# NUSTM/FacialMMT

Measured on AMD Instinct MI355X. Metric: utterances/sec T+A+V forward+bwd, 160-frame face seq, 1/2/4/8 GPU, higher is better.
Workload: dtype bf16; 1 GPU; configs[1]: T+A+V, RoBERTa-large (random init), 160-frame face seq (uint8 112x112 crops, fused pil-bicubic x2 + normalise), batch 4 utterances/GPU, bf16, fwd+bwd+clip+AdamW every step; global_batch=4, parallelism=dp1, hip_graphs=whole step: 2 graphs (fwd+bwd | clip+optimizer), text_encoder_concurrent_with_swin=True, swin_forward_pipelined_across_steps=False, text_encoder_parameters=bf16 with fp32 master weights in the optimizer

## Files before the change

facialmmt_amd/_lib.py:

```python
from __future__ import annotations

import ctypes as C
import os

_HERE = os.path.dirname(os.path.abspath(__file__))
LIB_PATH = os.path.join(_HERE, "libfmmt_hip.so")

F32, BF16 = 0, 1
GENERIC = 0x100
EPI_NONE, EPI_GELU, EPI_GELU_BWD, EPI_GELU_DG, EPI_MUL_AUX = 0, 1, 2, 3, 4
SAVE_DG = 0x200
BATCH_MAJOR = 0x400
RESIZE_PIL, RESIZE_CV2 = 0, 1

_p, _i, _f, _sz, _u64 = C.c_void_p, C.c_int, C.c_float, C.c_size_t, C.c_uint64

SIGNATURES = {
    "fmmt_version": (_i, []),
    "fmmt_linear_fwd": (_i, [_i, _i, _i, _i, _p, _i, _p, _i, _p, _p, _i, _p, _i, _p, _i, _p, _i, _p, _i, _p]),
    "fmmt_linear_splitk_workspace": (_sz, [_i, _i, _i]),
    "fmmt_linear_fwd_splitk": (_i, [_i, _i, _i, _i, _p, _i, _p, _i, _p, _p, _i, _p, _sz, _p]),
    "fmmt_linear_wgrad_workspace": (_sz, [_i, _i, _i, _i]),
    "fmmt_linear_wgrad": (_i, [_i, _i, _i, _i, _p, _i, _p, _i, _p, _p, _p, _i, _i, _p, _sz, _p]),
    "fmmt_linear_wgrad_partials": (_i, [_i, _i, _i, _i, _p, _i, _p, _i, _i, _p, _i, _i, _p, _sz, _p]),
    "fmmt_mlp_fwd": (_i, [_i, _i, _i, _p, _p, _p, _p, _p, _p, _p, _i, _p, _p, _p, _p]),
    "fmmt_mlp_ln_fwd": (_i, [_i, _i, _i, _p, _p, _p, _f, _p, _p, _p, _p, _p, _i, _p, _p, _p, _p, _p, _p, _p]),
    "fmmt_mlp_bwd_input": (_i, [_i, _i, _i, _p, _p, _p, _p, _p, _i, _p, _p, _p]),
    "fmmt_linear_ln_bwd_workspace": (_sz, [_i]),
    "fmmt_linear_ln_bwd": (_i, [_i, _i, _i, _i, _p, _p, _p, _p, _p, _p, _p, _p, _p, _p, _p, _sz, _p]),
    "fmmt_mlp_ln_bwd_input_workspace": (_sz, [_i]),
    "fmmt_mlp_ln_bwd_input": (_i, [_i, _i, _i, _p, _p, _p, _p, _p, _i, _p, _p, _p, _p, _p, _p, _p, _p, _p, _sz, _p]),
    "fmmt_linear_wgrad_finish": (_i, [_i, _i, _i, _i, _p, _p, _p, _sz, _p]),
    "fmmt_layernorm_fwd": (_i, [_i, _i, _i, _p, _p, _p, _f, _p, _p, _p, _i, _p]),
    "fmmt_layernorm_bwd_workspace": (_sz, [_i]),
    "fmmt_layernorm_bwd": (_i, [_i, _i, _i, _p, _p, _p, _p, _p, _p, _p, _p, _p, _i, _p, _sz, _p]),
    "fmmt_window_attn_fwd": (_i, [_i, _i, _i, _i, _i, _i, _i, _p, _p, _p, _p, _i, _i, _f, _p, _p, _p]),
    "fmmt_window_attn_bwd_workspace": (_sz, [_i]),
    "fmmt_window_attn_bwd": (_i, [_i, _i, _i, _i, _i, _i, _i, _p, _p, _p, _p, _p, _p, _p, _i, _i, _f, _p, _p, _p, _sz, _p]),
    "fmmt_window_block_fwd": (_i, [_i, _i, _i, _i, _i, _i, _i, _p, _p, _p, _f, _p, _p, _p, _p, _p, _p, _f, _p, _p, _p, _p, _p, _p, _p, _p]),
    "fmmt_window_block_fwd_ref": (_i, [_i, _i, _i, _i, _i, _i, _i, _p, _p, _p, _f, _p, _p, _p, _p, _p, _p, _f, _p, _p, _p, _p, _p, _p, _p, _p]),
    "fmmt_window_block_attn_bwd": (_i, [_i, _i, _i, _i, _i, _i, _i, _p, _p, _p, _p, _p, _p, _p, _p, _p, _f, _p, _p, _p, _p, _sz, _p]),
    "fmmt_window_block_attn_bwd_ref": (_i, [_i, _i, _i, _i, _i, _i, _i, _p, _p, _p, _p, _p, _p, _p, _p, _p, _f, _p, _p, _p, _p, _sz, _p]),
    "fmmt_linear_fwd_seg3": (_i, [_i, _i, _i, _i, _p, _i, _p, _p, _p, _i, _i, _p, _p, _p, _p, _i, _p]),
    "fmmt_select_frames_fwd": (_i, [_i, _i, _i, _i, _i, _i, _p, _p, _p, _p, _f, _p, _p, _p, _p]),
    "fmmt_select_frames_bwd": (_i, [_i, _i, _i, _i, _i, _i, _p, _p, _p, _p]),
    "fmmt_mha_fwd": (_i, [_i, _i, _i, _i, _i, _i, _p, _i, _p, _p, _i, _f, _p, _f, _u64, _p, _p, _i, _p, _p]),
    "fmmt_mha_bwd": (_i, [_i, _i, _i, _i, _i, _i, _p, _i, _p, _p, _i, _f, _p, _f, _u64, _p, _p, _p, _i, _p, _p, _i, _p, _p, _i, _p]),
    "fmmt_mha_avg_weights": (_i, [_i, _i, _i, _i, _i, _i, _p, _i, _p, _i, _f, _p, _f, _u64, _p, _p, _p, _p]),
    "fmmt_patch_im2col": (_i, [_i, _i, _p, _p, _p]),
    "fmmt_patch_col2im": (_i, [_i, _i, _p, _p, _p]),
    "fmmt_batchnorm1d_fwd": (_i, [_i, _i, _i, _p, _p, _p, _p, _p, _f, _f, _i, _p, _p, _p, _p]),
    "fmmt_batchnorm1d_bwd": (_i, [_i, _i, _i, _p, _p, _p, _p, _p, _i, _p, _p, _p, _p]),
    "fmmt_posemb_scale_fwd": (_i, [_i, _i, _i, _i, _p, _p, _f, _p, _p]),
    "fmmt_scale": (_i, [_i, _sz, _p, _f, _p, _p]),
    "fmmt_colsum": (_i, [_i, _i, _i, _i, _p, _i, _p, _p]),
    "fmmt_cast_batch": (_i, [_i, _i, _p, _p]),
    "fmmt_layernorm_bwd_bf16_workspace": (_sz, [_i, _i]),
    "fmmt_layernorm_bwd_bf16": (_i, [_i, _i, _f, _p, _p, _p, _p, _p, _p, _p, _sz, _p]),
    "fmmt_dropadd_ln_fwd": (_i, [_i, _i, _i, _f, _p, _p, _p, _p, _f, _u64, _p, _u64, _p, _p, _p]),
    "fmmt_dropadd_ln_bwd_workspace": (_sz, [_i, _i]),
    "fmmt_dropadd_ln_bwd": (_i, [_i, _i, _i, _f, _p, _p, _p, _f, _u64, _p, _u64, _p, _p, _p, _p, _p, _p, _sz, _p]),
    "fmmt_plm_dropadd_ln_fwd": (_i, [_i, _i, _f, _p, _p, _p, _p, _f, _u64, _p, _u64, _p, _p, _p]),
    "fmmt_embedding_bwd": (_i, [_i, _i, _i, _p, C.c_int64, _p, _p, _p]),
    "fmmt_plm_gelu_bwd_colsum_workspace": (_sz, [_i, _i]),
    "fmmt_plm_gelu_bwd_colsum": (_i, [_i, _i, _p, _p, _p, _p, _p, _sz, _p]),
    "fmmt_plm_dropadd_ln_bwd_workspace": (_sz, [_i, _i]),
    "fmmt_plm_dropadd_ln_bwd": (_i, [_i, _i, _f, _p, _p, _p, _f, _u64, _p, _u64, _p, _p, _p, _p, _p, _p, _sz, _p]),
    "fmmt_grad_handover": (_i, [_i, _i, _p, _p, _p, _p]),
    "fmmt_adamw_batch": (_i, [_i, _i, _p, _p, _p, _p, _f, _f, _f, _f, _f, _i, _p]),
    "fmmt_resize_table": (_i, [_i, _i, _i, _p, _p]),
    "fmmt_resize_band_rows": (_i, [_p, _i]),
    "fmmt_patch_embed_u8": (_i, [_i, _i, _i, _i, _p, _p, _p, _p, _p]),
    "fmmt_patch_embed_ln_fwd": (_i, [_i, _i, _i, _i, _p, _p, _p, _p, _p, _f, _p, _p, _p, _p, _p]),
    "fmmt_patch_embed_u8_ln_fwd": (_i, [_i, _i, _i, _i, _p, _p, _p, _p, _p, _p, _p, _f, _p, _p, _p, _p, _p, _p]),
    "fmmt_emotion_head_fwd": (_i, [_i, _i, _i, _i, _i, _p, _i, _p, _p, _p, _p, _p, _f, _p, _p, _p]),
    "fmmt_eval_accumulate": (_i, [_i, _i, _i, _p, _i, _p, _p, _p, _p, _p, _p, C.c_int64, C.c_int64, _p]),
}

POOL_HEAD_SIGNATURES = {
    "fmmt_pool_head_bwd_workspace": (_sz, [_i, _i, _i]),
    "fmmt_pool_head_fwd": (_i, [_i, _i, _i, _i, _i, _p, _p, _p, _p, _p, _p, _p, _p, _p, _f, _u64, _p, _p, _p, _p, _p, _p, _p, _sz, _p]),
    "fmmt_pool_head_bwd": (_i, [_i, _i, _i, _i, _i, _p, _p, _p, _p, _p, _p, _p, _p, _p, _p, _p, _p, _p, _p, _p, _p, _p, _p, _p, _sz, _p]),
}

RAGGED_SIGNATURES = {
    "fmmt_pack_frames": (_i, [_i, _i, _i, _sz, _p, _p, _p, _p, _p]),
    "fmmt_batchnorm1d_fwd_n": (_i, [_i, _i, _i, _p, _p, _p, _p, _p, _p, _f, _f, _i, _p, _p, _p, _p]),
    "fmmt_batchnorm1d_bwd_n": (_i, [_i, _i, _i, _p, _p, _p, _p, _p, _p, _i, _p, _p, _p, _p]),
    "fmmt_select_frames_fwd_n": (_i, [_i, _i, _i, _i, _i, _i, _p, _p, _p, _p, _f, _p, _p, _p, _p, _p]),
}

EVAL_COLLECT_SIGNATURES = {
    "fmmt_eval_accumulate_at": (_i, [_i, _i, _i, _p, _i, _p, _p, _p, _p, _p, _p, _p, _p, C.c_int64, _p]),
}

POOL_HEAD_ROWS_SIGNATURES = {
    "fmmt_pool_head_fwd_rows": (_i, [_i, _i, _i, _i, _i, _p, _p, _p, _p, _p, _p, _p, _p, _p, _f, _u64, _p, _p, _p, _p, _p, _p, _p, _p, _sz, _p]),
    "fmmt_pool_head_bwd_rows": (_i, [_i, _i, _i, _i, _i, _p, _p, _p, _p, _p, _p, _p, _p, _p, _p, _p, _p, _p, _p, _p, _p, _p, _p, _p, _p, _sz, _p]),
}

GUARD_SIGNATURES = {
    "fmmt_adamw_batch_guarded": (_i, [_i, _i, _p, _p, _p, _p, _f, _f, _f, _f, _f, _i, _p]),
    "fmmt_guard_commit": (_i, [_p, _p, _p, _p]),
    "fmmt_monitor_loss": (_i, [_p, _f, _p, _p]),
}
GUARD_LOSS_SUM, GUARD_MICRO_STEPS, GUARD_NONFINITE_LOSSES, GUARD_APPLIED, GUARD_SKIPPED, GUARD_LAST_NORM, GUARD_WORDS = 0, 1, 2, 3, 4, 5, 6

FMMT_EINVAL, FMMT_EALIGN, FMMT_EWORKSPACE = -1, -2, -3
_ERR = {-1: "FMMT_EINVAL (bad shape / unsupported size)", -2: "FMMT_EALIGN (pointer or leading dimension not 16-byte aligned)",
        -3: "FMMT_EWORKSPACE (workspace too small)"}

_lib = None


class FmmtError(RuntimeError):
    pass


def load():
    global _lib
    if _lib is not None:
        return _lib
    if not os.path.exists(LIB_PATH):
        raise FmmtError(f"{LIB_PATH} is missing: build it with `python -m facialmmt_amd.build` "
                        f"(or __graft_entry__.build()); there is no CPU / PyTorch fallback for the hot path")
    lib = C.CDLL(LIB_PATH)
    for name, (res, args) in list(SIGNATURES.items()) + list(POOL_HEAD_SIGNATURES.items()) + list(RAGGED_SIGNATURES.items()) + list(EVAL_COLLECT_SIGNATURES.items()) + list(POOL_HEAD_ROWS_SIGNATURES.items()) + list(GUARD_SIGNATURES.items()):
        fn = getattr(lib, name)
        fn.restype = res
        fn.argtypes = args
    _lib = lib
    return lib


def check(rc: int, what: str):
    if rc != 0:
        msg = _ERR.get(rc, f"hipError_t {rc}")
        raise FmmtError(f"{what} failed: {msg}")


def dtype_code(t) -> int:
    import torch
    if t == torch.float32:
        return F32
    if t == torch.bfloat16:
        return BF16
    raise FmmtError(f"unsupported activation dtype {t}: the HIP path computes in float32 (parity) or bfloat16 (throughput)")
```

facialmmt_amd/build.py:

```python
from __future__ import annotations

import glob
import os
import subprocess
import sys
from concurrent.futures import ThreadPoolExecutor

HERE = os.path.dirname(os.path.abspath(__file__))
CSRC = os.path.join(HERE, "csrc")
OUT = os.path.join(HERE, "libfmmt_hip.so")
SOURCES = ["gemm.hip", "layernorm.hip", "attn.hip", "wattn_mfma.hip", "wattn_bwd_ref.hip", "wblock.hip", "wblock_ref.hip", "mha_mfma.hip", "misc.hip", "preproc.hip", "mlp_fused.hip", "mlp_ref.hip", "patch_ln.hip", "lin_lnbwd.hip", "plm_fused.hip", "frame_filter.hip", "eval.hip", "pool_head.hip", "ragged.hip", "guard.hip"]
FLAGS = ["--offload-arch=gfx950", "-O3", "-std=c++17", "-fPIC", "-ffp-contract=fast"]


def _stale(target, deps):
    if not os.path.exists(target):
        return True
    t = os.path.getmtime(target)
    return any(os.path.getmtime(d) > t for d in deps)


def build(force: bool = False, verbose: bool = True, tag: str = "") -> str:
    hipcc = os.environ.get("HIPCC", "/opt/rocm/bin/hipcc")
    tag = tag or os.environ.get("FMMT_BUILD_TAG", "")
    csrc = os.environ.get("FMMT_CSRC_DIR", CSRC) if tag else CSRC
    headers = sorted(glob.glob(os.path.join(csrc, "*.h"))) + [os.path.join(csrc, "..", "..", "include", h) for h in ("fmmt.h", "fmmt_pool_head.h", "fmmt_ragged.h", "fmmt_eval_collect.h", "fmmt_pool_head_rows.h", "fmmt_guard.h")]
    objdir = os.path.join(HERE, "build_" + tag if tag else "build")
    out = os.path.join(HERE, f"libfmmt_hip_{tag}.so") if tag else OUT
    os.makedirs(objdir, exist_ok=True)
    jobs = []
    for s in SOURCES:
        src = os.path.join(csrc, s)
        obj = os.path.join(objdir, s.replace(".hip", ".o"))
        if force or _stale(obj, [src] + headers):
            jobs.append((src, obj))

    def cc(job):
        src, obj = job
        cmd = [hipcc] + FLAGS + os.environ.get("FMMT_CFLAGS", "").split() + ["-c", src, "-o", obj]
        if verbose:
            print(" ".join(cmd), flush=True)
        subprocess.run(cmd, check=True)

    with ThreadPoolExecutor(max_workers=4) as ex:
        list(ex.map(cc, jobs))
    objs = [os.path.join(objdir, s.replace(".hip", ".o")) for s in SOURCES]
    if force or jobs or _stale(out, objs):
        cmd = [hipcc, "--offload-arch=gfx950", "-shared", "-fPIC", "-o", out] + objs
        if verbose:
            print(" ".join(cmd), flush=True)
        subprocess.run(cmd, check=True)
    return out


if __name__ == "__main__":
    print(build(force="--force" in sys.argv))
```

facialmmt_amd/csrc/gemm.hip:

```cpp
#include "gemm_common.h"
#include "gemm_ph.h"
#include "gemm_ph3.h"
#include <stdlib.h>
#include <type_traits>

namespace {

template <typename T> struct Mma;
template <> struct Mma<bf16> {
    static constexpr int KM = 32;
    static constexpr int KP = 8;
    using frag = bf16x8;
    static __device__ __forceinline__ f32x4 mma(frag a, frag b, f32x4 c) {
        return __builtin_amdgcn_mfma_f32_16x16x32_bf16(a, b, c, 0, 0, 0);
    }
    static __device__ __forceinline__ frag load(const bf16* p) { return *reinterpret_cast<const bf16x8*>(p); }
};
template <> struct Mma<float> {
    static constexpr int KM = 4;
    static constexpr int KP = 1;
    using frag = float;
    static __device__ __forceinline__ f32x4 mma(frag a, frag b, f32x4 c) {
        return __builtin_amdgcn_mfma_f32_16x16x4f32(a, b, c, 0, 0, 0);
    }
// ... 362 lines not shown
    }

    auto compute = [&](int buf) {
        const T* sb = S + buf * STAGE;
        bf16x8 wf[NT], xf[MT];
#pragma unroll
        for (int b = 0; b < NT; ++b) wf[b] = *reinterpret_cast<const bf16x8*>(sb + woff[b]);
#pragma unroll
        for (int a = 0; a < MT; ++a) xf[a] = *reinterpret_cast<const bf16x8*>(sb + xoff[a]);
#pragma unroll
        for (int a = 0; a < MT; ++a)
#pragma unroll
            for (int b = 0; b < NT; ++b) acc[a][b] = __builtin_amdgcn_mfma_f32_16x16x32_bf16(wf[b], xf[a], acc[a][b], 0, 0, 0);
    };

    issue(0, 0);
    if (nk > 1) issue(1, BK);
    if constexpr (NK > 0) {
#pragma unroll
        for (int kt = 0; kt < NK; ++kt) {
            wait_stage(kt + 1 < NK);
            __builtin_amdgcn_s_barrier();
            if (kt + 2 < NK) issue((kt + 2) % 3, (kt + 2) * BK);
            compute(kt % 3);
        }
    } else {
        int cur = 0;
        for (int kt = 0; kt < nk; ++kt) {
            wait_stage(kt + 1 < nk);
            __builtin_amdgcn_s_barrier();
            if (kt + 2 < nk) issue(cur == 0 ? 2 : cur - 1, (kt + 2) * BK);
            compute(cur);
            cur = cur == 2 ? 0 : cur + 1;
        }
    }
    const bool plain = p.epi == 0 && !p.y_pre && !p.res && !p.aux && !p.rowscale;
    if (p.part || (!plain && BN != 128)) {
        nt_epilogue<T, MT, NT>(p, acc, m0 + wm * 64, n0 + wn * WN, li, lg);
    } else if (plain) {
        nt_epilogue_slab<T, MT, NT, 2, BN, 512>(p, acc, smem, wm, wn, li, lg, tid, m0, n0);
    } else {
        if constexpr (BN == 128) {
            asm volatile("s_waitcnt lgkmcnt(0)" ::: "memory");
            __builtin_amdgcn_s_barrier();
            nt_epilogue_wslab<T>(p, acc, smem + wave * (16 * 272), lane, li, lg, m0 + wm * 64, n0 + wn * WN);
        }
    }
}


template <int N> __device__ __forceinline__ void wait_vm() { asm volatile("s_waitcnt vmcnt(%0)" ::"n"(N) : "memory"); }

#define FMMT_RD(o, ad) "ds_read_b128 %" #o ", %" #ad "\n\t"
template <int NF>
__device__ __forceinline__ void nt_read_frags(bf16x8 (&o)[NF], const unsigned (&ad)[NF]) {
    static_assert(NF >= 10 && NF <= 12, "fragments per K block");
    if constexpr (NF == 12) {
        asm volatile(FMMT_RD(0, 12) FMMT_RD(1, 13) FMMT_RD(2, 14) FMMT_RD(3, 15) FMMT_RD(4, 16) FMMT_RD(5, 17) FMMT_RD(6, 18) FMMT_RD(7, 19)
                     FMMT_RD(8, 20) FMMT_RD(9, 21) FMMT_RD(10, 22) FMMT_RD(11, 23) "s_waitcnt lgkmcnt(0)"
                     : "=&v"(o[0]), "=&v"(o[1]), "=&v"(o[2]), "=&v"(o[3]), "=&v"(o[4]), "=&v"(o[5]), "=&v"(o[6]), "=&v"(o[7]),
                       "=&v"(o[8]), "=&v"(o[9]), "=&v"(o[10]), "=&v"(o[11])
                     : "v"(ad[0]), "v"(ad[1]), "v"(ad[2]), "v"(ad[3]), "v"(ad[4]), "v"(ad[5]), "v"(ad[6]), "v"(ad[7]),
                       "v"(ad[8]), "v"(ad[9]), "v"(ad[10]), "v"(ad[11])
                     : "memory");
    } else if constexpr (NF == 11) {
        asm volatile(FMMT_RD(0, 11) FMMT_RD(1, 12) FMMT_RD(2, 13) FMMT_RD(3, 14) FMMT_RD(4, 15) FMMT_RD(5, 16) FMMT_RD(6, 17) FMMT_RD(7, 18)
                     FMMT_RD(8, 19) FMMT_RD(9, 20) FMMT_RD(10, 21) "s_waitcnt lgkmcnt(0)"
                     : "=&v"(o[0]), "=&v"(o[1]), "=&v"(o[2]), "=&v"(o[3]), "=&v"(o[4]), "=&v"(o[5]), "=&v"(o[6]), "=&v"(o[7]),
                       "=&v"(o[8]), "=&v"(o[9]), "=&v"(o[10])
                     : "v"(ad[0]), "v"(ad[1]), "v"(ad[2]), "v"(ad[3]), "v"(ad[4]), "v"(ad[5]), "v"(ad[6]), "v"(ad[7]),
                       "v"(ad[8]), "v"(ad[9]), "v"(ad[10])
                     : "memory");
    } else {
        asm volatile(FMMT_RD(0, 10) FMMT_RD(1, 11) FMMT_RD(2, 12) FMMT_RD(3, 13) FMMT_RD(4, 14) FMMT_RD(5, 15) FMMT_RD(6, 16) FMMT_RD(7, 17)
                     FMMT_RD(8, 18) FMMT_RD(9, 19) "s_waitcnt lgkmcnt(0)"
                     : "=&v"(o[0]), "=&v"(o[1]), "=&v"(o[2]), "=&v"(o[3]), "=&v"(o[4]), "=&v"(o[5]), "=&v"(o[6]), "=&v"(o[7]),
                       "=&v"(o[8]), "=&v"(o[9])
                     : "v"(ad[0]), "v"(ad[1]), "v"(ad[2]), "v"(ad[3]), "v"(ad[4]), "v"(ad[5]), "v"(ad[6]), "v"(ad[7]),
                       "v"(ad[8]), "v"(ad[9])
                     : "memory");
    }
}

template <int BN, int BK, int NBUF, bool BATCH = true, bool HASOP = false, bool PIPE = false>
__global__ __launch_bounds__(512) void linear_nt_p256_kernel(LinArgs p) {
    static_assert(BK == 64 && BATCH, "one K step, batched fragment reads");
    using T = bf16;
    constexpr int BM = 256, PITCH = BK, MT = 8, NT = BN / 64, WN = BN / 4, CW = 4 * NT;
    constexpr int RPI = 8;
    constexpr int STAGE = (BN + BM) * PITCH;
    constexpr int NI = (BN + BM) / RPI;
    constexpr int CNT_LO = NI / 8;
    static_assert(BN % 64 == 0 && (NBUF - 2) * (CNT_LO + 2) <= 63, "tile / vmcnt immediate");
    extern __shared__ __attribute__((aligned(16))) char smem[];
    T* S = reinterpret_cast<T*>(smem);
    float* bias_s = reinterpret_cast<float*>(smem + (size_t)NBUF * STAGE * sizeof(T));

    const int tid = threadIdx.x, lane = tid & 63;
    const int wave = __builtin_amdgcn_readfirstlane(tid >> 6);
    const int wm = wave >> 2, wn = wave & 3;
    const int li = lane & 15, lg = lane >> 4;
    const T* __restrict__ xg = reinterpret_cast<const T*>(p.x);
    const T* __restrict__ wg = reinterpret_cast<const T*>(p.w);
    const int nk = p.K / BK;

    typedef __attribute__((address_space(1))) const void gptr_t;
    typedef __attribute__((address_space(3))) void lptr_t;
    auto key = [](int row) { return (row >> 1) & 7; };
    const int rl = lane >> 3, cl = lane & 7;
    const bool wperm = HASOP ? !p.chan_rows : true;
    auto wchan = [&](int r) {
        const int w = r / WN, q = r - w * WN;
        return wperm ? w * WN + chan_of<CW>(q >> 4, (q >> 2) & 3, q & 3) : r;
    };

    const int my_cnt = (NI - wave + 7) / 8 + (wave == 7 ? 1 : 0);
    const bool cnt_hi = my_cnt > CNT_LO;
    constexpr int NP = (NI + 7) / 8;
    unsigned poff[NP], boff = 0;
    auto tile_offsets = [&](int m0, int n0) {
#pragma unroll
        for (int i = 0; i < NP; ++i) {
            const int row0 = (i * 8 + wave) * RPI;
            if (row0 < BN) {
                const int r = row0 + rl;
                poff[i] = ((unsigned)(n0 + wchan(r)) * (unsigned)p.ldw + (unsigned)((cl ^ key(r)) << 3)) * 2u;
            } else {
                const int rx = row0 - BN;
                const int rb = min(m0 + rx, p.M - RPI);
                poff[i] = ((unsigned)(rb + rl) * (unsigned)p.ldx + (unsigned)((cl ^ key(rx + rl)) << 3)) * 2u;
            }
        }
        boff = p.bias ? (unsigned)(n0 + min(lane * 4, BN - 4)) * 4u : (unsigned)lane * 16u;
    };
    auto issue_piece = [&](int i, int slot, unsigned kbyte) {
        const int j = i * 8 + wave;
        if (j < NI) {
            const int row0 = j * RPI;
            const char* b = row0 < BN ? reinterpret_cast<const char*>(wg) : reinterpret_cast<const char*>(xg);
            __builtin_amdgcn_global_load_lds((gptr_t*)(b + (size_t)(poff[i] + kbyte)), (lptr_t*)(S + slot * STAGE + row0 * PITCH), 16, 0, 0);
        }
    };
    auto issue_bias = [&](int par) {
        if (wave == 7) {
            const char* b = p.bias ? reinterpret_cast<const char*>(p.bias) : reinterpret_cast<const char*>(wg);
            __builtin_amdgcn_global_load_lds((gptr_t*)(b + (size_t)boff), (lptr_t*)(bias_s + par * 256), 16, 0, 0);
        }
    };
    auto wait_landed = [&](int ahead, int stores) {
        const int n = (ahead <= 0 ? 0 : (ahead == 1 ? 1 : 2)) * (CNT_LO + (cnt_hi ? 1 : 0)) + stores;
        switch (n) {
#define FMMT_W(N) case N: wait_vm<N>(); break;
            FMMT_W(1) FMMT_W(2) FMMT_W(3) FMMT_W(4) FMMT_W(5) FMMT_W(6) FMMT_W(7) FMMT_W(8) FMMT_W(9) FMMT_W(10) FMMT_W(11) FMMT_W(12)
            FMMT_W(13) FMMT_W(14) FMMT_W(15) FMMT_W(16) FMMT_W(17) FMMT_W(18) FMMT_W(19) FMMT_W(20) FMMT_W(21) FMMT_W(22) FMMT_W(23) FMMT_W(24)
#undef FMMT_W
            default: wait_vm<0>(); break;
        }
    };
    static_assert(NBUF >= 2 && NBUF <= 4, "ring depth");
    static_assert(NI % 8 == 0 || NI % 8 <= 7, "wave 7 never owns a high count plus the bias slab");

    f32x4 acc[MT][NT];
#pragma unroll
    for (int a = 0; a < MT; ++a)
#pragma unroll
        for (int b = 0; b < NT; ++b) acc[a][b] = f32x4{0.f, 0.f, 0.f, 0.f};
    int woff[NT], xoff[MT];
#pragma unroll
    for (int b = 0; b < NT; ++b) {
// ... 13 lines not shown
            unsigned ad[NT + MT];
#pragma unroll
            for (int b = 0; b < NT; ++b) ad[b] = (((unsigned)woff[b] * 2u) ^ (kk ? 64u : 0u)) + sbase;
#pragma unroll
            for (int a = 0; a < MT; ++a) ad[NT + a] = (((unsigned)xoff[a] * 2u) ^ (kk ? 64u : 0u)) + sbase;
            bf16x8 fr[NT + MT];
            nt_read_frags<NT + MT>(fr, ad);
#pragma unroll
            for (int a = 0; a < MT; ++a)
#pragma unroll
                for (int b = 0; b < NT; ++b) acc[a][b] = __builtin_amdgcn_mfma_f32_16x16x32_bf16(fr[b], fr[NT + a], acc[a][b], 0, 0, 0);
        }
    };

    const int G = gridDim.x;
    const int total = p.tiles_m * p.tiles_n;
    const int first = ((int)blockIdx.x & 7) * (G >> 3) + ((int)blockIdx.x >> 3);
    const int tstep = G;
    const int ntile = first < total ? (total - first + G - 1) / G : 0;
    const int nsteps = ntile * nk;
    int it = first, ik = 0, ipar = 0, islot = 0;
    tile_offsets((first / p.tiles_n) * BM, (first % p.tiles_n) * BN);
    auto issue_advance = [&]() {
        islot = islot + 1 == NBUF ? 0 : islot + 1;
        if (++ik == nk) {
            ik = 0;
            it += tstep;
            ipar ^= 1;
            tile_offsets((it / p.tiles_n) * BM, (it % p.tiles_n) * BN);
        }
    };
    auto issue_next = [&]() {
        const unsigned kbyte = (unsigned)ik * (BK * 2);
#pragma unroll
        for (int i = 0; i < NP; ++i) issue_piece(i, islot, kbyte);
        issue_bias(ipar);
        issue_advance();
    };
#pragma unroll
    for (int s = 0; s < NBUF - 1; ++s)
        if (s < nsteps) issue_next();
    int ct = first, ck = 0, cpar = 0, cslot = 0, st_prev = 0;
    EpiPre<MT, NT> pre;
    constexpr int PR = BN == 192 ? 32 : 16;
    constexpr int SP = BN * 2 + 16;
    constexpr int CPR = BN / 8;
    constexpr int NSL = PR * CPR / 256;
    static_assert((PR * CPR) % 256 == 0, "whole store instructions");
    char* scratch = smem + (size_t)NBUF * STAGE * sizeof(T) + 2 * 256 * sizeof(float) + (size_t)wm * PR * SP;
    const bool lds_epi = !HASOP && p.epi == 0 && !p.y_pre && !p.part && p.K <= 1536;
    T* __restrict__ yg = reinterpret_cast<T*>(p.y);
    constexpr int XB = NT >= 4 ? 2 : 4;
    constexpr int UB = MT / XB, U = (BK / 32) * UB;
    bf16x8 pw[2][NT], px[2][XB];
    auto request = [&](int slot, int u) {
        const unsigned sbase = lds0 + (unsigned)slot * (unsigned)(STAGE * 2);
        const int kk = u / UB, h = u % UB;
        const unsigned flip = kk ? 64u : 0u;
        if (h == 0) {
#pragma unroll
            for (int b = 0; b < NT; ++b)
                asm volatile("ds_read_b128 %0, %1" : "=v"(pw[kk & 1][b]) : "v"((((unsigned)woff[b] * 2u) ^ flip) + sbase) : "memory");
        }
#pragma unroll
        for (int a = 0; a < XB; ++a)
            asm volatile("ds_read_b128 %0, %1" : "=v"(px[u & 1][a]) : "v"((((unsigned)xoff[h * XB + a] * 2u) ^ flip) + sbase) : "memory");
    };
    auto landed = [&](int u) {
        const int kk = u / UB, h = u % UB;
        asm volatile("s_waitcnt lgkmcnt(0)" ::: "memory");
#pragma unroll
        for (int a = 0; a < XB; ++a) asm volatile("" : "+v"(px[u & 1][a]));
        if (h == 0) {
#pragma unroll
            for (int b = 0; b < NT; ++b) asm volatile("" : "+v"(pw[kk & 1][b]));
        }
    };
    bool pend = false;
    auto sync_stage = [&](int k, int ck_k, int ct_k) {
        wait_landed(min(nsteps - 1 - k, NBUF - 2), st_prev);
        st_prev = 0;
        __builtin_amdgcn_s_barrier();
        if constexpr (HASOP) {
            if (ck_k == nk - 1) nt_epilogue_prefetch<MT, NT>(p, pre, (ct_k / p.tiles_n) * BM + wm * 128, (ct_k % p.tiles_n) * BN + wn * WN, li, lg);
        }
        if constexpr (PIPE) {
            pend = k + NBUF - 1 < nsteps;
        } else {
            if (k + NBUF - 1 < nsteps) issue_next();
        }
    };
    constexpr int NG = BN == 256 ? 1 : 2;
    auto issue_group = [&](int g) {
        if (!pend) return;
        const unsigned kbyte = (unsigned)ik * (BK * 2);
#pragma unroll
        for (int i = 0; i < NP; ++i)
            if ((i * NG) / NP == g) issue_piece(i, islot, kbyte);
        if (g == NG - 1) {
            issue_bias(ipar);
            issue_advance();
        }
    };
    if constexpr (PIPE) {
        if (nsteps > 0) {
            sync_stage(0, 0, first);
            issue_group(0);
            request(0, 0);
            landed(0);
        }
    }
    for (int s = 0; s < nsteps; ++s) {
        if constexpr (PIPE) {
            const int nslot = cslot + 1 == NBUF ? 0 : cslot + 1;
#pragma unroll
            for (int u = 0; u < U; ++u) {
                int grp_now = -1;
                if (u + 1 < U) {
                    request(cslot, u + 1);
                    if (u + 1 < NG) grp_now = u + 1;
                } else if (s + 1 < nsteps) {
                    const bool wrap = ck + 1 == nk;
                    sync_stage(s + 1, wrap ? 0 : ck + 1, wrap ? ct + tstep : ct);
                    request(nslot, 0);
                    grp_now = 0;
                }
                __builtin_amdgcn_sched_barrier(0);
                if (grp_now >= 0) issue_group(grp_now);
                {
                    const int kk = u / UB, h = u % UB;
#pragma unroll
                    for (int a = 0; a < XB; ++a)
#pragma unroll
                        for (int b = 0; b < NT; ++b)
                            acc[h * XB + a][b] = __builtin_amdgcn_mfma_f32_16x16x32_bf16(pw[kk & 1][b], px[u & 1][a], acc[h * XB + a][b], 0, 0, 0);
                }
                __builtin_amdgcn_sched_barrier(0);
                if (u + 1 < U) landed(u + 1);
                else if (s + 1 < nsteps) landed(0);
            }
        } else {
            sync_stage(s, ck, ct);
            compute(cslot);
        }
        cslot = cslot + 1 == NBUF ? 0 : cslot + 1;
        if (++ck == nk) {
            const int m0 = (ct / p.tiles_n) * BM, n0 = (ct % p.tiles_n) * BN;
            if (p.bias) {
#pragma unroll
                for (int b = 0; b < NT; ++b) {
                    const f32x4 bb = *reinterpret_cast<const f32x4*>(bias_s + cpar * 256 + wn * WN + chan_of<CW>(b, lg, 0));
#pragma unroll
                    for (int a = 0; a < MT; ++a) acc[a][b] += bb;
                }
            }
            const bool gelu_any = p.epi == FMMT_EPI_GELU || p.epi == FMMT_EPI_GELU_DG;
            if (BN == 256 && !HASOP && !p.part && ((p.epi == 0 && !p.y_pre) || gelu_any)) {
                if constexpr (BN == 256) {
                    char* ws = smem + (size_t)NBUF * STAGE * sizeof(T) + 2 * 256 * sizeof(float) + wave * (16 * 144);
                    T* __restrict__ ypre = reinterpret_cast<T*>(p.y_pre);
                    const int mw = m0 + wm * 128, nw = n0 + wn * WN;
                    const int rr = lane >> 3, rc = lane & 7;
                    auto emit = [&](int a, T* dst, bool gelu) {
#pragma unroll
                        for (int c = 0; c < 2; ++c) {
                            float t[8];
#pragma unroll
// ... 10 lines not shown
                            const bf16x8 v = *reinterpret_cast<const bf16x8*>(ws + (h * 8 + rr) * 144 + rc * 16);
                            if (m < p.M) __builtin_nontemporal_store(v, reinterpret_cast<bf16x8*>(dst + (size_t)m * p.ldy + nw + rc * 8));
                        }
                    };
                    auto emit_dg = [&](int a) {
                        bf16x8 dv[2];
#pragma unroll
                        for (int c = 0; c < 2; ++c) {
                            float t[8], d[8];
#pragma unroll
                            for (int e = 0; e < 8; ++e) t[e] = acc[a][2 * c + (e >> 2)][e & 3];
                            gelu_both_inplace<T>(t, d, 8);
                            bf16x8 v;
#pragma unroll
                            for (int e = 0; e < 8; ++e) { v[e] = (bf16)t[e]; dv[c][e] = (bf16)d[e]; }
                            *reinterpret_cast<bf16x8*>(ws + li * 144 + chan_of<CW>(2 * c, lg, 0) * 2) = v;
                        }
#pragma unroll
                        for (int pass = 0; pass < 2; ++pass) {
                            T* dst = pass == 0 ? yg : ypre;
#pragma unroll
                            for (int h = 0; h < 2; ++h) {
                                const int m = mw + a * 16 + h * 8 + rr;
                                const bf16x8 v = *reinterpret_cast<const bf16x8*>(ws + (h * 8 + rr) * 144 + rc * 16);
                                if (m < p.M && dst) __builtin_nontemporal_store(v, reinterpret_cast<bf16x8*>(dst + (size_t)m * p.ldy + nw + rc * 8));
                            }
                            if (pass == 0) {
#pragma unroll
                                for (int c = 0; c < 2; ++c) *reinterpret_cast<bf16x8*>(ws + li * 144 + chan_of<CW>(2 * c, lg, 0) * 2) = dv[c];
                            }
                        }
                    };
                    const bool two = gelu_any && ypre != nullptr;
#pragma unroll
                    for (int a = 0; a < MT; ++a) {
                        if (p.epi == FMMT_EPI_GELU_DG) {
                            emit_dg(a);
                        } else {
                            if (two) emit(a, ypre, false);
                            emit(a, yg, p.epi == FMMT_EPI_GELU);
                        }
                    }
                    if (!PIPE && mw + 128 <= p.M) st_prev = MT * 2 * (two ? 2 : 1);
                }
            } else if (lds_epi) {
                const int rows_left = p.M - (m0 + wm * 128);
                auto round = [&](int pass) {
                    asm volatile("s_waitcnt lgkmcnt(0)" ::: "memory");
                    __builtin_amdgcn_s_barrier();
#pragma unroll
                    for (int f = 0; f < PR / 16; ++f) {
                        const int a = pass * (PR / 16) + f;
                        char* row = scratch + (f * 16 + li) * SP + (wn * WN) * 2;
#pragma unroll
                        for (int c = 0; c < NT / 2; ++c) {
                            bf16x8 v;
#pragma unroll
                            for (int e = 0; e < 8; ++e) v[e] = (bf16)acc[a][2 * c + (e >> 2)][e & 3];
                            *reinterpret_cast<bf16x8*>(row + chan_of<CW>(2 * c, lg, 0) * 2) = v;
                        }
                        if constexpr (NT % 2) {
                            bf16x4 v;
#pragma unroll
                            for (int e = 0; e < 4; ++e) v[e] = (bf16)acc[a][NT - 1][e];
                            *reinterpret_cast<bf16x4*>(row + chan_of<CW>(NT - 1, lg, 0) * 2) = v;
                        }
                    }
                    asm volatile("s_waitcnt lgkmcnt(0)" ::: "memory");
                    __builtin_amdgcn_s_barrier();
#pragma unroll
                    for (int i = 0; i < NSL; ++i) {
                        const int q = i * 256 + wn * 64 + lane, r = q / CPR, cc = q - r * CPR;
                        const int row = pass * PR + r;
                        if (row < rows_left) {
                            const bf16x8 v = *reinterpret_cast<const bf16x8*>(scratch + r * SP + cc * 16);
                            __builtin_nontemporal_store(v, reinterpret_cast<bf16x8*>(yg + (size_t)(m0 + wm * 128 + row) * p.ldy + n0 + cc * 8));
                        }
                    }
                };
#pragma unroll
                for (int pass = 0; pass < 128 / PR; ++pass) round(pass);
                if (!PIPE && rows_left >= 128) st_prev = (128 / PR) * NSL;
            } else if constexpr (HASOP) {
                nt_epilogue<T, MT, NT, true, true>(p, acc, m0 + wm * 128, n0 + wn * WN, li, lg, &pre);
            } else {
                nt_epilogue<T, MT, NT, true, false, true>(p, acc, m0 + wm * 128, n0 + wn * WN, li, lg);
            }
#pragma unroll
            for (int a = 0; a < MT; ++a)
#pragma unroll
                for (int b = 0; b < NT; ++b) acc[a][b] = f32x4{0.f, 0.f, 0.f, 0.f};
            ck = 0;
            ct += tstep;
            cpar ^= 1;
        }
    }
}

template <int BN, int BK, int NBUF, bool BATCH, bool HASOP, bool PIPE = false>
int launch_p256_b(const LinArgs& a, hipStream_t st) {
    constexpr size_t lds = (size_t)NBUF * (BN + 256) * BK * 2 + 2 * 256 * sizeof(float) + (BN == 256 ? 8 * 16 * 144 : 2 * (BN == 192 ? 32 : 16) * (BN * 2 + 16));
    static_assert(lds <= 160 * 1024, "LDS");
    static FmmtLdsOnce lds_once;
    if (int rc_ = lds_once.set(reinterpret_cast<const void*>(&linear_nt_p256_kernel<BN, BK, NBUF, BATCH, HASOP, PIPE>), (int)lds)) return rc_;
    LinArgs p = a;
    p.tiles_m = (a.M + 255) / 256;
    p.tiles_n = a.N / BN;
    hipLaunchKernelGGL((linear_nt_p256_kernel<BN, BK, NBUF, BATCH, HASOP, PIPE>), dim3(256), dim3(512), lds, st, p);
    FMMT_CHECK_LAUNCH();
    return 0;
}
template <int BN, int BK, int NBUF>
int launch_p256(const LinArgs& a, hipStream_t st) {
    if constexpr (BN != 256) {
        if (a.res || a.aux || a.rowscale) return launch_p256_b<BN, BK, NBUF, true, true>(a, st);
    }
    if (a.K >= 384) return launch_p256_b<BN, BK, NBUF, true, false, true>(a, st);
    return launch_p256_b<BN, BK, NBUF, true, false>(a, st);
}

int p256_plan(const LinArgs& a) {
    constexpr int P256_MINM = 16384;
    if (a.ksplit || a.M < P256_MINM || a.M % 16 || a.K % 64 || a.K < 96 || a.ldx % 8 || a.ldw % 8) return 0;
    if ((unsigned long long)a.M * a.ldx >= (1ull << 31) || (unsigned long long)a.N * a.ldw >= (1ull << 31)) return 0;
    const bool has_op = a.res || a.aux || a.rowscale;
    if (has_op && (a.aux || a.ldres % 8 || a.ldaux % 8)) return 0;
    const int tm = (a.M + 255) / 256;
    int best = 0;
    double best_cost = 0;
    const int cand[3] = {256, 192, 128};
    const double pen[3] = {1.0, 1.04, 1.10};
    for (int i = 0; i < 3; ++i) {
        const int bn = cand[i];
        if (a.N % bn) continue;
        if (has_op && bn == 256) continue;
        const int tiles = tm * (a.N / bn);
        if (tiles < 256) continue;
        const double cost = (double)((tiles + 255) / 256) * bn * pen[i];
        if (!best || cost < best_cost) {
            best = bn;
            best_cost = cost;
        }
    }
    return best;
}

template <typename T, int BM, int BN, int BK, int NBUF, bool GLDS = false, bool SEG = false>
int launch_nt(const LinArgs& a, hipStream_t st) {
    constexpr int VEC = Vec<T>::N;
    constexpr size_t lds = (size_t)NBUF * (BM + BN) * (GLDS ? BK : BK + VEC) * sizeof(T);
    static FmmtLdsOnce lds_once;
    if (lds > 65536) {
        if (int rc_ = lds_once.set(reinterpret_cast<const void*>(&linear_nt_kernel<T, BM, BN, BK, NBUF, GLDS, SEG>), (int)lds)) return rc_;
    }
    LinArgs p = a;
    p.tiles_n = (a.N + BN - 1) / BN;
    p.tiles_m = (a.M + BM - 1) / BM;
    const int grid = p.tiles_m * p.tiles_n;
    const int splits = a.ksplit ? (a.K + a.ksplit - 1) / a.ksplit : 1;
    hipLaunchKernelGGL((linear_nt_kernel<T, BM, BN, BK, NBUF, GLDS, SEG>), dim3(grid, splits), dim3(256), lds, st, p);
    FMMT_CHECK_LAUNCH();
    return 0;
}

template <typename T, int BM, int BN>
int dispatch_nt_bk(const LinArgs& a, hipStream_t st) {
    if constexpr (sizeof(T) == 2) {
        if (!a.ksplit && a.K == 96) return launch_nt<T, BM, BN, 96, 1>(a, st);
        if (!a.ksplit && a.K <= 64) return launch_nt<T, BM, BN, 64, 1>(a, st);
        if (a.K % 64 == 0 && !a.ksplit && a.ldx % 8 == 0 && a.ldw % 8 == 0) {
            if constexpr (BM == 64) {
                const int tiles = ((a.M + BM - 1) / BM) * ((a.N + BN - 1) / BN);
                if (a.K >= 2048 && tiles <= 256) return launch_nt<T, BM, BN, 64, 4, true>(a, st);
            }
            return launch_nt<T, BM, BN, 64, 2, true>(a, st);
        }
        if (a.K % 64 == 0 && (!a.ksplit || a.ksplit % 64 == 0)) return launch_nt<T, BM, BN, 64, 2>(a, st);
        return launch_nt<T, BM, BN, 32, 2>(a, st);
    } else {
        return launch_nt<T, BM, BN, 16, 2>(a, st);
    }
}

int ph_plan(const LinArgs& a, int* epi3) {
    const bool mul_aux = a.epi == FMMT_EPI_MUL_AUX && a.aux && !a.res && !a.y_pre && !a.bias;
    if (a.ksplit || a.part || (a.aux && !mul_aux)) return 0;
    const bool gelu_pre = a.epi == FMMT_EPI_GELU && a.y_pre, has_op = a.res || a.rowscale;
    if (!gelu_pre && !mul_aux && (a.epi != 0 || a.y_pre)) return 0;
    if (gelu_pre && (has_op || a.K < 1536)) return 0;
    if (mul_aux && (a.ldaux % 8 || (unsigned long long)a.M * a.ldaux >= (1ull << 31))) return 0;
    if (a.M < 4096 || a.M % 8 || a.N % 128 || a.K % 64 || a.K < 192 || a.ldx % 8 || a.ldw % 8 || a.ldy % 8) return 0;
    if (a.res && a.ldres % 8) return 0;
    if (a.rowscale && a.rows_per_scale <= 0) return 0;
    if ((unsigned long long)a.M * a.ldx >= (1ull << 31) || (unsigned long long)a.N * a.ldw >= (1ull << 31) || (unsigned long long)a.M * a.ldy >= (1ull << 31) ||
        (a.res && (unsigned long long)a.M * a.ldres >= (1ull << 31)))
        return 0;
    if (a.N % 256) {
        if (gelu_pre || a.K > 512) return 0;
        const long long t384 = (long long)((a.M + 383) / 384) * (a.N / 128), r384 = (t384 + 255) / 256;
// ... 38 lines not shown
        if (const int bn = p256_plan(a))
            return bn == 256 ? launch_p256<256, 64, 2>(a, st) : bn == 192 ? launch_p256<192, 64, 2>(a, st) : launch_p256<128, 64, 3>(a, st);
        constexpr int DEEP_MINM = 65536, DEEP_MINK = 96;
        const bool big = a.M >= DEEP_MINM && !a.ksplit && a.K % 32 == 0 && a.K >= DEEP_MINK && a.ldx % 8 == 0 && a.ldw % 8 == 0 &&
                         !(a.K == 96 && a.epi == FMMT_EPI_GELU);
        if (big && (a.N % 128 == 0 || n96)) {
            constexpr size_t lds = (size_t)3 * (256 + 128) * 64 * 2;
            constexpr size_t lds96 = (size_t)3 * (256 + 96) * 32 * 2;
            static FmmtLdsOnce lds_once[7];
            {
                const void* fns[] = {reinterpret_cast<const void*>(&linear_nt_deep_kernel),
                                     reinterpret_cast<const void*>(&linear_nt_deep32_kernel<0, 128>),
                                     reinterpret_cast<const void*>(&linear_nt_deep32_kernel<6, 128>),
                                     reinterpret_cast<const void*>(&linear_nt_deep32_kernel<3, 128>),
                                     reinterpret_cast<const void*>(&linear_nt_deep32_kernel<0, 96>),
                                     reinterpret_cast<const void*>(&linear_nt_deep32_kernel<6, 96>),
                                     reinterpret_cast<const void*>(&linear_nt_deep32_kernel<3, 96>)};
                const int sizes[] = {(int)lds, (int)lds / 2, (int)lds / 2, (int)lds / 2, (int)lds96, (int)lds96, (int)lds96};
                for (int i = 0; i < 7; ++i)
                    if (int rc_ = lds_once[i].set(fns[i], sizes[i])) return rc_;
            }
            LinArgs p = a;
            p.tiles_m = (a.M + 255) / 256;
                    if (n96) {
                p.tiles_n = a.N / 96;
                if (a.K == 192) hipLaunchKernelGGL((linear_nt_deep32_kernel<6, 96>), dim3(p.tiles_m * p.tiles_n), dim3(512), lds96, st, p);
                else if (a.K == 96) hipLaunchKernelGGL((linear_nt_deep32_kernel<3, 96>), dim3(p.tiles_m * p.tiles_n), dim3(512), lds96, st, p);
                else hipLaunchKernelGGL((linear_nt_deep32_kernel<0, 96>), dim3(p.tiles_m * p.tiles_n), dim3(512), lds96, st, p);
                FMMT_CHECK_LAUNCH();
                return 0;
            }
            p.tiles_n = a.N / 128;
            if (a.epi != 0 || a.K <= 512 || a.K % 64 != 0) {
                if (a.K == 192) hipLaunchKernelGGL((linear_nt_deep32_kernel<6, 128>), dim3(p.tiles_m * p.tiles_n), dim3(512), lds / 2, st, p);
                else if (a.K == 96) hipLaunchKernelGGL((linear_nt_deep32_kernel<3, 128>), dim3(p.tiles_m * p.tiles_n), dim3(512), lds / 2, st, p);
                else hipLaunchKernelGGL((linear_nt_deep32_kernel<0, 128>), dim3(p.tiles_m * p.tiles_n), dim3(512), lds / 2, st, p);
            } else {
                hipLaunchKernelGGL(linear_nt_deep_kernel, dim3(p.tiles_m * p.tiles_n), dim3(512), lds, st, p);
            }
            FMMT_CHECK_LAUNCH();
            return 0;
        }
    }
    return n96 ? dispatch_nt_bk<T, 128, 96>(a, st) : dispatch_nt_bk<T, 128, 128>(a, st);
}

template <typename T>
__global__ void splitk_finish_kernel(const float* __restrict__ part, int splits, int M, int N, const float* __restrict__ bias,
                                     T* __restrict__ y, int ldy) {
    const size_t i = (size_t)blockIdx.x * blockDim.x + threadIdx.x;
    if (i >= (size_t)M * N) return;
    const int m = (int)(i / N), n = (int)(i - (size_t)m * N);
    float t = bias ? bias[n] : 0.f;
    for (int s = 0; s < splits; ++s) t += part[(size_t)s * M * N + i];
    y[(size_t)m * ldy + n] = from_f32<T>(t);
}

int splitk_plan(int M, int N, int K, int* ksplit) {
    const int bm = M <= 4096 ? 64 : 128;
    const int tiles = ((M + bm - 1) / bm) * ((N + 127) / 128);
    if (tiles >= 128 || K < 4096) { *ksplit = 0; return 1; }
    int splits = 512 / tiles;
    if (splits > 32) splits = 32;
    int ks = (K + splits - 1) / splits;
    ks = (ks + 63) / 64 * 64;
    *ksplit = ks;
    return (K + ks - 1) / ks;
}

struct TnArgs {
    int M, N, K;
    const void* dy; int lddy;
    const void* x; int ldx;
    float* part_w;
    float* part_b;
    const float* rowscale; int rows_per_scale;
    int tiles_k;
    int chunk;
    int tiles_n;
    int x_gelu;
    int* hdr;
    int splits;
    int npad;
};

__device__ __forceinline__ int tn_swz(int row) { return (row & 3) | (((row >> 3) & 1) << 2); }
__device__ __forceinline__ bf16x8 lds_tr_frag_swz(const bf16* s, int row0, int c0, int li, int lg) {
    const int r = row0 + lg * 8 + (li >> 2);
    const bf16* a0 = s + r * 128 + (((c0 >> 4) ^ tn_swz(r)) << 4) + (li & 3) * 4;
    typedef __attribute__((address_space(3))) s16x4 lds_s16x4;
    s16x4 lo = __builtin_amdgcn_ds_read_tr16_b64_v4i16((lds_s16x4*)(a0));
    s16x4 hi = __builtin_amdgcn_ds_read_tr16_b64_v4i16((lds_s16x4*)(a0 + 4 * 128));
    union { struct { s16x4 lo, hi; } s; bf16x8 v; } u;
    u.s.lo = lo;
    u.s.hi = hi;
    return u.v;
}

template <int BMS> struct TnWaves { static constexpr int value = BMS >= 64 ? 2 : 3; };
template <typename T, int BMS, bool FEW = false, int PF = 1>
__global__ __launch_bounds__(256) __attribute__((amdgpu_waves_per_eu(TnWaves<BMS>::value)))
void linear_tn_kernel(TnArgs p) {
    constexpr int VEC = Vec<T>::N;
    constexpr bool SWZ = sizeof(T) == 2;
    constexpr int PITCH = SWZ ? 128 : 128 + VEC;
    constexpr int CV = 128 / VEC;
    constexpr int NV = BMS * CV / 256;
    constexpr int KM = sizeof(T) == 2 ? 32 : 4;

    extern __shared__ __attribute__((aligned(16))) char smem[];
    T* As = reinterpret_cast<T*>(smem);
    T* Bs = As + 2 * BMS * PITCH;
    float* bsum = reinterpret_cast<float*>(Bs + 2 * BMS * PITCH);

    const int tid = threadIdx.x, lane = tid & 63, wave = tid >> 6;
    const int wn = wave >> 1, wk = wave & 1;
    const int li = lane & 15, lg = lane >> 4;
    const int tiles = p.tiles_n * p.tiles_k;
    const int logical = xcd_remap(blockIdx.x, gridDim.x);
    const int split = logical / tiles, tile = logical - split * tiles;
    const int tile_n = tile / p.tiles_k, tile_k = tile % p.tiles_k;
    const int n0 = tile_n * 128, k0 = tile_k * 128;
    const int mbeg = split * p.chunk, mend = min(p.M, mbeg + p.chunk);
    if (p.hdr && blockIdx.x == 0 && tid == 0) { p.hdr[0] = p.splits; p.hdr[1] = 0; p.hdr[2] = p.N; }

    const T* __restrict__ dyg = reinterpret_cast<const T*>(p.dy);
    const T* __restrict__ xg = reinterpret_cast<const T*>(p.x);
    const bool do_bias = (p.part_b != nullptr) && (tile_k == 0);

    struct Regs { Vec<T> a[NV], b[NV]; float s[NV]; };
    Regs R0, R1;
    float colsum[VEC];
#pragma unroll
    for (int e = 0; e < VEC; ++e) colsum[e] = 0.f;

    int sidx[NV], srem[NV];
#pragma unroll
    for (int i = 0; i < NV; ++i) {
        const int m = mbeg + (tid + i * 256) / CV;
        sidx[i] = p.rowscale ? m / p.rows_per_scale : 0;
        srem[i] = p.rowscale ? m - sidx[i] * p.rows_per_scale : 0;
    }
    auto gload = [&](Regs& R, int mb) {
#pragma unroll
        for (int i = 0; i < NV; ++i) {
            const int v = tid + i * 256;
            const int row = v / CV, c = (v % CV) * VEC;
            const int m = mb + row;
            const bool mv = m < mend;
            R.a[i] = (mv && n0 + c < p.N) ? ldvec<T>(dyg + (size_t)m * p.lddy + n0 + c) : zerovec<T>();
            if (p.rowscale) {
                R.s[i] = mv ? p.rowscale[sidx[i]] : 0.f;
                srem[i] += BMS;
                while (srem[i] >= p.rows_per_scale) {
                    srem[i] -= p.rows_per_scale;
                    ++sidx[i];
                }
            }
            R.b[i] = (mv && k0 + c < p.K) ? ldvec<T>(xg + (size_t)m * p.ldx + k0 + c) : zerovec<T>();
        }
    };
    auto lstore = [&](Regs& R, int buf) {
#pragma unroll
        for (int i = 0; i < NV; ++i) {
            const int v = tid + i * 256;
            const int row = v / CV, c = (v % CV) * VEC;
// ... 241 lines not shown
        }
    if (do_bias && li == 0) {
#pragma unroll
        for (int a = 0; a < 4; ++a)
#pragma unroll
            for (int r = 0; r < 4; ++r) p.part_b[n0 + a * 16 + lg * 4 + r] = accb[a][r];
    }
}

int launch_tn_few(int M, int N, int K, const void* dy, int lddy, const void* x, int ldx, float* dw, float* db, int* hdr, hipStream_t st) {
    constexpr int lds = 80 * 1024;
    static FmmtLdsOnce lds_once;
    if (int rc_ = lds_once.set(reinterpret_cast<const void*>(&linear_tn_few_kernel), lds)) return rc_;
    TnArgs a{M, N, K, dy, lddy, x, ldx, dw, db, nullptr, 1, K / 64, (M + 7) / 8, N / 64, 0, hdr, 1};
    hipLaunchKernelGGL(linear_tn_few_kernel, dim3((N / 64) * (K / 64)), dim3(512), lds, st, a);
    FMMT_CHECK_LAUNCH();
    return 0;
}

bool tn_few_ok(int M, int N, int K, int dtype) {
    return dtype == FMMT_BF16 && M > 128 && M <= 2048 && N % 64 == 0 && K % 64 == 0 && (N / 64) * (K / 64) >= 8 && (N / 64) * (K / 64) <= 1024;
}

__device__ __forceinline__ int tn_swz2(int row) { return ((row >> 1) & 1) | (((row >> 3) & 1) << 1); }
template <int CH>
__device__ __forceinline__ int tn_sigma(int row, int blk) {
    if constexpr (CH == 192) return blk < 8 ? (blk ^ tn_swz(row)) : 8 + ((blk & 3) ^ tn_swz2(row));
    else return blk ^ tn_swz(row);
}


#define FMMT_TR2(o0, o1, ad, im) "ds_read_b64_tr_b16 %" #o0 ", %" #ad "\n\tds_read_b64_tr_b16 %" #o1 ", %" #ad " offset:%" #im "\n\t"
template <int FA, int OFFA, int OFFB>
__device__ __forceinline__ void tn_read12(s16x4 (&o)[24], const unsigned (&ad)[12]) {
    static_assert(FA == 8 || FA == 6, "fragment split");
    if constexpr (FA == 8) {
        asm volatile(FMMT_TR2(0, 1, 24, 36) FMMT_TR2(2, 3, 25, 36) FMMT_TR2(4, 5, 26, 36) FMMT_TR2(6, 7, 27, 36)
                     FMMT_TR2(8, 9, 28, 36) FMMT_TR2(10, 11, 29, 36) FMMT_TR2(12, 13, 30, 36) FMMT_TR2(14, 15, 31, 36)
                     FMMT_TR2(16, 17, 32, 37) FMMT_TR2(18, 19, 33, 37) FMMT_TR2(20, 21, 34, 37) FMMT_TR2(22, 23, 35, 37)
                     "s_waitcnt lgkmcnt(0)"
                     : "=&v"(o[0]), "=&v"(o[1]), "=&v"(o[2]), "=&v"(o[3]), "=&v"(o[4]), "=&v"(o[5]), "=&v"(o[6]), "=&v"(o[7]),
                       "=&v"(o[8]), "=&v"(o[9]), "=&v"(o[10]), "=&v"(o[11]), "=&v"(o[12]), "=&v"(o[13]), "=&v"(o[14]), "=&v"(o[15]),
                       "=&v"(o[16]), "=&v"(o[17]), "=&v"(o[18]), "=&v"(o[19]), "=&v"(o[20]), "=&v"(o[21]), "=&v"(o[22]), "=&v"(o[23])
                     : "v"(ad[0]), "v"(ad[1]), "v"(ad[2]), "v"(ad[3]), "v"(ad[4]), "v"(ad[5]), "v"(ad[6]), "v"(ad[7]),
                       "v"(ad[8]), "v"(ad[9]), "v"(ad[10]), "v"(ad[11]), "n"(OFFA), "n"(OFFB)
                     : "memory");
    } else {
        asm volatile(FMMT_TR2(0, 1, 24, 36) FMMT_TR2(2, 3, 25, 36) FMMT_TR2(4, 5, 26, 36) FMMT_TR2(6, 7, 27, 36)
                     FMMT_TR2(8, 9, 28, 36) FMMT_TR2(10, 11, 29, 36) FMMT_TR2(12, 13, 30, 37) FMMT_TR2(14, 15, 31, 37)
                     FMMT_TR2(16, 17, 32, 37) FMMT_TR2(18, 19, 33, 37) FMMT_TR2(20, 21, 34, 37) FMMT_TR2(22, 23, 35, 37)
                     "s_waitcnt lgkmcnt(0)"
                     : "=&v"(o[0]), "=&v"(o[1]), "=&v"(o[2]), "=&v"(o[3]), "=&v"(o[4]), "=&v"(o[5]), "=&v"(o[6]), "=&v"(o[7]),
                       "=&v"(o[8]), "=&v"(o[9]), "=&v"(o[10]), "=&v"(o[11]), "=&v"(o[12]), "=&v"(o[13]), "=&v"(o[14]), "=&v"(o[15]),
                       "=&v"(o[16]), "=&v"(o[17]), "=&v"(o[18]), "=&v"(o[19]), "=&v"(o[20]), "=&v"(o[21]), "=&v"(o[22]), "=&v"(o[23])
                     : "v"(ad[0]), "v"(ad[1]), "v"(ad[2]), "v"(ad[3]), "v"(ad[4]), "v"(ad[5]), "v"(ad[6]), "v"(ad[7]),
                       "v"(ad[8]), "v"(ad[9]), "v"(ad[10]), "v"(ad[11]), "n"(OFFA), "n"(OFFB)
                     : "memory");
    }
}

template <int TNn, int TKk, int NBUF, int WN, bool SCALED = false>
__global__ __launch_bounds__(512) void linear_tn_dma_kernel(TnArgs p) {
    using T = bf16;
    constexpr int BT = 32, WK = 8 / WN;
    constexpr int CPRA = TNn / 8, CPRB = TKk / 8;
    constexpr int A_EL = BT * TNn, B_EL = BT * TKk, STAGE = A_EL + B_EL;
    constexpr int NIA = BT * CPRA / 64, NIB = BT * CPRB / 64, NI = NIA + NIB;
    static_assert((BT * CPRA) % 64 == 0 && (BT * CPRB) % 64 == 0, "whole DMA instructions per operand");
    constexpr int CNT = NI / 8, REM = NI % 8;
    constexpr int FA = TNn / (16 * WN), FB = TKk / (16 * WK);
    static_assert(TNn % (16 * WN) == 0 && TKk % (16 * WK) == 0 && FA + FB == 12 && NBUF >= 2 && NBUF <= 5, "tile");
    extern __shared__ __attribute__((aligned(16))) char smem[];
    T* S = reinterpret_cast<T*>(smem);

    const int tid = threadIdx.x, lane = tid & 63;
    const int wave = __builtin_amdgcn_readfirstlane(tid >> 6);
    const int wn = wave / WK, wk = wave % WK;
    const int li = lane & 15, lg = lane >> 4;
    const int tiles = p.tiles_n * p.tiles_k;
    const int logical = xcd_remap(blockIdx.x, gridDim.x);
    const int split = logical / tiles, tile = logical - split * tiles;
    const int tile_n = tile / p.tiles_k, tile_k = tile % p.tiles_k;
    const int n0 = tile_n * TNn, k0 = tile_k * TKk;
    const int mbeg = split * p.chunk, mend = min(p.M, mbeg + p.chunk);
    const int NP = p.npad ? p.npad : p.N;
    if (p.hdr && blockIdx.x == 0 && tid == 0) { p.hdr[0] = p.splits; p.hdr[1] = TNn; p.hdr[2] = NP; }
    const T* __restrict__ dyg = reinterpret_cast<const T*>(p.dy);
    const T* __restrict__ xg = reinterpret_cast<const T*>(p.x);
    const bool extra = wave < REM;

    typedef __attribute__((address_space(1))) const void gptr_t;
    typedef __attribute__((address_space(3))) void lptr_t;
    constexpr int NISS = CNT + (REM != 0 ? 1 : 0);
    unsigned goff[NISS];
#pragma unroll
    for (int i = 0; i < NISS; ++i) {
        const int j = i * 8 + wave;
        if (j < NIA) {
            const int q = j * 64 + lane, row = q / CPRA, pos = q - row * CPRA;
            const int gpos = (tn_sigma<TNn>(row, pos >> 1) << 1) | (pos & 1);
            int col = n0 + gpos * 8;
            if (col >= p.N) col -= NP - p.N;
            goff[i] = (unsigned)(row * p.lddy + col) * 2u;
        } else {
            const int q = (j - NIA) * 64 + lane, row = q / CPRB, pos = q - row * CPRB;
            const int gpos = (tn_sigma<TKk>(row, pos >> 1) << 1) | (pos & 1);
            goff[i] = (unsigned)(row * p.ldx + k0 + gpos * 8) * 2u;
        }
    }
    auto issue_one = [&](T* base, int i, int mb) {
        const int j = i * 8 + wave;
        const char* sb = j < NIA ? reinterpret_cast<const char*>(dyg) + (size_t)mb * p.lddy * 2 : reinterpret_cast<const char*>(xg) + (size_t)mb * p.ldx * 2;
        T* dst = j < NIA ? base + j * 512 : base + A_EL + (j - NIA) * 512;
        __builtin_amdgcn_global_load_lds((gptr_t*)(sb + goff[i]), (lptr_t*)dst, 16, 0, 0);
    };
    auto issue = [&](int slot, int mb) {
        T* base = S + slot * STAGE;
#pragma unroll
        for (int i = 0; i < CNT; ++i) issue_one(base, i, mb);
        if constexpr (REM != 0)
            if (extra) issue_one(base, CNT, mb);
    };
    auto wait_landed = [&](bool steady) {
        if (!steady) { wait_vm<0>(); return; }
        if constexpr (REM != 0) {
            if (extra) wait_vm<(NBUF - 2) * (CNT + 1)>();
            else wait_vm<(NBUF - 2) * CNT>();
        } else {
            wait_vm<(NBUF - 2) * CNT>();
        }
    };

    static_assert(FA > WK && FA <= 3 * WK, "positions 0, WK and 2 WK");
    const int o0 = wk * p.tiles_k + tile_k;
    const bool has0 = p.part_b != nullptr && o0 < FA;
    const bool has1 = has0 && p.tiles_k == 1 && o0 + WK < FA;
    const bool has2 = has1 && FA > 2 * WK && o0 + 2 * WK < FA;
    const int rot = has0 ? o0 : 0;
    auto block_of = [&](int j) { const int a = j + rot; return a >= FA ? a - FA : a; };
    unsigned foff[12];
    {
        const int r0 = lg * 8 + (li >> 2);
#pragma unroll
        for (int a = 0; a < FA; ++a) {
            const int c0 = wn * (TNn / WN) + block_of(a) * 16;
            foff[a] = (unsigned)(r0 * TNn + (tn_sigma<TNn>(r0, c0 >> 4) << 4) + (li & 3) * 4) * 2u;
        }
#pragma unroll
        for (int b = 0; b < FB; ++b) {
            const int c0 = wk * (TKk / WK) + b * 16;
            foff[FA + b] = (unsigned)(A_EL + r0 * TKk + (tn_sigma<TKk>(r0, c0 >> 4) << 4) + (li & 3) * 4) * 2u;
        }
    }
    const unsigned lds0 = (unsigned)(uintptr_t)(lptr_t*)S;

    f32x4 acc[FA][FB];
#pragma unroll
    for (int a = 0; a < FA; ++a)
#pragma unroll
        for (int b = 0; b < FB; ++b) acc[a][b] = f32x4{0.f, 0.f, 0.f, 0.f};
    f32x4 accb0 = f32x4{0.f, 0.f, 0.f, 0.f}, accb1 = f32x4{0.f, 0.f, 0.f, 0.f}, accb2 = f32x4{0.f, 0.f, 0.f, 0.f};
    bf16x8 ones;
#pragma unroll
    for (int e = 0; e < 8; ++e) ones[e] = (bf16)1.0f;

    auto compute = [&](int slot) {
        const unsigned sbase = lds0 + (unsigned)slot * (unsigned)(STAGE * 2);
// ... 426 lines not shown
                   const float* rowscale, int rows_per_scale, int x_epi, int* hdr, hipStream_t st) {
    if (x_epi != 0 && x_epi != FMMT_EPI_GELU) return FMMT_EINVAL;
    if (tn_few_ok(M, N, K, dtype) && !rowscale && !x_epi && lddy % 8 == 0 && ldx % 8 == 0)
        return launch_tn_few(M, N, K, dy, lddy, x, ldx, part_w, part_b, hdr, st);
    if (dtype == FMMT_BF16 && hdr && !x_epi && lddy % 8 == 0 && ldx % 8 == 0) {
        const TnPlan pd = tn_plan_dma(M, N, K);
        const bool scaled_ok = !rowscale || (rows_per_scale >= 32 && pd.tn && pd.tk != 192 && pd.chunk / rows_per_scale + 2 <= 1024);
        if (pd.tn && scaled_ok) {
            TnArgs a{M, N, K, dy, lddy, x, ldx, part_w, part_b, rowscale, rows_per_scale, pd.tiles_k, pd.chunk, pd.tiles_n, 0, hdr, pd.splits, pd.npad};
            const int grid = pd.tiles_n * pd.tiles_k * pd.splits;
            if (rowscale) return pd.tk == 256 ? launch_tn_dma<256, 256, 4, 2, true>(a, grid, st) : launch_tn_dma<192, 384, 4, 2, true>(a, grid, st);
            if (pd.tk == 192) return launch_tn_dma<384, 192, 4, 4>(a, grid, st);
            return pd.tk == 256 ? launch_tn_dma<256, 256, 4, 2>(a, grid, st) : launch_tn_dma<192, 384, 4, 2>(a, grid, st);
        }
    }
    const TnPlan pl = tn_plan(M, N, K, dtype);
    TnArgs a{M, N, K, dy, lddy, x, ldx, part_w, part_b, rowscale, rows_per_scale, pl.tiles_k, pl.chunk, pl.tiles_n, x_epi == FMMT_EPI_GELU, hdr, pl.splits};
    dim3 grid(pl.tiles_n * pl.tiles_k * pl.splits);
    if (dtype == FMMT_BF16) {
        if (M <= 4096) return launch_tn<bf16, 32, true>(a, grid, st);
        if (M <= 262144) return launch_tn<bf16, 64, false, 2>(a, grid, st);
        return launch_tn<bf16, 32, false, 2>(a, grid, st);
    }
    return launch_tn<float, 16>(a, grid, st);
}
}

extern "C" int fmmt_linear_wgrad_partials(int dtype, int M, int N, int K,
                                          const void* dy, int lddy, const void* x, int ldx, int want_bias,
                                          const float* rowscale, int rows_per_scale, int x_epi,
                                          void* workspace, size_t workspace_bytes, void* stream) {
    if (M <= 0 || N <= 0 || K <= 0) return FMMT_EINVAL;
    if (dtype != FMMT_BF16 && dtype != FMMT_F32) return FMMT_EINVAL;
    const int vec = dtype == FMMT_BF16 ? 8 : 4;
    if (N % vec || K % vec || lddy % vec || ldx % vec) return FMMT_EINVAL;
    if (rowscale && rows_per_scale <= 0) return FMMT_EINVAL;
    if (!aligned16(dy) || !aligned16(x) || !aligned16(workspace)) return FMMT_EALIGN;
    if (workspace_bytes < tn_ws_bytes(M, N, K, dtype)) return FMMT_EWORKSPACE;
    const int smax = tn_smax(M, N, K, dtype);
    int* hdr = reinterpret_cast<int*>(workspace);
    float* part_b = reinterpret_cast<float*>(reinterpret_cast<char*>(workspace) + TN_HDR);
    float* part_w = part_b + (size_t)smax * tn_rows(M, N, K, dtype);
    return launch_tn_plan(dtype, M, N, K, dy, lddy, x, ldx, part_w, want_bias ? part_b : nullptr, rowscale, rows_per_scale, x_epi, hdr,
                          reinterpret_cast<hipStream_t>(stream));
}

extern "C" int fmmt_linear_wgrad_finish(int dtype, int M, int N, int K, float* dw, float* db,
                                        const void* workspace, size_t workspace_bytes, void* stream) {
    if (M <= 0 || N <= 0 || K <= 0 || !dw) return FMMT_EINVAL;
    if (dtype != FMMT_BF16 && dtype != FMMT_F32) return FMMT_EINVAL;
    if (!aligned16(dw) || !aligned16(workspace)) return FMMT_EALIGN;
    if (workspace_bytes < tn_ws_bytes(M, N, K, dtype)) return FMMT_EWORKSPACE;
    hipStream_t st = reinterpret_cast<hipStream_t>(stream);
    const int smax = tn_smax(M, N, K, dtype);
    const int* hdr = reinterpret_cast<const int*>(workspace);
    const float* part_b = reinterpret_cast<const float*>(reinterpret_cast<const char*>(workspace) + TN_HDR);
    const int rows = tn_rows(M, N, K, dtype);
    const float* part_w = part_b + (size_t)smax * rows;
    const size_t nw = (size_t)N * K;
    if (nw % 4 || N % 4) return FMMT_EINVAL;
    const int wblocks = (int)(((size_t)rows * K / 4 + 63) / 64), bblocks = db ? (rows / 4 + 63) / 64 : 0;
    hipLaunchKernelGGL(reduce_partials_kernel, dim3(wblocks + bblocks), dim3(64 * RP_GROUPS), 0, st, part_w, dw, nw, hdr, wblocks, part_b, db, (size_t)N, K);
    FMMT_CHECK_LAUNCH();
    return 0;
}

extern "C" int fmmt_linear_wgrad(int dtype, int M, int N, int K,
                                 const void* dy, int lddy, const void* x, int ldx,
                                 float* dw, float* db, const float* rowscale, int rows_per_scale, int x_epi,
                                 void* workspace, size_t workspace_bytes, void* stream) {
    if (!aligned16(dw)) return FMMT_EALIGN;
    const bool few = M > 0 && N > 0 && K > 0 && tn_few_ok(M, N, K, dtype) && !rowscale && !x_epi && lddy % 8 == 0 && ldx % 8 == 0;
    if (M > 0 && N > 0 && K > 0 && (dtype == FMMT_BF16 || dtype == FMMT_F32) && (few || tn_smax(M, N, K, dtype) == 1)) {
        const int vec = dtype == FMMT_BF16 ? 8 : 4;
        if (N % vec || K % vec || lddy % vec || ldx % vec) return FMMT_EINVAL;
        if (rowscale && rows_per_scale <= 0) return FMMT_EINVAL;
        if (!aligned16(dy) || !aligned16(x)) return FMMT_EALIGN;
        return launch_tn_plan(dtype, M, N, K, dy, lddy, x, ldx, dw, db, rowscale, rows_per_scale, x_epi, nullptr, reinterpret_cast<hipStream_t>(stream));
    }
    if (int rc = fmmt_linear_wgrad_partials(dtype, M, N, K, dy, lddy, x, ldx, db != nullptr, rowscale, rows_per_scale, x_epi,
                                            workspace, workspace_bytes, stream)) return rc;
    return fmmt_linear_wgrad_finish(dtype, M, N, K, dw, db, workspace, workspace_bytes, stream);
}
```

facialmmt_amd/csrc/gemm_common.h:

```cpp
#pragma once
#include "fmmt_common.h"
#include "../../include/fmmt.h"

namespace {

struct LinArgs {
    int M, N, K;
    const void* x; int ldx;
    const void* w; int ldw;
    const float* bias;
    void* y; int ldy;
    void* y_pre;
    int epi;
    const void* aux; int ldaux;
    const void* res; int ldres;
    const float* rowscale; int rows_per_scale;
    int tiles_n, tiles_m;
    int chan_rows;
    int ksplit;
    float* part;
    const void* w1; const void* w2;
    const float* bias1; const float* bias2;
    int wseg, wseg_mode;
};

template <int CW>
__device__ __forceinline__ int chan_of(int nt, int g, int r) {
    const int t0 = nt * 4;
    return (t0 < (CW / 8) * 8) ? (t0 / 8) * 32 + g * 8 + (t0 % 8) + r : (CW / 8) * 32 + g * 4 + r;
}

template <int MT, int NT>
struct EpiPre {
    bf16x8 full[MT][NT / 2 > 0 ? NT / 2 : 1];
    bf16x4 tail[MT];
    float rs[MT];
};
template <int MT, int NT>
__device__ __forceinline__ void nt_epilogue_prefetch(const LinArgs& p, EpiPre<MT, NT>& pre, int mbase, int nbase, int li, int lg) {
    const bool use_aux = p.epi == FMMT_EPI_GELU_BWD || p.epi == FMMT_EPI_MUL_AUX;
    const bf16* __restrict__ src = reinterpret_cast<const bf16*>(use_aux ? p.aux : p.res);
    const int ld = use_aux ? p.ldaux : p.ldres;
#pragma unroll
    for (int a = 0; a < MT; ++a) {
        const int m = min(mbase + a * 16 + li, p.M - 1);
        pre.rs[a] = row_scale(p.rowscale, m, p.rows_per_scale);
        if (src) {
#pragma unroll
            for (int c = 0; c < NT / 2; ++c)
                pre.full[a][c] = *reinterpret_cast<const bf16x8*>(src + (size_t)m * ld + nbase + chan_of<4 * NT>(2 * c, lg, 0));
            if constexpr (NT % 2) pre.tail[a] = *reinterpret_cast<const bf16x4*>(src + (size_t)m * ld + nbase + chan_of<4 * NT>(NT - 1, lg, 0));
        }
    }
}

template <typename T, int MT, int NT, bool BIAS_DONE = false, bool PRE = false, bool NOOPS = false>
__device__ __forceinline__ void nt_epilogue(const LinArgs& p, f32x4 (&acc)[MT][NT], int mbase, int nbase, int li, int lg,
                                            const EpiPre<MT, NT>* pre = nullptr) {
    constexpr int VEC = Vec<T>::N;
    T* __restrict__ yg = reinterpret_cast<T*>(p.y);
    T* __restrict__ ypre = reinterpret_cast<T*>(p.y_pre);
    const T* __restrict__ auxg = reinterpret_cast<const T*>(p.aux);
    const T* __restrict__ resg = reinterpret_cast<const T*>(p.res);
        if (p.part) {
            float* pp = p.part + (size_t)blockIdx.y * p.M * p.N;
#pragma unroll
            for (int a = 0; a < MT; ++a) {
                const int m = mbase + a * 16 + li;
                if (m >= p.M) continue;
#pragma unroll
                for (int b = 0; b < NT; ++b) {
                    const int n = nbase + chan_of<4 * NT>(b, lg, 0);
                    if (n + 4 <= p.N) *reinterpret_cast<f32x4*>(pp + (size_t)m * p.N + n) = acc[a][b];
                }
            }
            return;
        }
        constexpr int TPC = VEC / 4;
#pragma unroll
        for (int a = 0; a < MT; ++a) {
            const int m = mbase + a * 16 + li;
            if (m >= p.M) continue;
            float rs;
            if constexpr (NOOPS) rs = 1.0f;
            else if constexpr (PRE) rs = pre->rs[a];
            else rs = row_scale(p.rowscale, m, p.rows_per_scale);
#pragma unroll
            for (int b0 = 0; b0 < NT; b0 += TPC) {
                const int w = (NT - b0 >= TPC) ? VEC : 4;
                const int n = nbase + chan_of<4 * NT>(b0, lg, 0);
                if (n + w > p.N) continue;
                float v[VEC];
#pragma unroll
                for (int e = 0; e < VEC; ++e) v[e] = (e < w) ? acc[a][b0 + (e >> 2)][e & 3] : 0.f;
                if (!BIAS_DONE && p.bias) {
#pragma unroll
                    for (int e4 = 0; e4 < VEC; e4 += 4)
                        if (e4 < w) {
                            const f32x4 bb = *reinterpret_cast<const f32x4*>(p.bias + n + e4);
#pragma unroll
                            for (int r = 0; r < 4; ++r) v[e4 + r] += bb[r];
                        }
                }
                auto load_chunk = [&](const T* base, int ld, float* out) {
                    if constexpr (PRE) {
                        if (w == VEC) {
#pragma unroll
                            for (int e = 0; e < 8; ++e) out[e] = (float)pre->full[a][b0 / 2][e];
                        } else {
#pragma unroll
                            for (int e = 0; e < 4; ++e) out[e] = (float)pre->tail[a][e];
                        }
                        return;
                    }
                    if (w == VEC) {
                        const Vec<T> t = ldvec<T>(base + (size_t)m * ld + n);
#pragma unroll
                        for (int e = 0; e < VEC; ++e) out[e] = t.get(e);
                    } else {
#pragma unroll
                        for (int e = 0; e < 4; ++e) out[e] = to_f32(base[(size_t)m * ld + n + e]);
                    }
                };
                auto store_chunk = [&](T* base, int ld, const float* in) {
                    if (w == VEC) {
                        Vec<T> t;
#pragma unroll
                        for (int e = 0; e < VEC; ++e) t.set(e, in[e]);
                        stvec<T>(base + (size_t)m * ld + n, t);
                    } else {
                        T o[4];
#pragma unroll
                        for (int e = 0; e < 4; ++e) o[e] = from_f32<T>(in[e]);
                        *reinterpret_cast<uint2*>(base + (size_t)m * ld + n) = *reinterpret_cast<const uint2*>(o);
                    }
                };
                if (p.epi == FMMT_EPI_GELU) {
                    if (ypre) store_chunk(ypre, p.ldy, v);
                    gelu_inplace<T>(v, VEC);
                } else if (p.epi == FMMT_EPI_GELU_DG) {
                    float d[VEC];
                    gelu_both_inplace<T>(v, d, VEC);
                    if (ypre) store_chunk(ypre, p.ldy, d);
                } else if (!NOOPS && p.epi == FMMT_EPI_GELU_BWD) {
                    float ax[VEC];
                    load_chunk(auxg, p.ldaux, ax);
#pragma unroll
                    for (int e = 0; e < VEC; ++e) ax[e] = (e < w) ? ax[e] : 0.f;
                    gelu_grad_mul_inplace<T>(v, ax, VEC);
                } else if (!NOOPS && p.epi == FMMT_EPI_MUL_AUX) {
                    float ax[VEC];
                    load_chunk(auxg, p.ldaux, ax);
#pragma unroll
                    for (int e = 0; e < VEC; ++e) v[e] *= (e < w) ? ax[e] : 0.f;
                }
#pragma unroll
                for (int e = 0; e < VEC; ++e) v[e] *= rs;
                if (!NOOPS && resg) {
                    float rx[VEC];
                    load_chunk(resg, p.ldres, rx);
#pragma unroll
                    for (int e = 0; e < VEC; ++e) v[e] += (e < w) ? rx[e] : 0.f;
                }
                store_chunk(yg, p.ldy, v);
            }
        }
}

template <typename T, int MT, int NT, int NWN, int BN, int NTHREADS>
__device__ __forceinline__ void nt_epilogue_slab(const LinArgs& p, f32x4 (&acc)[MT][NT], char* lds, int wm, int wn, int li, int lg, int tid,
                                                 int m0, int n0) {
    static_assert(sizeof(T) == 2, "bf16 path");
    constexpr int CW = 4 * NT, WN = BN / NWN, RPW = MT * 16, GPP = 128 / RPW, PITCH = BN * 4 + 16, CPR = BN / 8;
    constexpr int PER = 128 * CPR / NTHREADS;
    static_assert(128 % RPW == 0 && (128 * CPR) % NTHREADS == 0, "slab geometry");
    T* __restrict__ yg = reinterpret_cast<T*>(p.y);
#pragma unroll
    for (int pass = 0; pass < 2; ++pass) {
        asm volatile("s_waitcnt lgkmcnt(0)" ::: "memory");
        __builtin_amdgcn_s_barrier();
        if (wm / GPP == pass) {
#pragma unroll
            for (int a = 0; a < MT; ++a)
#pragma unroll
                for (int b = 0; b < NT; ++b)
                    *reinterpret_cast<f32x4*>(lds + ((wm % GPP) * RPW + a * 16 + li) * PITCH + (wn * WN + chan_of<CW>(b, lg, 0)) * 4) = acc[a][b];
        }
        asm volatile("s_waitcnt lgkmcnt(0)" ::: "memory");
        __builtin_amdgcn_s_barrier();
#pragma unroll
        for (int i = 0; i < PER; ++i) {
            const int q = i * NTHREADS + tid, r = q / CPR, cc = q - r * CPR;
            const int m = m0 + pass * 128 + r, n = n0 + cc * 8;
            if (m < p.M) {
                const f32x4 lo = *reinterpret_cast<const f32x4*>(lds + r * PITCH + cc * 32);
                const f32x4 hi = *reinterpret_cast<const f32x4*>(lds + r * PITCH + cc * 32 + 16);
                float v[8];
#pragma unroll
                for (int e = 0; e < 4; ++e) { v[e] = lo[e]; v[4 + e] = hi[e]; }
                if (p.bias) {
                    const f32x4 b0 = *reinterpret_cast<const f32x4*>(p.bias + n), b1 = *reinterpret_cast<const f32x4*>(p.bias + n + 4);
#pragma unroll
                    for (int e = 0; e < 4; ++e) { v[e] += b0[e]; v[4 + e] += b1[e]; }
                }
                Vec<T> t;
#pragma unroll
                for (int e = 0; e < 8; ++e) t.set(e, v[e]);
                stvec<T>(yg + (size_t)m * p.ldy + n, t);
            }
        }
    }
}

template <typename T>
__device__ __forceinline__ void nt_epilogue_wslab(const LinArgs& p, f32x4 (&acc)[4][4], char* wslab, int lane, int li, int lg, int mbase, int nbase) {
    static_assert(sizeof(T) == 2, "bf16 path");
    constexpr int PITCH = 64 * 4 + 16;
    T* __restrict__ yg = reinterpret_cast<T*>(p.y);
    T* __restrict__ ypre = reinterpret_cast<T*>(p.y_pre);
    const T* __restrict__ auxg = reinterpret_cast<const T*>(p.aux);
    const T* __restrict__ resg = reinterpret_cast<const T*>(p.res);
#pragma unroll
    for (int a = 0; a < 4; ++a) {
#pragma unroll
        for (int b = 0; b < 4; ++b) *reinterpret_cast<f32x4*>(wslab + li * PITCH + chan_of<16>(b, lg, 0) * 4) = acc[a][b];
#pragma unroll
        for (int i = 0; i < 2; ++i) {
            const int q = i * 64 + lane, r = q >> 3, cc = q & 7;
            const int m = mbase + a * 16 + r, n = nbase + cc * 8;
            const f32x4 lo = *reinterpret_cast<const f32x4*>(wslab + r * PITCH + cc * 32);
            const f32x4 hi = *reinterpret_cast<const f32x4*>(wslab + r * PITCH + cc * 32 + 16);
            if (m < p.M) {
                float v[8];
#pragma unroll
                for (int e = 0; e < 4; ++e) { v[e] = lo[e]; v[4 + e] = hi[e]; }
                if (p.bias) {
                    const f32x4 b0 = *reinterpret_cast<const f32x4*>(p.bias + n), b1 = *reinterpret_cast<const f32x4*>(p.bias + n + 4);
#pragma unroll
                    for (int e = 0; e < 4; ++e) { v[e] += b0[e]; v[4 + e] += b1[e]; }
                }
                const float rs = row_scale(p.rowscale, m, p.rows_per_scale);
                auto put = [&](T* base, int ld) {
                    Vec<T> t;
#pragma unroll
                    for (int e = 0; e < 8; ++e) t.set(e, v[e]);
                    stvec<T>(base + (size_t)m * ld + n, t);
                };
// ... 38 lines not shown
```

facialmmt_amd/csrc/gemm_ph3.h:

```cpp
#pragma once
#include <type_traits>
#include "gemm_common.h"

namespace {

template <int OFF> __device__ __forceinline__ void q3_rd(bf16x8& dst, unsigned addr) {
    asm volatile("ds_read_b128 %0, %1 offset:%2" : "=v"(dst) : "v"(addr), "n"(OFF) : "memory");
}

template <int NE> __device__ __forceinline__ void q3_gelu(float (&v)[NE]) {
#pragma unroll
    for (int j = 0; j < NE; ++j) v[j] = gelu_exp_f(v[j]);
}
template <int NE> __device__ __forceinline__ void q3_gelu_grad_mul(float (&v)[NE], const float (&pre)[NE]) {
#pragma unroll
    for (int j = 0; j < NE; ++j) v[j] *= gelu_grad_exp_f(pre[j]);
}

template <int EPI = 2, bool STAGGER = true, int WT = 2>
__global__ __launch_bounds__(512) void linear_nt_ph3_kernel(LinArgs p) {
    const int p_M = p.M, p_K = p.K, p_ldx = p.ldx, p_ldw = p.ldw, p_ldy = p.ldy, p_ldaux = p.ldaux, p_ldres = p.ldres, p_tiles_m = p.tiles_m, p_tiles_n = p.tiles_n,
              p_rows_per_scale = p.rows_per_scale;
    const void* const p_x = p.x; const void* const p_w = p.w; const void* const p_aux = p.aux; const void* const p_res = p.res;
    void* const p_y = p.y; void* const p_y_pre = p.y_pre;
    const float* const p_bias = p.bias; const float* const p_rowscale = p.rowscale;
    static_assert(WT == 2 || WT == 4, "wave layout");
    constexpr int BM = WT * 96, BN = (8 / WT) * 64;
    constexpr int WP = BN / 64, XP = BM / 64;
    constexpr int XOFF = BN * 128, XB = BM * 128;
    constexpr int BUF = XOFF + XB;
    extern __shared__ __attribute__((aligned(16))) char smem[];
    typedef __attribute__((address_space(1))) const void gptr_t;
    typedef __attribute__((address_space(3))) void lptr_t;

    const int tid = threadIdx.x, lane = tid & 63;
    const int wave = __builtin_amdgcn_readfirstlane(tid >> 6);
    const int wm = WT == 2 ? wave >> 2 : wave >> 1, wn = WT == 2 ? wave & 3 : wave & 1;
    const int grp = wave >> 2;
    const int li = lane & 15, lg = lane >> 4;
    const char* __restrict__ xg = reinterpret_cast<const char*>(p_x);
    const char* __restrict__ wg = reinterpret_cast<const char*>(p_w);
    const int nk = p_K >> 6;
    const unsigned lds0 = (unsigned)(uintptr_t)(lptr_t*)smem;

    const int G = gridDim.x;
    const int total = p_tiles_m * p_tiles_n;
    const int first = ((int)blockIdx.x & 7) * (G >> 3) + ((int)blockIdx.x >> 3);
    const int ntile = first < total ? (total - first + G - 1) / G : 0;
    const int nsteps = ntile * nk;
    if (nsteps == 0) return;

    const int r8 = lane >> 3, cp = lane & 7;
    unsigned xo[XP], wo[WP];
    int st_tile = first, st_k = 0, st_step = 0;
    auto tile_offsets = [&](int t) __attribute__((always_inline)) {
        const int m0 = (t / p_tiles_n) * BM, n0 = (t % p_tiles_n) * BN;
#pragma unroll
        for (int i = 0; i < XP; ++i) {
            const int r = (XP * wave + i) * 8 + r8;
            xo[i] = (unsigned)min(m0 + r, p_M - 1) * (unsigned)p_ldx * 2u + (unsigned)((cp ^ ((r >> 1) & 7)) << 4);
        }
#pragma unroll
        for (int i = 0; i < WP; ++i) {
            const int r = (WP * wave + i) * 8 + r8;
            const int q = r & 63;
            const int ch = (r & ~63) + chan_of<16>(q >> 4, (q >> 2) & 3, q & 3);
            wo[i] = (unsigned)(n0 + ch) * (unsigned)p_ldw * 2u + (unsigned)((cp ^ ((r >> 1) & 7)) << 4);
        }
    };
    auto stage_x = [&](int buf) __attribute__((always_inline)) {
        const unsigned kb = (unsigned)st_k * 128u;
        char* dst = smem + buf * BUF + XOFF + (XP * wave) * 1024;
#pragma unroll
        for (int i = 0; i < XP; ++i) __builtin_amdgcn_global_load_lds((gptr_t*)(xg + (size_t)(xo[i] + kb)), (lptr_t*)(dst + i * 1024), 16, 0, 0);
    };
    auto stage_w = [&](int buf) __attribute__((always_inline)) {
        const unsigned kb = (unsigned)st_k * 128u;
        char* dst = smem + buf * BUF + (WP * wave) * 1024;
#pragma unroll
        for (int i = 0; i < WP; ++i) __builtin_amdgcn_global_load_lds((gptr_t*)(wg + (size_t)(wo[i] + kb)), (lptr_t*)(dst + i * 1024), 16, 0, 0);
    };
    auto advance = [&]() __attribute__((always_inline)) {
        if (st_step + 1 >= nsteps) return;
        ++st_step;
        if (++st_k == nk) {
            st_k = 0;
            st_tile += G;
            tile_offsets(st_tile);
        }
    };

    const unsigned sw0 = (unsigned)(((0 + lg) ^ ((li >> 1) & 7)) << 4), sw1 = (unsigned)(((4 + lg) ^ ((li >> 1) & 7)) << 4);
    const unsigned xrow = (unsigned)(wm * 96 + li) * 128u, wrow = (unsigned)(wn * 64 + li) * 128u;
    const unsigned xa0 = lds0 + XOFF + xrow + sw0, xa1 = lds0 + XOFF + xrow + sw1;
    const unsigned wa0 = lds0 + wrow + sw0, wa1 = lds0 + wrow + sw1;

    f32x4 acc[6][4];
    bf16x8 cf[4][2], tfa[2][2], tfb[4][2];

    auto landed = [&]() __attribute__((always_inline)) { asm volatile("s_waitcnt lgkmcnt(0)" ::: "memory"); };
    auto bar = [&]() __attribute__((always_inline)) {
        __builtin_amdgcn_sched_barrier(0);
        __builtin_amdgcn_s_barrier();
        __builtin_amdgcn_sched_barrier(0);
    };
// ... 297 lines not shown
```

facialmmt_amd/csrc/layernorm.hip:

```cpp
#include "fmmt_common.h"
#include "../../include/fmmt.h"

namespace {

constexpr int LN_BWD_MAX_BLOCKS = 1024;

struct LnArgs {
    int M, C;
    const void* x;
    const float* gamma;
    const float* beta;
    float eps;
    void* y;
    float* mean;
    float* rstd;
    int merge_hw;
    const void* dy;
    const void* add;
    void* dx;
    float* part;
};

template <bool MERGE>
__device__ __forceinline__ size_t src_offset(int row, int ch, int C, int hw) {
    if constexpr (!MERGE) {
        return (size_t)row * C + ch;
    } else {
        const int Cq = C >> 2, hh = hw >> 1;
        const int q = ch / Cq, cc = ch - q * Cq;
        const int n = row / (hh * hh), rem = row - n * hh * hh;
        const int h2 = rem / hh, w2 = rem - h2 * hh;
        const size_t tok = (size_t)n * hw * hw + (size_t)(2 * h2 + (q & 1)) * hw + 2 * w2 + (q >> 1);
        return tok * Cq + cc;
    }
}

template <int G> __device__ __forceinline__ float group_sum(float v) {
    if constexpr (G == 16) return group16_sum(v);
    else return wave_sum(v);
}

template <typename T, int G, int NCH, bool MERGE>
__global__ __launch_bounds__(256) void ln_fwd_kernel(LnArgs p) {
    constexpr int VEC = Vec<T>::N;
    constexpr int ROWS = 256 / G;
    const int sub = threadIdx.x % G, rib = threadIdx.x / G;
    const int chunks = p.C / VEC;
    const T* __restrict__ xg = reinterpret_cast<const T*>(p.x);
    T* __restrict__ yg = reinterpret_cast<T*>(p.y);
    const float invC = 1.0f / (float)p.C;
    for (int row = blockIdx.x * ROWS + rib; row < p.M; row += gridDim.x * ROWS) {
        Vec<T> v[NCH];
        float s = 0.f;
#pragma unroll
        for (int i = 0; i < NCH; ++i) {
            const int c = sub + i * G;
            if (c < chunks) {
                v[i] = ldvec<T>(xg + src_offset<MERGE>(row, c * VEC, p.C, p.merge_hw));
#pragma unroll
                for (int e = 0; e < VEC; ++e) s += v[i].get(e);
            }
        }
        const float mean = group_sum<G>(s) * invC;
        float q = 0.f;
#pragma unroll
        for (int i = 0; i < NCH; ++i) {
            const int c = sub + i * G;
            if (c < chunks) {
#pragma unroll
                for (int e = 0; e < VEC; ++e) {
                    const float d = v[i].get(e) - mean;
                    q += d * d;
                }
            }
        }
        const float rstd = rsqrtf(group_sum<G>(q) * invC + p.eps);
#pragma unroll
        for (int i = 0; i < NCH; ++i) {
            const int c = sub + i * G;
            if (c < chunks) {
                Vec<T> o;
#pragma unroll
                for (int e = 0; e < VEC; ++e) {
                    const int ch = c * VEC + e;
                    o.set(e, (v[i].get(e) - mean) * rstd * p.gamma[ch] + p.beta[ch]);
                }
                stvec<T>(yg + (size_t)row * p.C + c * VEC, o);
            }
        }
        if (sub == 0) {
            if (p.mean) p.mean[row] = mean;
            if (p.rstd) p.rstd[row] = rstd;
        }
    }
}

template <typename T, int G, int NCH, bool MERGE>
__global__ __launch_bounds__(256) void ln_bwd_kernel(LnArgs p) {
    constexpr int VEC = Vec<T>::N;
    constexpr int ROWS = 256 / G;
    __shared__ float red[2][ROWS][G * VEC];
    const int sub = threadIdx.x % G, rib = threadIdx.x / G;
    const int chunks = p.C / VEC;
    const T* __restrict__ xg = reinterpret_cast<const T*>(p.x);
    const T* __restrict__ dyg = reinterpret_cast<const T*>(p.dy);
    const T* __restrict__ addg = reinterpret_cast<const T*>(p.add);
    T* __restrict__ dxg = reinterpret_cast<T*>(p.dx);
    const float invC = 1.0f / (float)p.C;

    float dg[NCH][VEC], db[NCH][VEC];
#pragma unroll
    for (int i = 0; i < NCH; ++i)
#pragma unroll
        for (int e = 0; e < VEC; ++e) dg[i][e] = db[i][e] = 0.f;

    for (int row = blockIdx.x * ROWS + rib; row < p.M; row += gridDim.x * ROWS) {
        const float mean = p.mean[row], rstd = p.rstd[row];
        constexpr bool EARLY_ADD = MERGE || NCH >= 3;
        Vec<T> xv[NCH], gv[NCH], avp[EARLY_ADD ? NCH : 1];
        float s1 = 0.f, s2 = 0.f;
        if constexpr (EARLY_ADD) {
#pragma unroll
            for (int i = 0; i < NCH; ++i) {
                const int c = sub + i * G;
                if (c < chunks) {
                    const size_t off = src_offset<MERGE>(row, c * VEC, p.C, p.merge_hw);
                    xv[i] = ldvec<T>(xg + off);
                    gv[i] = ldvec<T>(dyg + (size_t)row * p.C + c * VEC);
                    if (addg) avp[i] = ldvec<T>(addg + off);
                }
            }
        }
#pragma unroll
        for (int i = 0; i < NCH; ++i) {
            const int c = sub + i * G;
            if (c < chunks) {
                if constexpr (!EARLY_ADD) {
                    xv[i] = ldvec<T>(xg + src_offset<MERGE>(row, c * VEC, p.C, p.merge_hw));
                    gv[i] = ldvec<T>(dyg + (size_t)row * p.C + c * VEC);
                }
#pragma unroll
                for (int e = 0; e < VEC; ++e) {
                    const float xh = (xv[i].get(e) - mean) * rstd;
                    const float dyv = gv[i].get(e);
                    const float g = dyv * p.gamma[c * VEC + e];
                    s1 += g;
                    s2 += g * xh;
                    dg[i][e] += dyv * xh;
                    db[i][e] += dyv;
                }
            }
        }
        s1 = group_sum<G>(s1) * invC;
        s2 = group_sum<G>(s2) * invC;
#pragma unroll
        for (int i = 0; i < NCH; ++i) {
            const int c = sub + i * G;
            if (c < chunks) {
                const size_t off = src_offset<MERGE>(row, c * VEC, p.C, p.merge_hw);
                Vec<T> o, av;
                if constexpr (EARLY_ADD) {
                    if (addg) av = avp[i];
                } else {
                    if (addg) av = ldvec<T>(addg + off);
                }
#pragma unroll
                for (int e = 0; e < VEC; ++e) {
                    const float xh = (xv[i].get(e) - mean) * rstd;
                    const float g = gv[i].get(e) * p.gamma[c * VEC + e];
                    float d = rstd * (g - s1 - xh * s2);
                    if (addg) d += av.get(e);
                    o.set(e, d);
                }
                stvec<T>(dxg + off, o);
            }
        }
    }

    float* part = p.part + (size_t)blockIdx.x * 2 * p.C;
#pragma unroll
    for (int i = 0; i < NCH; ++i) {
        __syncthreads();
#pragma unroll
        for (int e = 0; e < VEC; ++e) {
            red[0][rib][sub * VEC + e] = dg[i][e];
            red[1][rib][sub * VEC + e] = db[i][e];
        }
        __syncthreads();
        for (int t = threadIdx.x; t < 2 * G * VEC; t += 256) {
            const int which = t / (G * VEC), col = t % (G * VEC);
            const int ch = i * G * VEC + col;
            if (ch < p.C) {
                float a = 0.f;
#pragma unroll
                for (int r = 0; r < ROWS; ++r) a += red[which][r][col];
                part[which * p.C + ch] = a;
            }
        }
    }
}

__global__ __launch_bounds__(1024) void ln_reduce_kernel(const float* __restrict__ part, int nblocks, int C, float* dgamma, float* dbeta) {
    __shared__ float red[64][17];
    const int tx = threadIdx.x & 15, ty = threadIdx.x >> 4;
    const int i = blockIdx.x * 16 + tx;
    float a = 0.f;
    if (i < 2 * C)
        for (int b = ty; b < nblocks; b += 64) a += part[(size_t)b * 2 * C + i];
    red[ty][tx] = a;
    __syncthreads();
    if (ty < 16) {
        float t = (red[ty][tx] + red[ty + 16][tx]) + (red[ty + 32][tx] + red[ty + 48][tx]);
        red[ty][tx] = t;
    }
    __syncthreads();
    if (ty == 0 && i < 2 * C) {
        a = 0.f;
#pragma unroll
        for (int g = 0; g < 16; ++g) a += red[g][tx];
        if (i < C) { if (dgamma) dgamma[i] = a; }
        else { if (dbeta) dbeta[i - C] = a; }
    }
}

template <typename T, bool MERGE, bool BWD>
int launch_ln(const LnArgs& a, int g, int nch, int grid, hipStream_t st) {
#define FMMT_LN_CASE(GG, N)                                                                                  \
    if (g == GG && nch == N) {                                                                               \
        if constexpr (BWD) hipLaunchKernelGGL((ln_bwd_kernel<T, GG, N, MERGE>), dim3(grid), dim3(256), 0, st, a); \
        else hipLaunchKernelGGL((ln_fwd_kernel<T, GG, N, MERGE>), dim3(grid), dim3(256), 0, st, a);          \
        FMMT_CHECK_LAUNCH();                                                                                 \
        return 0;                                                                                            \
    }
    FMMT_LN_CASE(16, 1)
    FMMT_LN_CASE(16, 2)
    FMMT_LN_CASE(16, 3)
    FMMT_LN_CASE(64, 2)
    FMMT_LN_CASE(64, 3)
    FMMT_LN_CASE(64, 6)
#undef FMMT_LN_CASE
    return FMMT_EINVAL;
}

bool pick_shape(int C, int vec, int* g, int* nch) {
    const int chunks = C / vec;
    if (chunks <= 48) {
        *g = 16;
        *nch = (chunks + 15) / 16;
        return true;
    }
    *g = 64;
    const int need = (chunks + 63) / 64;
    *nch = need <= 2 ? 2 : need <= 3 ? 3 : need <= 6 ? 6 : -1;
    return *nch > 0;
}

int check_ln(int dtype, int M, int C, int merge_hw) {
    if (dtype != FMMT_BF16 && dtype != FMMT_F32) return FMMT_EINVAL;
    const int vec = dtype == FMMT_BF16 ? 8 : 4;
    if (M <= 0 || C <= 0 || C % vec) return FMMT_EINVAL;
    if (merge_hw) {
        if (merge_hw % 2 || C % 4 || (C / 4) % vec) return FMMT_EINVAL;
        if (M % ((merge_hw / 2) * (merge_hw / 2))) return FMMT_EINVAL;
    }
    int g, nch;
    return pick_shape(C, vec, &g, &nch) ? 0 : FMMT_EINVAL;
}

}

extern "C" int fmmt_layernorm_fwd(int dtype, int M, int C, const void* x, const float* gamma, const float* beta,
                                  float eps, void* y, float* mean, float* rstd, int merge_hw, void* stream) {
    if (int e = check_ln(dtype, M, C, merge_hw)) return e;
    LnArgs a{};
    a.M = M; a.C = C; a.x = x; a.gamma = gamma; a.beta = beta; a.eps = eps; a.y = y; a.mean = mean; a.rstd = rstd;
    a.merge_hw = merge_hw;
    hipStream_t st = reinterpret_cast<hipStream_t>(stream);
    const int vec = dtype == FMMT_BF16 ? 8 : 4;
    int g, nch;
    pick_shape(C, vec, &g, &nch);
    const int rows = 256 / g;
    int grid = (M + rows - 1) / rows;
    if (grid > 8192) grid = 8192;
    if (dtype == FMMT_BF16) return merge_hw ? launch_ln<bf16, true, false>(a, g, nch, grid, st) : launch_ln<bf16, false, false>(a, g, nch, grid, st);
    return merge_hw ? launch_ln<float, true, false>(a, g, nch, grid, st) : launch_ln<float, false, false>(a, g, nch, grid, st);
}

extern "C" size_t fmmt_layernorm_bwd_workspace(int C) { return (size_t)LN_BWD_MAX_BLOCKS * 2 * (size_t)C * sizeof(float); }

extern "C" int fmmt_layernorm_bwd(int dtype, int M, int C, const void* dy, const void* x, const float* mean,
                                  const float* rstd, const float* gamma, const void* add, void* dx,
                                  float* dgamma, float* dbeta, int merge_hw,
                                  void* workspace, size_t workspace_bytes, void* stream) {
    if (int e = check_ln(dtype, M, C, merge_hw)) return e;
    if (workspace_bytes < fmmt_layernorm_bwd_workspace(C)) return FMMT_EWORKSPACE;
    LnArgs a{};
    a.M = M; a.C = C; a.x = x; a.gamma = gamma; a.mean = const_cast<float*>(mean); a.rstd = const_cast<float*>(rstd);
    a.merge_hw = merge_hw; a.dy = dy; a.add = add; a.dx = dx; a.part = reinterpret_cast<float*>(workspace);
    hipStream_t st = reinterpret_cast<hipStream_t>(stream);
    const int vec = dtype == FMMT_BF16 ? 8 : 4;
    int g, nch;
    pick_shape(C, vec, &g, &nch);
    const int rows = 256 / g;
    int grid = (M + rows - 1) / rows;
    if (grid > LN_BWD_MAX_BLOCKS) grid = LN_BWD_MAX_BLOCKS;
    int rc;
    if (dtype == FMMT_BF16) rc = merge_hw ? launch_ln<bf16, true, true>(a, g, nch, grid, st) : launch_ln<bf16, false, true>(a, g, nch, grid, st);
    else rc = merge_hw ? launch_ln<float, true, true>(a, g, nch, grid, st) : launch_ln<float, false, true>(a, g, nch, grid, st);
    if (rc) return rc;
    hipLaunchKernelGGL(ln_reduce_kernel, dim3((2 * C + 15) / 16), dim3(1024), 0, st, a.part, grid, C, dgamma, dbeta);
    FMMT_CHECK_LAUNCH();
    return 0;
}
```

facialmmt_amd/modules/SwinTransformer/Swin_Transformer.py:

```python
from __future__ import annotations

import torch
import torch.nn as nn

from ... import ops


def to_2tuple(v):
    return tuple(v) if isinstance(v, (tuple, list)) else (v, v)


def _require(cond: bool, msg: str):
    if not cond:
        raise NotImplementedError("facialmmt_amd HIP path: " + msg)


DROP_PATH_ONE_DRAW = True


class DropPath(nn.Module):

    def __init__(self, drop_prob: float = 0.0):
        super().__init__()
        self.drop_prob = float(drop_prob)
        self._rows = None

    def sample_scale(self, n: int, device):
        if self.drop_prob == 0.0 or not self.training:
            return None
        if self._rows:
            row = self._rows.pop(0)
            if row.shape[0] == n and row.device == torch.device(device):
                return row
        keep = 1.0 - self.drop_prob
        return torch.empty(n, dtype=torch.float32, device=device).bernoulli_(keep).div_(keep)

    def forward(self, x):
        s = self.sample_scale(x.shape[0], x.device)
        return x if s is None else x * s.to(x.dtype).view(-1, *([1] * (x.dim() - 1)))

    def extra_repr(self):
        return f"drop_prob={self.drop_prob}"


class Flatten(nn.Module):
    def forward(self, input):
        return input.view(input.size(0), -1)


class Mlp(nn.Module):

    def __init__(self, in_features, hidden_features=None, out_features=None, act_layer=nn.GELU, drop=0.):
        super().__init__()
        out_features = out_features or in_features
        hidden_features = hidden_features or in_features
        _require(act_layer is nn.GELU, "Mlp activation must be nn.GELU (erf form)")
        self.fc1 = nn.Linear(in_features, hidden_features)
        self.act = act_layer()
        self.fc2 = nn.Linear(hidden_features, out_features)
        self.drop = nn.Dropout(drop)

    def forward(self, x, res=None, rowscale=None, rows_per_scale=1):
        _require(self.drop.p == 0.0 or not self.training, "Mlp dropout p > 0 in training")
        return ops.mlp(x, self.fc1.weight, self.fc1.bias, self.fc2.weight, self.fc2.bias, res, rowscale, rows_per_scale)


class WindowAttention(nn.Module):

    def __init__(self, dim, window_size, num_heads, qkv_bias=True, qk_scale=None, attn_drop=0., proj_drop=0.):
        super().__init__()
        self.dim = dim
        self.window_size = window_size
        self.num_heads = num_heads
        head_dim = dim // num_heads
        self.scale = qk_scale or head_dim ** -0.5
        ws_h, ws_w = window_size
        self.relative_position_bias_table = nn.Parameter(torch.zeros((2 * ws_h - 1) * (2 * ws_w - 1), num_heads))
        t = torch.arange(ws_h * ws_w)
        ti, tj = t // ws_w, t % ws_w
        rel = (ti[:, None] - ti[None, :] + ws_h - 1) * (2 * ws_w - 1) + (tj[:, None] - tj[None, :] + ws_w - 1)
        self.register_buffer("relative_position_index", rel)
        self.qkv = nn.Linear(dim, dim * 3, bias=qkv_bias)
        self.attn_drop = nn.Dropout(attn_drop)
        self.proj = nn.Linear(dim, dim)
        self.proj_drop = nn.Dropout(proj_drop)
        nn.init.trunc_normal_(self.relative_position_bias_table, std=.02)
        self.softmax = nn.Softmax(dim=-1)
        self._index_i32 = None

    def _index(self, device):
        if self._index_i32 is None or self._index_i32.device != device:
            self._index_i32 = self.relative_position_index.to(device=device, dtype=torch.int32).contiguous()
        return self._index_i32

    def _check(self):
        _require(tuple(self.window_size) == (7, 7), "window_size must be 7 (kernel constant)")
        _require(self.dim // self.num_heads == 32, "head_dim must be 32")
        _require(not self.training or (self.attn_drop.p == 0.0 and self.proj_drop.p == 0.0),
                 "attention / projection dropout p > 0 in training")

    def forward_tokens(self, x, n_img, H, W, shift, mask, res=None, rowscale=None, mask_is_shift=False):
        self._check()
        qkv = ops.linear(x, self.qkv.weight, self.qkv.bias)
        o = ops.window_attn_core(qkv.view(-1, 3 * self.dim), self.relative_position_bias_table, self._index(x.device),
                                 mask, n_img, H, W, self.num_heads, shift, float(self.scale), mask_is_shift)
        return ops.linear(o.view(n_img, H * W, self.dim), self.proj.weight, self.proj.bias, res, rowscale, H * W)

    def forward(self, x, mask=None):
        B_, N, C = x.shape
        assert N == self.window_size[0] * self.window_size[1] and C == self.dim, "input feature has wrong size"
        return self.forward_tokens(x, B_, self.window_size[0], self.window_size[1], 0, mask)

    def extra_repr(self) -> str:
        return f'dim={self.dim}, window_size={self.window_size}, num_heads={self.num_heads}'

    def flops(self, N):
        return N * self.dim * 3 * self.dim + 2 * self.num_heads * N * (self.dim // self.num_heads) * N + N * self.dim * self.dim


def build_shift_mask(H, W, window_size, shift_size):
    def region(n):
        r = torch.zeros(n, dtype=torch.long)
        r[n - window_size:n - shift_size] = 1
        r[n - shift_size:] = 2
        return r
    rid = region(H)[:, None] * 3 + region(W)[None, :]
    ids = rid.view(H // window_size, window_size, W // window_size, window_size).permute(0, 2, 1, 3).reshape(-1, window_size * window_size)
    same = ids[:, None, :] == ids[:, :, None]
    return torch.where(same, torch.tensor(0.0), torch.tensor(-100.0))


class SwinTransformerBlock(nn.Module):

    def __init__(self, dim, input_resolution, num_heads, window_size=7, shift_size=0,
                 mlp_ratio=4., qkv_bias=True, qk_scale=None, drop=0., attn_drop=0., drop_path=0.,
                 act_layer=nn.GELU, norm_layer=nn.LayerNorm):
        super().__init__()
        self.dim = dim
        self.input_resolution = input_resolution
        self.num_heads = num_heads
        self.window_size = window_size
        self.shift_size = shift_size
        self.mlp_ratio = mlp_ratio
        if min(self.input_resolution) <= self.window_size:
            self.shift_size = 0
            self.window_size = min(self.input_resolution)
        assert 0 <= self.shift_size < self.window_size, "shift_size must in 0-window_size"
        _require(norm_layer is nn.LayerNorm, "norm_layer must be nn.LayerNorm")
        self.norm1 = norm_layer(dim)
        self.attn = WindowAttention(dim, window_size=to_2tuple(self.window_size), num_heads=num_heads,
                                    qkv_bias=qkv_bias, qk_scale=qk_scale, attn_drop=attn_drop, proj_drop=drop)
        self.drop_path = DropPath(drop_path) if drop_path > 0. else nn.Identity()
        self.norm2 = norm_layer(dim)
        self.mlp = Mlp(in_features=dim, hidden_features=int(dim * mlp_ratio), act_layer=act_layer, drop=drop)
        attn_mask = None
        if self.shift_size > 0:
            H, W = self.input_resolution
            attn_mask = build_shift_mask(H, W, self.window_size, self.shift_size)
        self.register_buffer("attn_mask", attn_mask)
        self._mask_checked = None

    def _mask_is_standard(self) -> bool:
        m = self.attn_mask
        if m is None:
            return False
        key = (m.data_ptr(), m._version)
        if self._mask_checked is None or self._mask_checked[0] != key:
            H, W = self.input_resolution
            ok = bool(torch.equal(m.detach().float().cpu(), build_shift_mask(H, W, self.window_size, self.shift_size)))
            self._mask_checked = (key, ok)
        return self._mask_checked[1]

    def _scale(self, n, device):
        return self.drop_path.sample_scale(n, device) if isinstance(self.drop_path, DropPath) else None

    def forward(self, x):
        H, W = self.input_resolution
        B, L, C = x.shape
        assert L == H * W, "input feature has wrong size"
        a = self.attn
        std = self._mask_is_standard()
        if ops.window_block_fusable(x, C, a.num_heads, a.window_size, self.shift_size, self.attn_mask, std):
            a._check()
            x = ops.window_block(x, self.norm1.weight, self.norm1.bias, self.norm1.eps, a.qkv.weight, a.qkv.bias, a.proj.weight, a.proj.bias,
                                 a.relative_position_bias_table, a._index(x.device), self.attn_mask, B, H, W, a.num_heads, self.shift_size,
                                 float(a.scale), self._scale(B, x.device))
        else:
            x, xn = ops.residual_layer_norm(x, self.norm1.weight, self.norm1.bias, self.norm1.eps)
            x = a.forward_tokens(xn, B, H, W, self.shift_size, self.attn_mask, res=x, rowscale=self._scale(B, x.device), mask_is_shift=std)
        mlp = self.mlp
        if ops.mlp_ln_fusable(x, mlp.fc1.weight, mlp.fc2.weight, mlp.fc1.bias, mlp.fc2.bias) and (mlp.drop.p == 0.0 or not self.training):
            return ops.mlp_ln(x, self.norm2.weight, self.norm2.bias, self.norm2.eps, mlp.fc1.weight, mlp.fc1.bias, mlp.fc2.weight, mlp.fc2.bias,
                              self._scale(B, x.device), L)
        x, xn = ops.residual_layer_norm(x, self.norm2.weight, self.norm2.bias, self.norm2.eps)
        return mlp(xn, res=x, rowscale=self._scale(B, x.device), rows_per_scale=L)

    def extra_repr(self) -> str:
        return (f"dim={self.dim}, input_resolution={self.input_resolution}, num_heads={self.num_heads}, "
                f"window_size={self.window_size}, shift_size={self.shift_size}, mlp_ratio={self.mlp_ratio}")

    def flops(self):
        H, W = self.input_resolution
        nW = H * W / self.window_size / self.window_size
        return 2 * self.dim * H * W + nW * self.attn.flops(self.window_size * self.window_size) + 2 * H * W * self.dim * self.dim * self.mlp_ratio


class PatchMerging(nn.Module):

    def __init__(self, input_resolution, dim, norm_layer=nn.LayerNorm):
        super().__init__()
        self.input_resolution = input_resolution
        self.dim = dim
        self.reduction = nn.Linear(4 * dim, 2 * dim, bias=False)
        self.norm = norm_layer(4 * dim)

    def forward(self, x):
        H, W = self.input_resolution
        B, L, C = x.shape
        assert L == H * W, "input feature has wrong size"
        assert H % 2 == 0 and W % 2 == 0, f"x size ({H}*{W}) are not even."
        _require(H == W, "square token grid")
        xn = ops.layer_norm(x, self.norm.weight, self.norm.bias, self.norm.eps, merge_hw=H)
        return ops.linear(xn, self.reduction.weight)

    def extra_repr(self) -> str:
        return f"input_resolution={self.input_resolution}, dim={self.dim}"

    def flops(self):
        H, W = self.input_resolution
        return H * W * self.dim + (H // 2) * (W // 2) * 4 * self.dim * 2 * self.dim


class BasicLayer(nn.Module):

    def __init__(self, dim, input_resolution, depth, num_heads, window_size, mlp_ratio=4., qkv_bias=True,
                 qk_scale=None, drop=0., attn_drop=0., drop_path=0., norm_layer=nn.LayerNorm, downsample=None,
                 use_checkpoint=False):
        super().__init__()
        self.dim = dim
        self.input_resolution = input_resolution
        self.depth = depth
        self.use_checkpoint = use_checkpoint
        _require(not use_checkpoint, "activation checkpointing (288 GB of HBM: activations are kept)")
        self.blocks = nn.ModuleList([
            SwinTransformerBlock(dim=dim, input_resolution=input_resolution, num_heads=num_heads,
                                 window_size=window_size, shift_size=0 if (i % 2 == 0) else window_size // 2,
                                 mlp_ratio=mlp_ratio, qkv_bias=qkv_bias, qk_scale=qk_scale, drop=drop,
                                 attn_drop=attn_drop,
                                 drop_path=drop_path[i] if isinstance(drop_path, list) else drop_path,
                                 norm_layer=norm_layer)
            for i in range(depth)])
        self.downsample = downsample(input_resolution, dim=dim, norm_layer=norm_layer) if downsample is not None else None

    def forward(self, x):
        for blk in self.blocks:
            x = blk(x)
        if self.downsample is not None:
            x = self.downsample(x)
        return x

    def extra_repr(self) -> str:
        return f"dim={self.dim}, input_resolution={self.input_resolution}, depth={self.depth}"

    def flops(self):
        return sum(b.flops() for b in self.blocks) + (self.downsample.flops() if self.downsample is not None else 0)


class PatchEmbed(nn.Module):

    def __init__(self, img_size=224, patch_size=4, in_chans=3, embed_dim=96, norm_layer=None):
        super().__init__()
        img_size = to_2tuple(img_size)
        patch_size = to_2tuple(patch_size)
        self.img_size = img_size
        self.patch_size = patch_size
        self.patches_resolution = [img_size[0] // patch_size[0], img_size[1] // patch_size[1]]
        self.num_patches = self.patches_resolution[0] * self.patches_resolution[1]
        self.in_chans = in_chans
        self.embed_dim = embed_dim
        self.proj = nn.Conv2d(in_chans, embed_dim, kernel_size=patch_size, stride=patch_size)
        self.norm = norm_layer(embed_dim) if norm_layer is not None else None

    def forward_u8(self, x, resize="pil", dtype=None):
        _require(tuple(self.img_size) == (224, 224) and tuple(self.patch_size) == (4, 4) and self.in_chans == 3,
                 "PatchEmbed kernel is built for 3x224x224 images and 4x4 patches")
        B = x.shape[0]
        w2d = self.proj.weight.view(self.embed_dim, -1)
        dt = dtype or self.proj.weight.dtype
        if ops.patch_embed_u8_ln_fusable(x, w2d, self.norm, dt):
            return ops.patch_embed_u8_ln(x, resize, w2d, self.proj.bias, self.norm.weight, self.norm.bias, self.norm.eps, dt).view(B, self.num_patches, self.embed_dim)
        cols = ops.patch_embed_u8(x, resize, dt)
        if ops.patch_proj_ln_fusable(cols, w2d, self.norm):
            return ops.patch_proj_ln(cols, w2d, self.proj.bias, self.norm.weight, self.norm.bias, self.norm.eps).view(B, self.num_patches, self.embed_dim)
        y = ops.linear(cols, w2d, self.proj.bias).view(B, self.num_patches, self.embed_dim)
        if self.norm is not None:
            y = ops.layer_norm(y, self.norm.weight, self.norm.bias, self.norm.eps)
        return y

    def forward(self, x):
        B, C, H, W = x.shape
        assert H == self.img_size[0] and W == self.img_size[1], \
            f"Input image size ({H}*{W}) doesn't match model ({self.img_size[0]}*{self.img_size[1]})."
        _require(tuple(self.img_size) == (224, 224) and tuple(self.patch_size) == (4, 4) and C == 3,
                 "PatchEmbed kernel is built for 3x224x224 images and 4x4 patches")
        cols = ops.patch_im2col(x)
        w2d = self.proj.weight.view(self.embed_dim, -1)
        if ops.patch_proj_ln_fusable(cols, w2d, self.norm):
            return ops.patch_proj_ln(cols, w2d, self.proj.bias, self.norm.weight, self.norm.bias, self.norm.eps).view(B, self.num_patches, self.embed_dim)
        y = ops.linear(cols, w2d, self.proj.bias).view(B, self.num_patches, self.embed_dim)
        if self.norm is not None:
            y = ops.layer_norm(y, self.norm.weight, self.norm.bias, self.norm.eps)
        return y

    def flops(self):
        Ho, Wo = self.patches_resolution
        f = Ho * Wo * self.embed_dim * self.in_chans * (self.patch_size[0] * self.patch_size[1])
        return f + (Ho * Wo * self.embed_dim if self.norm is not None else 0)


class SwinTransformer(nn.Module):

    def __init__(self, img_size=224, patch_size=4, in_chans=3, embed_dim=96, depths=[2, 2, 6, 2],
                 num_heads=[3, 6, 12, 24], window_size=7, mlp_ratio=4., qkv_bias=True, qk_scale=None,
                 drop_rate=0., attn_drop_rate=0., drop_path_rate=0.1, norm_layer=nn.LayerNorm, ape=False,
                 patch_norm=True, use_checkpoint=False, **kwargs):
        super().__init__()
        self.num_layers = len(depths)
        self.embed_dim = embed_dim
        self.ape = ape
        self.patch_norm = patch_norm
        self.num_features = int(embed_dim * 2 ** (self.num_layers - 1))
        self.mlp_ratio = mlp_ratio
        _require(not ape, "absolute position embedding (ape=True)")
        self.patch_embed = PatchEmbed(img_size=img_size, patch_size=patch_size, in_chans=in_chans, embed_dim=embed_dim,
                                      norm_layer=norm_layer if self.patch_norm else None)
        self.patches_resolution = self.patch_embed.patches_resolution
        self.pos_drop = nn.Dropout(p=drop_rate)
        dpr = [v.item() for v in torch.linspace(0, drop_path_rate, sum(depths))]
        self.layers = nn.ModuleList()
        for i in range(self.num_layers):
            self.layers.append(BasicLayer(
                dim=int(embed_dim * 2 ** i),
                input_resolution=(self.patches_resolution[0] // (2 ** i), self.patches_resolution[1] // (2 ** i)),
                depth=depths[i], num_heads=num_heads[i], window_size=window_size, mlp_ratio=self.mlp_ratio,
                qkv_bias=qkv_bias, qk_scale=qk_scale, drop=drop_rate, attn_drop=attn_drop_rate,
                drop_path=dpr[sum(depths[:i]):sum(depths[:i + 1])], norm_layer=norm_layer,
                downsample=PatchMerging if (i < self.num_layers - 1) else None, use_checkpoint=use_checkpoint))
        self.output_layer = nn.Sequential(norm_layer(self.num_features), Flatten(), nn.Linear(49 * 768, 512), nn.BatchNorm1d(512))
        self.apply(self._init_weights)
        keep = [1.0 - blk.drop_path.drop_prob for layer in self.layers for blk in layer.blocks
                if isinstance(blk.drop_path, DropPath) and blk.drop_path.drop_prob > 0.0 for _ in range(2)]
        self.register_buffer("_dp_keep", torch.tensor(keep, dtype=torch.float32).view(-1, 1), persistent=False)
        self.register_buffer("_dp_inv", (1.0 / torch.tensor(keep, dtype=torch.float64)).float().view(-1, 1), persistent=False)

    def _draw_drop_paths(self, n, device):
        dps = [blk.drop_path for layer in self.layers for blk in layer.blocks if isinstance(blk.drop_path, DropPath) and blk.drop_path.drop_prob > 0.0]
        for dp in dps:
            dp._rows = None
        if not DROP_PATH_ONE_DRAW or not self.training or not dps or self._dp_keep.numel() != 2 * len(dps) or self._dp_keep.device != torch.device(device):
            return
        keep = self._dp_keep
        pool = torch.where(torch.rand(keep.shape[0], n, dtype=torch.float32, device=device) < keep, self._dp_inv, 0.0)
        for i, dp in enumerate(dps):
            dp._rows = [pool[2 * i], pool[2 * i + 1]]

    def _init_weights(self, m):
        if isinstance(m, nn.Linear):
            nn.init.trunc_normal_(m.weight, std=.02)
            if m.bias is not None:
                nn.init.constant_(m.bias, 0)
        elif isinstance(m, nn.LayerNorm):
            nn.init.constant_(m.bias, 0)
            nn.init.constant_(m.weight, 1.0)

    @torch.jit.ignore
    def no_weight_decay(self):
        return {'absolute_pos_embed'}

    @torch.jit.ignore
    def no_weight_decay_keywords(self):
        return {'relative_position_bias_table'}

    def _head(self, x, n_valid=None):
        ln, _, fc, bn = self.output_layer
        x = ops.layer_norm(x, ln.weight, ln.bias, ln.eps)
        x = ops.linear(x.reshape(x.shape[0], -1), fc.weight, fc.bias)
        use_batch = self.training or not bn.track_running_stats
        if self.training and bn.track_running_stats:
            bn.num_batches_tracked += 1
        return ops.batch_norm_1d(x, bn.weight, bn.bias, bn.running_mean, bn.running_var, bn.momentum, bn.eps, use_batch, n_valid=n_valid)

    input_resize = "pil"
    input_dtype = None

    def forward_features(self, x, n_valid=None):
        _require(self.pos_drop.p == 0.0 or not self.training, "pos_drop p > 0 in training")
        if x.dtype == torch.uint8:
            x = self.patch_embed.forward_u8(x, self.input_resize, self.input_dtype)
        else:
            x = self.patch_embed(x)
        self._draw_drop_paths(x.shape[0], x.device)
        for layer in self.layers:
            x = layer(x)
        return self._head(x, n_valid)

    def forward(self, x, n_valid=None):
        if n_valid is not None:
            return self.forward_features(x, n_valid)
        if len(x) == 1:
            return self.forward_features(torch.cat((x, x), dim=0))[:1]
        return self.forward_features(x)
```

facialmmt_amd/ops.py:

```python
from __future__ import annotations

import math
import weakref

import torch
from torch.autograd import Function

from . import _lib
from ._lib import EPI_GELU, EPI_GELU_BWD, EPI_GELU_DG, EPI_MUL_AUX, EPI_NONE, SAVE_DG, check, dtype_code


def _st():
    return torch.cuda.current_stream().cuda_stream


def _p(t):
    return None if t is None else t.data_ptr()


def _c16(t: torch.Tensor) -> torch.Tensor:
    t = t.contiguous()
    return t.clone() if t.data_ptr() % 16 else t


def _need_cuda(t: torch.Tensor, what: str):
    if not t.is_cuda:
        raise _lib.FmmtError(f"{what}: the hot path runs on the GPU only (got a {t.device} tensor); "
                             f"the CPU restatement lives in oracle/ and is test infrastructure")


def _ws(nbytes: int, device) -> torch.Tensor:
    return torch.empty(max(int(nbytes), 16), dtype=torch.uint8, device=device)


def linear_raw(x2, w, bias, *, epi=EPI_NONE, y_pre=None, aux=None, res=None, rowscale=None, rows_per_scale=1):
    M, K = x2.shape
    N = w.shape[0]
    y = torch.empty((M, N), dtype=x2.dtype, device=x2.device)
    lib = _lib.load()
    if epi == EPI_NONE and res is None and rowscale is None and K >= 4096:
        nbytes = lib.fmmt_linear_splitk_workspace(M, N, K)
        if nbytes:
            ws = _ws(nbytes, x2.device)
            rc = lib.fmmt_linear_fwd_splitk(dtype_code(x2.dtype), M, N, K, _p(x2), K, _p(w), K, _p(bias), _p(y), N,
                                            _p(ws), nbytes, _st())
            check(rc, f"fmmt_linear_fwd_splitk(M={M},N={N},K={K})")
            return y
    rc = lib.fmmt_linear_fwd(dtype_code(x2.dtype), M, N, K, _p(x2), K, _p(w), K, _p(bias), _p(y), N, _p(y_pre),
                             epi, _p(aux), N, _p(res), N, _p(rowscale), rows_per_scale, _st())
    check(rc, f"fmmt_linear_fwd(M={M},N={N},K={K})")
    return y


def wgrad_partials_raw(dy2, x2, want_bias, ws, nbytes, rowscale=None, rows_per_scale=1, x_gelu=False):
    M, N = dy2.shape
    K = x2.shape[1]
    rc = _lib.load().fmmt_linear_wgrad_partials(dtype_code(dy2.dtype), M, N, K, _p(dy2), N, _p(x2), K, 1 if want_bias else 0,
                                                _p(rowscale), rows_per_scale, EPI_GELU if x_gelu else EPI_NONE, _p(ws), nbytes, _st())
    check(rc, f"fmmt_linear_wgrad_partials(M={M},N={N},K={K})")


def wgrad_raw(dy2, x2, want_bias, rowscale=None, rows_per_scale=1, x_gelu=False, out=None):
    M, N = dy2.shape
    K = x2.shape[1]
    lib = _lib.load()
    if out is not None:
        dw, db = out
        assert dw.shape == (N, K) and dw.dtype == torch.float32 and dw.is_contiguous() and (not want_bias or (db.shape == (N,) and db.is_contiguous()))
    else:
        dw = torch.empty((N, K), dtype=torch.float32, device=dy2.device)
        db = torch.empty((N,), dtype=torch.float32, device=dy2.device) if want_bias else None
    nbytes = lib.fmmt_linear_wgrad_workspace(dtype_code(dy2.dtype), M, N, K)
    ws = _ws(nbytes, dy2.device)
    if M <= 2048:
        rc = lib.fmmt_linear_wgrad(dtype_code(dy2.dtype), M, N, K, _p(dy2), N, _p(x2), K, _p(dw), _p(db), _p(rowscale), rows_per_scale,
                                   EPI_GELU if x_gelu else EPI_NONE, _p(ws), nbytes, _st())
        check(rc, f"fmmt_linear_wgrad(M={M},N={N},K={K})")
        return dw, db
    wgrad_partials_raw(dy2, x2, want_bias, ws, nbytes, rowscale, rows_per_scale, x_gelu)
    rc = lib.fmmt_linear_wgrad_finish(dtype_code(dy2.dtype), M, N, K, _p(dw), _p(db), _p(ws), nbytes, _st())
    check(rc, f"fmmt_linear_wgrad_finish(M={M},N={N},K={K})")
    return dw, db


_CAST_CACHE: dict = {}


def _lp(w: torch.Tensor, dtype, transpose: bool = False) -> torch.Tensor:
    base = w._base if w._base is not None else w
    wd = w.detach()
    if wd.dtype == dtype and not transpose:
        return wd.contiguous()
    capturing = wd.is_cuda and torch.cuda.is_current_stream_capturing()
    key = (w.storage_offset(), tuple(w.shape), tuple(w.stride()), dtype, transpose)
    if capturing and _PIN_SCOPE:
        pin = _PINNED.get(id(base))
        if pin is not None and key in pin:
            return pin[key]
    sub = None if capturing else _CAST_CACHE.get(id(base))
    if sub is not None:
        hit = sub.get(key)
        if hit is not None and hit[0] == w._version:
            return hit[1]
    out = wd.to(dtype)
    out = out.t().contiguous() if transpose else out.contiguous()
    if capturing:
        return out
    if sub is None:
        sub = _CAST_CACHE[id(base)] = {}
        weakref.finalize(base, _CAST_CACHE.pop, id(base), None)
    sub[key] = (w._version, out)
    return out


_PINNED: dict = {}
_PIN_SCOPE: list = []


class pinned_scope:

    def __init__(self, shadows):
        self.shadows = shadows

    def __enter__(self):
        if self.shadows is not None:
            _PIN_SCOPE.append(self.shadows)
        return self

    def __exit__(self, *exc):
        if self.shadows is not None:
            _PIN_SCOPE.remove(self.shadows)
        return False


class PinnedShadows:

    def __init__(self, params):
        import numpy as np
        recs, self.keep = [], []
        tiles = 0
        for p in params:
            sub = _CAST_CACHE.get(id(p))
            if not sub or not p.is_cuda or p.dtype not in (torch.float32, torch.bfloat16):
                continue
            pins = _PINNED.setdefault(id(p), {})
            if not pins:
                weakref.finalize(p, _PINNED.pop, id(p), None)
            for key, (_, shadow) in sub.items():
                off, shape, stride, dtype, transpose = key
                if dtype != torch.bfloat16 or len(shape) != 2 or stride[1] != 1:
                    continue
                rows, cols = shape
                dst = pins.get(key)
                if dst is None:
                    dst = pins[key] = torch.empty_like(shadow)
                self.keep.append((p, dst))
                tr, tc = (rows + 63) // 64, (cols + 63) // 64
                recs.append((p.untyped_storage().data_ptr() + off * p.element_size(), dst.data_ptr(), rows, cols, stride[0],
                             (1 if transpose else 0) | (2 if p.dtype == torch.float32 else 0), tiles, tc))
                tiles += tr * tc
        self.n, self.tiles = len(recs), tiles
        self.desc = None
# ... 465 lines not shown
                                            _p(rowscale), rows_per_scale, _p(dh), _p(dx), _st())
        check(rc, f"fmmt_mlp_bwd_input(M={M},C={C})")
        return dh, dx
    dh = linear_raw(dy2, _lp(w2, dt, transpose=True), None, epi=EPI_MUL_AUX if dg else EPI_GELU_BWD, aux=h_pre, rowscale=rowscale, rows_per_scale=rows_per_scale)
    return dh, linear_raw(dh, _lp(w1, dt, transpose=True), None)


class MlpLnFn(Function):

    @staticmethod
    def forward(ctx, x, ln_w, ln_b, eps, w1, b1, w2, b2, rowscale, rows_per_scale, grad_on=True):
        _need_cuda(x, "mlp_ln")
        C = x.shape[-1]
        x2 = x.reshape(-1, C).contiguous()
        M = x2.shape[0]
        train = grad_on and any(ctx.needs_input_grad)
        dev = x.device
        g, b = ln_w.detach().float().contiguous(), ln_b.detach().float().contiguous()
        y = torch.empty_like(x2)
        xn = torch.empty_like(x2) if train else None
        mean = torch.empty(M, dtype=torch.float32, device=dev) if train else None
        rstd = torch.empty(M, dtype=torch.float32, device=dev) if train else None
        h_pre = torch.empty((M, 4 * C), dtype=x.dtype, device=dev) if train else None
        h = torch.empty_like(h_pre) if train else None
        ctx.dg = bool(train and _MLP_SAVE_DG and C in _MLP_FUSED_DG_WIDTHS)
        w1l, w2l, b1f, b2f = _lp(w1, x.dtype), _lp(w2, x.dtype), b1.detach().float().contiguous(), b2.detach().float().contiguous()
        rc = _lib.load().fmmt_mlp_ln_fwd(dtype_code(x.dtype) | (SAVE_DG if ctx.dg else 0), M, C, _p(x2), _p(g), _p(b), float(eps), _p(w1l), _p(b1f),
                                         _p(w2l), _p(b2f), _p(rowscale), rows_per_scale, _p(y), _p(xn), _p(mean), _p(rstd),
                                         _p(h_pre), _p(h), _st())
        check(rc, f"fmmt_mlp_ln_fwd(M={M},C={C})")
        ctx.save_for_backward(x2, xn, mean, rstd, g, w1, w2, h_pre, h, rowscale)
        ctx.rps = rows_per_scale
        ctx.xshape = x.shape
        return y.reshape(x.shape)

    @staticmethod
    def backward(ctx, dy):
        x2, xn, mean, rstd, g, w1, w2, h_pre, h, rowscale = ctx.saved_tensors
        C = x2.shape[1]
        lib = _lib.load()
        dy2 = dy.reshape(-1, C).contiguous()
        M, dt = x2.shape[0], x2.dtype
        if _MLP_BWD_FUSED and _MLP_BWD_LN and _mlp_dtype_ok(dt) and C in _MLP_BWD_WIDTHS and M >= 4096:
            dh = torch.empty((M, 4 * C), dtype=dt, device=x2.device)
            dx = torch.empty_like(x2)
            dg = torch.empty(C, dtype=torch.float32, device=x2.device)
            db = torch.empty(C, dtype=torch.float32, device=x2.device)
            nbytes = lib.fmmt_mlp_ln_bwd_input_workspace(C)
            ws = _ws(nbytes, x2.device)
            w2t, w1t = _lp(w2, dt, transpose=True), _lp(w1, dt, transpose=True)
            rc = lib.fmmt_mlp_ln_bwd_input(dtype_code(dt) | (SAVE_DG if ctx.dg else 0), M, C, _p(dy2), _p(h_pre), _p(w2t), _p(w1t),
                                           _p(rowscale), ctx.rps, _p(x2), _p(mean), _p(rstd), _p(g), _p(dh), _p(dx), _p(dg), _p(db), _p(ws), nbytes, _st())
            check(rc, f"fmmt_mlp_ln_bwd_input(M={M},C={C})")
            dw2, db2 = wgrad_raw(dy2, h, True, rowscale, ctx.rps)
            dw1, db1 = wgrad_raw(dh, xn, True)
            return dx.reshape(ctx.xshape), dg, db, None, dw1, db1, dw2, db2, None, None, None
        dh, dxn = mlp_bwd_input_raw(dy2, h_pre, w1, w2, rowscale, ctx.rps, ctx.dg)
        dw2, db2 = wgrad_raw(dy2, h, True, rowscale, ctx.rps)
        dw1, db1 = wgrad_raw(dh, xn, True)
        del dh
        dx = torch.empty_like(x2)
        dg = torch.empty(C, dtype=torch.float32, device=x2.device)
        db = torch.empty(C, dtype=torch.float32, device=x2.device)
        nbytes = lib.fmmt_layernorm_bwd_workspace(C)
        ws = _ws(nbytes, x2.device)
        rc = lib.fmmt_layernorm_bwd(dtype_code(x2.dtype), x2.shape[0], C, _p(dxn), _p(x2), _p(mean), _p(rstd), _p(g), _p(dy2), _p(dx), _p(dg), _p(db), 0,
                                    _p(ws), nbytes, _st())
        check(rc, "fmmt_layernorm_bwd(mlp_ln)")
        return dx.reshape(ctx.xshape), dg, db, None, dw1, db1, dw2, db2, None, None, None


def mlp_ln_fusable(x, w1, w2, b1, b2):
    C = x.shape[-1]
    return (_MLP_FUSED and x.is_cuda and _mlp_dtype_ok(x.dtype) and C in _MLP_FUSED_WIDTHS and w1.shape == (4 * C, C) and w2.shape == (C, 4 * C)
            and b1 is not None and b2 is not None and x.numel() // C >= 4096)


def mlp_ln(x, ln_w, ln_b, eps, w1, b1, w2, b2, rowscale=None, rows_per_scale=1):
    return MlpLnFn.apply(x, ln_w, ln_b, eps, w1, b1, w2, b2, rowscale, rows_per_scale, torch.is_grad_enabled())


def mlp(x, w1, b1, w2, b2, res=None, rowscale=None, rows_per_scale=1):
    return MlpFn.apply(x, w1, b1, w2, b2, res, rowscale, rows_per_scale, torch.is_grad_enabled())


class LayerNormFn(Function):
    @staticmethod
    def forward(ctx, x, gamma, beta, eps, merge_hw):
        _need_cuda(x, "layer_norm")
        lib = _lib.load()
        x = x.contiguous()
        if merge_hw:
            n, L, Cq = x.shape
            assert L == merge_hw * merge_hw
            M, C = n * (merge_hw // 2) ** 2, 4 * Cq
            out_shape = (n, (merge_hw // 2) ** 2, C)
        else:
            C = x.shape[-1]
            M = x.numel() // C
            out_shape = x.shape
        y = torch.empty(out_shape, dtype=x.dtype, device=x.device)
        mean = torch.empty(M, dtype=torch.float32, device=x.device)
        rstd = torch.empty(M, dtype=torch.float32, device=x.device)
        g, b = gamma.detach().float().contiguous(), beta.detach().float().contiguous()
        rc = lib.fmmt_layernorm_fwd(dtype_code(x.dtype), M, C, _p(x), _p(g), _p(b), eps, _p(y), _p(mean), _p(rstd),
                                    merge_hw, _st())
        check(rc, f"fmmt_layernorm_fwd(M={M},C={C},merge={merge_hw})")
        ctx.save_for_backward(x, mean, rstd, g)
        ctx.dims = (M, C, merge_hw)
        return y

    @staticmethod
    def backward(ctx, dy):
        x, mean, rstd, g = ctx.saved_tensors
        M, C, merge_hw = ctx.dims
        lib = _lib.load()
        dy = dy.contiguous()
        dx = torch.empty_like(x)
        dg = torch.empty(C, dtype=torch.float32, device=x.device)
        db = torch.empty(C, dtype=torch.float32, device=x.device)
        nbytes = lib.fmmt_layernorm_bwd_workspace(C)
        ws = _ws(nbytes, x.device)
        rc = lib.fmmt_layernorm_bwd(dtype_code(x.dtype), M, C, _p(dy), _p(x), _p(mean), _p(rstd), _p(g), None, _p(dx),
                                    _p(dg), _p(db), merge_hw, _p(ws), nbytes, _st())
        check(rc, f"fmmt_layernorm_bwd(M={M},C={C},merge={merge_hw})")
        return dx, dg, db, None, None


def layer_norm(x, gamma, beta, eps=1e-5, merge_hw=0):
    return LayerNormFn.apply(x, gamma, beta, eps, merge_hw)


_PATCH_LN = True


class PatchProjLnFn(Function):

    @staticmethod
    def forward(ctx, cols, weight, bias, gamma, beta, eps, grad_on=True):
        _need_cuda(cols, "patch_proj_ln")
        M, K = cols.shape
        C = weight.shape[0]
        train = grad_on and any(ctx.needs_input_grad)
        dev, dt = cols.device, cols.dtype
        g, b = gamma.detach().float().contiguous(), beta.detach().float().contiguous()
        y = torch.empty((M, C), dtype=dt, device=dev)
        x_pre = torch.empty_like(y) if train else None
        mean = torch.empty(M, dtype=torch.float32, device=dev) if train else None
        rstd = torch.empty(M, dtype=torch.float32, device=dev) if train else None
        rc = _lib.load().fmmt_patch_embed_ln_fwd(dtype_code(dt), M, C, K, _p(cols), _p(_lp(weight, dt)), _p(bias.detach().float().contiguous() if bias is not None else None),
                                                 _p(g), _p(b), float(eps), _p(x_pre), _p(y), _p(mean), _p(rstd), _st())
        check(rc, f"fmmt_patch_embed_ln_fwd(M={M})")
        ctx.save_for_backward(cols, weight, x_pre, mean, rstd, g)
        ctx.has_bias = bias is not None
        return y

    @staticmethod
    def backward(ctx, dy):
        cols, weight, x_pre, mean, rstd, g = ctx.saved_tensors
        M, C = x_pre.shape
        lib = _lib.load()
        dy = dy.contiguous()
        dxp = torch.empty_like(x_pre)
        dg = torch.empty(C, dtype=torch.float32, device=dy.device)
        db = torch.empty(C, dtype=torch.float32, device=dy.device)
        nbytes = lib.fmmt_layernorm_bwd_workspace(C)
# ... 988 lines not shown
```

include/fmmt.h:

```cpp
#ifndef FMMT_H
#define FMMT_H
#include <stddef.h>
#include <stdint.h>

#ifdef __cplusplus
extern "C" {
#endif

#define FMMT_F32 0
#define FMMT_BF16 1
#define FMMT_GENERIC 0x100
#define FMMT_SAVE_DG 0x200
#define FMMT_BATCH_MAJOR 0x400

#define FMMT_EINVAL (-1)
#define FMMT_EALIGN (-2)
#define FMMT_EWORKSPACE (-3)

#define FMMT_EPI_GELU 1
#define FMMT_EPI_GELU_BWD 2
#define FMMT_EPI_GELU_DG 3
#define FMMT_EPI_MUL_AUX 4

int fmmt_version(void);
// ... 98 lines not shown
                 const float* lse, void* dq, int lddq, void* dk, void* dv, int lddkv, void* stream);

int fmmt_mha_avg_weights(int dtype, int Lq, int Lk, int B, int E, int num_heads, const void* q, int ldq, const void* k, int ldkv,
                         float scale, const float* key_bias, float dropout_p, uint64_t seed, const uint64_t* seed_dev,
                         const float* lse, float* weights, void* stream);

int fmmt_patch_im2col(int dtype, int n_img, const void* img, void* cols, void* stream);
int fmmt_patch_col2im(int dtype, int n_img, const void* cols, void* dimg, void* stream);

int fmmt_batchnorm1d_fwd(int dtype, int n, int C, const void* x, const float* gamma, const float* beta,
                         float* running_mean, float* running_var, float momentum, float eps,
                         int training, void* y, float* save_mean, float* save_invstd, void* stream);
int fmmt_batchnorm1d_bwd(int dtype, int n, int C, const void* dy, const void* x, const float* gamma,
                         const float* save_mean, const float* save_invstd, int training,
                         void* dx, float* dgamma, float* dbeta, void* stream);

int fmmt_posemb_scale_fwd(int dtype, int L, int B, int E, const void* x, const float* table,
                          float scale, void* y, void* stream);

int fmmt_scale(int dtype, size_t n, const void* x, float alpha, void* y, void* stream);

int fmmt_colsum(int dtype, int out_dtype, int M, int N, const void* x, int ldx, void* out, void* stream);

size_t fmmt_layernorm_bwd_bf16_workspace(int M, int C);
int fmmt_layernorm_bwd_bf16(int M, int C, float eps, const void* dy, const void* x, const void* gamma, void* dx,
                            void* dgamma, void* dbeta, void* workspace, size_t workspace_bytes, void* stream);

int fmmt_plm_dropadd_ln_fwd(int M, int C, float eps, const void* h, const void* res, const void* gamma, const void* beta, float p,
                            uint64_t seed, const uint64_t* seed_dev, uint64_t salt, void* xsum, void* y, void* stream);
size_t fmmt_plm_dropadd_ln_bwd_workspace(int M, int C);
int fmmt_plm_dropadd_ln_bwd(int M, int C, float eps, const void* dy, const void* xsum, const void* gamma, float p, uint64_t seed,
                            const uint64_t* seed_dev, uint64_t salt, void* dx, void* dh, void* dgamma, void* dbeta, void* dbias, void* workspace,
                            size_t workspace_bytes, void* stream);

size_t fmmt_plm_gelu_bwd_colsum_workspace(int M, int H);
int fmmt_plm_gelu_bwd_colsum(int M, int H, const void* dact, const void* pre, void* dpre, void* dbias, void* workspace, size_t workspace_bytes, void* stream);

int fmmt_embedding_bwd(int T, int C, int V, const int64_t* ids, int64_t padding_idx, const void* dy, void* dweight, void* stream);

int fmmt_dropadd_ln_fwd(int param_dtype, int M, int C, float eps, const void* h, const void* res, const void* gamma, const void* beta, float p,
                        uint64_t seed, const uint64_t* seed_dev, uint64_t salt, void* xsum, void* y, void* stream);
size_t fmmt_dropadd_ln_bwd_workspace(int M, int C);
int fmmt_dropadd_ln_bwd(int param_dtype, int M, int C, float eps, const void* dy, const void* xsum, const void* gamma, float p, uint64_t seed,
                        const uint64_t* seed_dev, uint64_t salt, void* dx, void* dh, void* dgamma, void* dbeta, void* dbias, void* workspace,
                        size_t workspace_bytes, void* stream);

int fmmt_select_frames_fwd(int dtype, int nF, int NL, int B, int Lv, int D, const float* preds, const void* vision_inputs,
                           const float* vision_mask, const int64_t* num_imgs, float threshold, void* out, float* new_mask,
                           int32_t* src_face, void* stream);
int fmmt_select_frames_bwd(int dtype, int nF, int NL, int B, int Lv, int D, const void* dout, const int32_t* src_face, float* dpreds,
                           void* stream);

int fmmt_cast_batch(int n_desc, int n_tiles, const void* desc, void* stream);

int fmmt_grad_handover(int n_desc, int n_blocks, const void* desc, float* partial, float* norm_out, void* stream);

int fmmt_adamw_batch(int n_desc, int n_blocks, const void* desc, const float* lr, const float* step, const float* total_norm,
                     float beta1, float beta2, float eps, float weight_decay, float max_norm, int hf_semantics, void* stream);

#define FMMT_RESIZE_PIL 0
#define FMMT_RESIZE_CV2 1
int fmmt_resize_table(int mode, int in_size, int out_size, int32_t* table, float* lut);
int fmmt_resize_band_rows(const int32_t* table, int out_size);
int fmmt_patch_embed_u8(int dtype, int mode, int n_img, int in_size, const void* img_u8, const int32_t* table_dev,
                        const float* lut_dev, void* cols, void* stream);

int fmmt_patch_embed_ln_fwd(int dtype, int M, int C, int K, const void* cols, const void* w, const float* bias, const float* ln_gamma,
                            const float* ln_beta, float eps, void* x_pre, void* y, float* mean, float* rstd, void* stream);

int fmmt_patch_embed_u8_ln_fwd(int dtype, int mode, int n_img, int in_size, const void* img_u8, const int32_t* table_dev, const float* lut_dev,
                               const void* w, const float* bias, const float* ln_gamma, const float* ln_beta, float eps,
                               void* cols, void* x_pre, void* y, float* mean, float* rstd, void* stream);

int fmmt_emotion_head_fwd(int dtype, int N, int K, int H, int NL, const void* feats, int ld, const float* w1, const float* b1, const float* w2,
                          const float* b2, const float* gumbel, float tau, float* preds, float* importance, void* stream);
int fmmt_eval_accumulate(int dtype, int B, int NL, const void* logits, int ld, const int64_t* labels, double* loss_sum, int64_t* count,
                         int64_t* confusion, int32_t* pred, float* logits_out, int64_t out_offset, int64_t out_capacity, void* stream);

#include "fmmt_pool_head.h"
#include "fmmt_ragged.h"
#include "fmmt_eval_collect.h"
#include "fmmt_pool_head_rows.h"
#include "fmmt_guard.h"

#ifdef __cplusplus
}
#endif
#endif
```

Measured before the change: 74.02 utterances/s.

## Skip MLP compute for drop-path-dropped images via compacted row plans

Adds a device-side drop-path plan that reorders images so kept ones come first, records how many rows to process and a per-row offset back to the original rows. Row-limited variants of the linear forward, weight-gradient partials and layernorm forward/backward kernels read that count on device, so Swin MLP blocks only run GEMMs on rows whose residual branch survives. The residual add scatters through the row offsets and the backward gathers the incoming gradient accordingly. This cuts GEMM work in proportion to the drop-path rate, at the cost of extra plan and gather kernels and new templated kernel variants; it is limited to bf16 shapes that match the expected kernel families.

```diff
diff --git a/facialmmt_amd/_lib.py b/facialmmt_amd/_lib.py
--- a/facialmmt_amd/_lib.py
+++ b/facialmmt_amd/_lib.py
@@ -104,6 +104,17 @@
     "fmmt_guard_commit": (_i, [_p, _p, _p, _p]),
     "fmmt_monitor_loss": (_i, [_p, _f, _p, _p]),
 }
+
+ROWS_SIGNATURES = {
+    "fmmt_droppath_plan": (_i, [_i, _i, _i, _i, _p, _p, _p, _p, _p, _p]),
+    "fmmt_gather_rows": (_i, [_i, _sz, _i, _p, _p, _p, _p, _p]),
+    "fmmt_linear_fwd_rows": (_i, [_i, _i, _i, _i, _p, _i, _p, _i, _p, _p, _i, _p, _i, _p, _i, _p, _i, _p, _i, _p, _p, _p]),
+    "fmmt_linear_fwd_rows_kernel": (_i, [_i, _i, _i, _i, _i, _i, _i, _i, _i, _i, _i]),
+    "fmmt_linear_wgrad_rows_kernel": (_i, [_i, _i, _i, _i, _i]),
+    "fmmt_linear_wgrad_partials_rows": (_i, [_i, _i, _i, _i, _p, _i, _p, _i, _i, _p, _i, _i, _p, _sz, _p, _p]),
+    "fmmt_layernorm_fwd_rows": (_i, [_i, _i, _i, _p, _p, _p, _f, _p, _p, _p, _p, _p, _i, _p, _p]),
+    "fmmt_layernorm_bwd_rows": (_i, [_i, _i, _i, _p, _p, _p, _p, _p, _p, _p, _p, _p, _p, _sz, _p, _p, _i, _p]),
+}
 GUARD_LOSS_SUM, GUARD_MICRO_STEPS, GUARD_NONFINITE_LOSSES, GUARD_APPLIED, GUARD_SKIPPED, GUARD_LAST_NORM, GUARD_WORDS = 0, 1, 2, 3, 4, 5, 6
 
 FMMT_EINVAL, FMMT_EALIGN, FMMT_EWORKSPACE = -1, -2, -3
@@ -125,7 +136,7 @@
         raise FmmtError(f"{LIB_PATH} is missing: build it with `python -m facialmmt_amd.build` "
                         f"(or __graft_entry__.build()); there is no CPU / PyTorch fallback for the hot path")
     lib = C.CDLL(LIB_PATH)
-    for name, (res, args) in list(SIGNATURES.items()) + list(POOL_HEAD_SIGNATURES.items()) + list(RAGGED_SIGNATURES.items()) + list(EVAL_COLLECT_SIGNATURES.items()) + list(POOL_HEAD_ROWS_SIGNATURES.items()) + list(GUARD_SIGNATURES.items()):
+    for name, (res, args) in list(SIGNATURES.items()) + list(POOL_HEAD_SIGNATURES.items()) + list(RAGGED_SIGNATURES.items()) + list(EVAL_COLLECT_SIGNATURES.items()) + list(POOL_HEAD_ROWS_SIGNATURES.items()) + list(GUARD_SIGNATURES.items()) + list(ROWS_SIGNATURES.items()):
         fn = getattr(lib, name)
         fn.restype = res
         fn.argtypes = args
diff --git a/facialmmt_amd/build.py b/facialmmt_amd/build.py
--- a/facialmmt_amd/build.py
+++ b/facialmmt_amd/build.py
@@ -9,7 +9,7 @@
 HERE = os.path.dirname(os.path.abspath(__file__))
 CSRC = os.path.join(HERE, "csrc")
 OUT = os.path.join(HERE, "libfmmt_hip.so")
-SOURCES = ["gemm.hip", "layernorm.hip", "attn.hip", "wattn_mfma.hip", "wattn_bwd_ref.hip", "wblock.hip", "wblock_ref.hip", "mha_mfma.hip", "misc.hip", "preproc.hip", "mlp_fused.hip", "mlp_ref.hip", "patch_ln.hip", "lin_lnbwd.hip", "plm_fused.hip", "frame_filter.hip", "eval.hip", "pool_head.hip", "ragged.hip", "guard.hip"]
+SOURCES = ["gemm.hip", "layernorm.hip", "attn.hip", "wattn_mfma.hip", "wattn_bwd_ref.hip", "wblock.hip", "wblock_ref.hip", "mha_mfma.hip", "misc.hip", "preproc.hip", "mlp_fused.hip", "mlp_ref.hip", "patch_ln.hip", "lin_lnbwd.hip", "plm_fused.hip", "frame_filter.hip", "eval.hip", "pool_head.hip", "ragged.hip", "guard.hip", "rows.hip"]
 FLAGS = ["--offload-arch=gfx950", "-O3", "-std=c++17", "-fPIC", "-ffp-contract=fast"]
 
 
@@ -24,7 +24,7 @@
     hipcc = os.environ.get("HIPCC", "/opt/rocm/bin/hipcc")
     tag = tag or os.environ.get("FMMT_BUILD_TAG", "")
     csrc = os.environ.get("FMMT_CSRC_DIR", CSRC) if tag else CSRC
-    headers = sorted(glob.glob(os.path.join(csrc, "*.h"))) + [os.path.join(csrc, "..", "..", "include", h) for h in ("fmmt.h", "fmmt_pool_head.h", "fmmt_ragged.h", "fmmt_eval_collect.h", "fmmt_pool_head_rows.h", "fmmt_guard.h")]
+    headers = sorted(glob.glob(os.path.join(csrc, "*.h"))) + [os.path.join(csrc, "..", "..", "include", h) for h in ("fmmt.h", "fmmt_pool_head.h", "fmmt_ragged.h", "fmmt_eval_collect.h", "fmmt_pool_head_rows.h", "fmmt_guard.h", "fmmt_rows.h")]
     objdir = os.path.join(HERE, "build_" + tag if tag else "build")
     out = os.path.join(HERE, f"libfmmt_hip_{tag}.so") if tag else OUT
     os.makedirs(objdir, exist_ok=True)
diff --git a/facialmmt_amd/csrc/gemm.hip b/facialmmt_amd/csrc/gemm.hip
--- a/facialmmt_amd/csrc/gemm.hip
+++ b/facialmmt_amd/csrc/gemm.hip
@@ -468,9 +468,13 @@
     }
 }
 
-template <int BN, int BK, int NBUF, bool BATCH = true, bool HASOP = false, bool PIPE = false>
+template <int BN, int BK, int NBUF, bool BATCH = true, bool HASOP = false, bool PIPE = false, bool ROWMAP = false>
 __global__ __launch_bounds__(512) void linear_nt_p256_kernel(LinArgs p) {
     static_assert(BK == 64 && BATCH, "one K step, batched fragment reads");
+    if (p.m_rows) {
+        p.M = min(max(*p.m_rows, 0), p.M);
+        p.tiles_m = (p.M + 255) / 256;
+    }
     using T = bf16;
     constexpr int BM = 256, PITCH = BK, MT = 8, NT = BN / 64, WN = BN / 4, CW = 4 * NT;
     constexpr int RPI = 8;
@@ -650,7 +654,7 @@
         st_prev = 0;
         __builtin_amdgcn_s_barrier();
         if constexpr (HASOP) {
-            if (ck_k == nk - 1) nt_epilogue_prefetch<MT, NT>(p, pre, (ct_k / p.tiles_n) * BM + wm * 128, (ct_k % p.tiles_n) * BN + wn * WN, li, lg);
+            if (ck_k == nk - 1) nt_epilogue_prefetch<MT, NT, ROWMAP>(p, pre, (ct_k / p.tiles_n) * BM + wm * 128, (ct_k % p.tiles_n) * BN + wn * WN, li, lg);
         }
         if constexpr (PIPE) {
             pend = k + NBUF - 1 < nsteps;
@@ -827,7 +831,7 @@
                 for (int pass = 0; pass < 128 / PR; ++pass) round(pass);
                 if (!PIPE && rows_left >= 128) st_prev = (128 / PR) * NSL;
             } else if constexpr (HASOP) {
-                nt_epilogue<T, MT, NT, true, true>(p, acc, m0 + wm * 128, n0 + wn * WN, li, lg, &pre);
+                nt_epilogue<T, MT, NT, true, true, false, ROWMAP>(p, acc, m0 + wm * 128, n0 + wn * WN, li, lg, &pre);
             } else {
                 nt_epilogue<T, MT, NT, true, false, true>(p, acc, m0 + wm * 128, n0 + wn * WN, li, lg);
             }
@@ -842,24 +846,29 @@
     }
 }
 
-template <int BN, int BK, int NBUF, bool BATCH, bool HASOP, bool PIPE = false>
+template <int BN, int BK, int NBUF, bool BATCH, bool HASOP, bool PIPE = false, bool ROWMAP = false>
 int launch_p256_b(const LinArgs& a, hipStream_t st) {
     constexpr size_t lds = (size_t)NBUF * (BN + 256) * BK * 2 + 2 * 256 * sizeof(float) + (BN == 256 ? 8 * 16 * 144 : 2 * (BN == 192 ? 32 : 16) * (BN * 2 + 16));
     static_assert(lds <= 160 * 1024, "LDS");
     static FmmtLdsOnce lds_once;
-    if (int rc_ = lds_once.set(reinterpret_cast<const void*>(&linear_nt_p256_kernel<BN, BK, NBUF, BATCH, HASOP, PIPE>), (int)lds)) return rc_;
+    if (int rc_ = lds_once.set(reinterpret_cast<const void*>(&linear_nt_p256_kernel<BN, BK, NBUF, BATCH, HASOP, PIPE, ROWMAP>), (int)lds)) return rc_;
     LinArgs p = a;
     p.tiles_m = (a.M + 255) / 256;
     p.tiles_n = a.N / BN;
-    hipLaunchKernelGGL((linear_nt_p256_kernel<BN, BK, NBUF, BATCH, HASOP, PIPE>), dim3(256), dim3(512), lds, st, p);
+    hipLaunchKernelGGL((linear_nt_p256_kernel<BN, BK, NBUF, BATCH, HASOP, PIPE, ROWMAP>), dim3(256), dim3(512), lds, st, p);
     FMMT_CHECK_LAUNCH();
     return 0;
 }
 template <int BN, int BK, int NBUF>
 int launch_p256(const LinArgs& a, hipStream_t st) {
     if constexpr (BN != 256) {
+        if (a.row_delta) {
+            if constexpr (BN == 192) return (a.res || a.rowscale) && !a.aux ? launch_p256_b<BN, BK, NBUF, true, true, false, true>(a, st) : FMMT_EINVAL;
+            else return FMMT_EINVAL;
+        }
         if (a.res || a.aux || a.rowscale) return launch_p256_b<BN, BK, NBUF, true, true>(a, st);
     }
+    if (a.row_delta) return FMMT_EINVAL;
     if (a.K >= 384) return launch_p256_b<BN, BK, NBUF, true, false, true>(a, st);
     return launch_p256_b<BN, BK, NBUF, true, false>(a, st);
 }
@@ -1064,6 +1073,7 @@
     int* hdr;
     int splits;
     int npad;
+    const int* m_rows;
 };
 
 __device__ __forceinline__ int tn_swz(int row) { return (row & 3) | (((row >> 3) & 1) << 2); }
@@ -1471,7 +1481,14 @@
     const int split = logical / tiles, tile = logical - split * tiles;
     const int tile_n = tile / p.tiles_k, tile_k = tile % p.tiles_k;
     const int n0 = tile_n * TNn, k0 = tile_k * TKk;
-    const int mbeg = split * p.chunk, mend = min(p.M, mbeg + p.chunk);
+    int rows_m = p.M, chunk = p.chunk;
+    if (p.m_rows) {
+        rows_m = min(max(*p.m_rows, 0), p.M);
+        const int c = ((rows_m + p.splits - 1) / p.splits + 63) / 64 * 64;
+        if (c >= 512 && rows_m < p.M) chunk = c;
+    }
+    int mbeg = split * chunk, mend = min(rows_m, mbeg + chunk);
+    if (mbeg >= mend) mbeg = mend = 0;
     const int NP = p.npad ? p.npad : p.N;
     if (p.hdr && blockIdx.x == 0 && tid == 0) { p.hdr[0] = p.splits; p.hdr[1] = TNn; p.hdr[2] = NP; }
     const T* __restrict__ dyg = reinterpret_cast<const T*>(p.dy);
@@ -2064,3 +2081,89 @@
                                             workspace, workspace_bytes, stream)) return rc;
     return fmmt_linear_wgrad_finish(dtype, M, N, K, dw, db, workspace, workspace_bytes, stream);
 }
+
+namespace {
+int rows_kernel(const LinArgs& a) {
+    if (a.M <= 4096) return 0;
+    int epi3 = 2;
+    if (const int ph = ph_plan(a, &epi3)) return (ph == 3 && epi3 == 6 && !a.row_delta) ? 36 : 0;
+    if (const int bn = p256_plan(a)) {
+        if (bn == 128) return 0;
+        if (a.row_delta && (!(a.res || a.rowscale) || a.aux || bn == 256)) return 0;
+        return bn;
+    }
+    return 0;
+}
+}
+
+extern "C" int fmmt_linear_fwd_rows(int dtype, int M, int N, int K,
+                                    const void* x, int ldx, const void* w, int ldw, const float* bias,
+                                    void* y, int ldy, void* y_pre,
+                                    int epi, const void* aux, int ldaux,
+                                    const void* res, int ldres, const float* rowscale, int rows_per_scale,
+                                    const int* m_rows, const int* row_delta, void* stream) {
+    if (!m_rows) return row_delta ? FMMT_EINVAL : fmmt_linear_fwd(dtype, M, N, K, x, ldx, w, ldw, bias, y, ldy, y_pre, epi, aux, ldaux, res, ldres, rowscale, rows_per_scale, stream);
+    if (dtype != FMMT_BF16 || M <= 0 || N <= 0 || K <= 0) return FMMT_EINVAL;
+    if (K % 8 || N % 4 || ldx % 8 || ldw % 8 || ldy % 4) return FMMT_EINVAL;
+    if (epi < 0 || epi > FMMT_EPI_MUL_AUX) return FMMT_EINVAL;
+    if ((epi == FMMT_EPI_GELU_BWD || epi == FMMT_EPI_MUL_AUX) && (!aux || ldaux % 4)) return FMMT_EINVAL;
+    if (res && ldres % 4) return FMMT_EINVAL;
+    if ((rowscale || row_delta) && rows_per_scale <= 0) return FMMT_EINVAL;
+    if (!aligned16(x) || !aligned16(w) || !aligned16(y) || (bias && !aligned16(bias)) ||
+        (res && !aligned16(res)) || (aux && !aligned16(aux)) || (y_pre && !aligned16(y_pre)))
+        return FMMT_EALIGN;
+    LinArgs a{M, N, K, x, ldx, w, ldw, bias, y, ldy, y_pre, epi, aux, ldaux, res, ldres, rowscale, rows_per_scale, 0, 0, 0, 0, nullptr};
+    a.m_rows = m_rows;
+    a.row_delta = row_delta;
+    hipStream_t st = reinterpret_cast<hipStream_t>(stream);
+    const int kind = rows_kernel(a);
+    if (!kind) return FMMT_EINVAL;
+    if (kind == 36) return launch_ph3<6>(a, st);
+    return kind == 256 ? launch_p256<256, 64, 2>(a, st) : launch_p256<192, 64, 2>(a, st);
+}
+
+extern "C" int fmmt_linear_fwd_rows_kernel(int M, int N, int K, int has_bias, int has_y_pre, int epi, int has_aux, int has_res, int has_rowscale,
+                                           int rows_per_scale, int has_row_delta) {
+    if (M <= 0 || N <= 0 || K <= 0 || K % 8 || N % 8) return 0;
+    static const int one = 0;
+    const void* some = &one;
+    LinArgs a{M, N, K, some, K, some, K, has_bias ? reinterpret_cast<const float*>(some) : nullptr, const_cast<void*>(some), N, has_y_pre ? const_cast<void*>(some) : nullptr,
+              epi, has_aux ? some : nullptr, N, has_res ? some : nullptr, N, has_rowscale ? reinterpret_cast<const float*>(some) : nullptr, rows_per_scale, 0, 0, 0, 0, nullptr};
+    a.m_rows = &one;
+    a.row_delta = has_row_delta ? &one : nullptr;
+    return rows_kernel(a);
+}
+
+extern "C" int fmmt_linear_wgrad_rows_kernel(int M, int N, int K, int has_rowscale, int rows_per_scale) {
+    if (M <= 0 || N <= 0 || K <= 0 || N % 8 || K % 8) return 0;
+    if (tn_few_ok(M, N, K, FMMT_BF16) && !has_rowscale) return 0;
+    const TnPlan pd = tn_plan_dma(M, N, K);
+    if (!pd.tn || pd.tk == 192) return 0;
+    if (has_rowscale && !(rows_per_scale >= 32 && pd.chunk / rows_per_scale + 2 <= 1024)) return 0;
+    return pd.tn;
+}
+
+extern "C" int fmmt_linear_wgrad_rows_kernel(int M, int N, int K, int has_rowscale, int rows_per_scale);
+extern "C" int fmmt_linear_wgrad_partials_rows(int dtype, int M, int N, int K,
+                                               const void* dy, int lddy, const void* x, int ldx, int want_bias,
+                                               const float* rowscale, int rows_per_scale, int x_epi,
+                                               void* workspace, size_t workspace_bytes, const int* m_rows, void* stream) {
+    if (!m_rows) return fmmt_linear_wgrad_partials(dtype, M, N, K, dy, lddy, x, ldx, want_bias, rowscale, rows_per_scale, x_epi, workspace, workspace_bytes, stream);
+    if (dtype != FMMT_BF16 || M <= 0 || N <= 0 || K <= 0 || x_epi) return FMMT_EINVAL;
+    if (N % 8 || K % 8 || lddy % 8 || ldx % 8) return FMMT_EINVAL;
+    if (rowscale && rows_per_scale <= 0) return FMMT_EINVAL;
+    if (!aligned16(dy) || !aligned16(x) || !aligned16(workspace)) return FMMT_EALIGN;
+    if (workspace_bytes < tn_ws_bytes(M, N, K, dtype)) return FMMT_EWORKSPACE;
+    if (!fmmt_linear_wgrad_rows_kernel(M, N, K, rowscale != nullptr, rows_per_scale)) return FMMT_EINVAL;
+    const TnPlan pd = tn_plan_dma(M, N, K);
+    const int smax = tn_smax(M, N, K, dtype);
+    int* hdr = reinterpret_cast<int*>(workspace);
+    float* part_b = reinterpret_cast<float*>(reinterpret_cast<char*>(workspace) + TN_HDR);
+    float* part_w = part_b + (size_t)smax * tn_rows(M, N, K, dtype);
+    TnArgs a{M, N, K, dy, lddy, x, ldx, part_w, want_bias ? part_b : nullptr, rowscale, rows_per_scale, pd.tiles_k, pd.chunk, pd.tiles_n, 0, hdr, pd.splits, pd.npad};
+    a.m_rows = m_rows;
+    const int grid = pd.tiles_n * pd.tiles_k * pd.splits;
+    hipStream_t st = reinterpret_cast<hipStream_t>(stream);
+    if (rowscale) return pd.tk == 256 ? launch_tn_dma<256, 256, 4, 2, true>(a, grid, st) : launch_tn_dma<192, 384, 4, 2, true>(a, grid, st);
+    return pd.tk == 256 ? launch_tn_dma<256, 256, 4, 2>(a, grid, st) : launch_tn_dma<192, 384, 4, 2>(a, grid, st);
+}
diff --git a/facialmmt_amd/csrc/gemm_common.h b/facialmmt_amd/csrc/gemm_common.h
--- a/facialmmt_amd/csrc/gemm_common.h
+++ b/facialmmt_amd/csrc/gemm_common.h
@@ -22,6 +22,8 @@
     const void* w1; const void* w2;
     const float* bias1; const float* bias2;
     int wseg, wseg_mode;
+    const int* m_rows;
+    const int* row_delta;
 };
 
 template <int CW>
@@ -35,8 +37,9 @@
     bf16x8 full[MT][NT / 2 > 0 ? NT / 2 : 1];
     bf16x4 tail[MT];
     float rs[MT];
+    int mrow[MT];
 };
-template <int MT, int NT>
+template <int MT, int NT, bool ROWMAP = false>
 __device__ __forceinline__ void nt_epilogue_prefetch(const LinArgs& p, EpiPre<MT, NT>& pre, int mbase, int nbase, int li, int lg) {
     const bool use_aux = p.epi == FMMT_EPI_GELU_BWD || p.epi == FMMT_EPI_MUL_AUX;
     const bf16* __restrict__ src = reinterpret_cast<const bf16*>(use_aux ? p.aux : p.res);
@@ -45,16 +48,21 @@
     for (int a = 0; a < MT; ++a) {
         const int m = min(mbase + a * 16 + li, p.M - 1);
         pre.rs[a] = row_scale(p.rowscale, m, p.rows_per_scale);
+        int mo = m;
+        if constexpr (ROWMAP) {
+            mo = m + p.row_delta[m / p.rows_per_scale];
+            pre.mrow[a] = mo;
+        }
         if (src) {
 #pragma unroll
             for (int c = 0; c < NT / 2; ++c)
-                pre.full[a][c] = *reinterpret_cast<const bf16x8*>(src + (size_t)m * ld + nbase + chan_of<4 * NT>(2 * c, lg, 0));
-            if constexpr (NT % 2) pre.tail[a] = *reinterpret_cast<const bf16x4*>(src + (size_t)m * ld + nbase + chan_of<4 * NT>(NT - 1, lg, 0));
+                pre.full[a][c] = *reinterpret_cast<const bf16x8*>(src + (size_t)mo * ld + nbase + chan_of<4 * NT>(2 * c, lg, 0));
+            if constexpr (NT % 2) pre.tail[a] = *reinterpret_cast<const bf16x4*>(src + (size_t)mo * ld + nbase + chan_of<4 * NT>(NT - 1, lg, 0));
         }
     }
 }
 
-template <typename T, int MT, int NT, bool BIAS_DONE = false, bool PRE = false, bool NOOPS = false>
+template <typename T, int MT, int NT, bool BIAS_DONE = false, bool PRE = false, bool NOOPS = false, bool ROWMAP = false>
 __device__ __forceinline__ void nt_epilogue(const LinArgs& p, f32x4 (&acc)[MT][NT], int mbase, int nbase, int li, int lg,
                                             const EpiPre<MT, NT>* pre = nullptr) {
     constexpr int VEC = Vec<T>::N;
@@ -85,6 +93,8 @@
             if constexpr (NOOPS) rs = 1.0f;
             else if constexpr (PRE) rs = pre->rs[a];
             else rs = row_scale(p.rowscale, m, p.rows_per_scale);
+            int my = m;
+            if constexpr (PRE && ROWMAP) my = pre->mrow[a];
 #pragma unroll
             for (int b0 = 0; b0 < NT; b0 += TPC) {
                 const int w = (NT - b0 >= TPC) ? VEC : 4;
@@ -122,26 +132,26 @@
                         for (int e = 0; e < 4; ++e) out[e] = to_f32(base[(size_t)m * ld + n + e]);
                     }
                 };
-                auto store_chunk = [&](T* base, int ld, const float* in) {
+                auto store_chunk = [&](T* base, int ld, const float* in, int mr) {
                     if (w == VEC) {
                         Vec<T> t;
 #pragma unroll
                         for (int e = 0; e < VEC; ++e) t.set(e, in[e]);
-                        stvec<T>(base + (size_t)m * ld + n, t);
+                        stvec<T>(base + (size_t)mr * ld + n, t);
                     } else {
                         T o[4];
 #pragma unroll
                         for (int e = 0; e < 4; ++e) o[e] = from_f32<T>(in[e]);
-                        *reinterpret_cast<uint2*>(base + (size_t)m * ld + n) = *reinterpret_cast<const uint2*>(o);
+                        *reinterpret_cast<uint2*>(base + (size_t)mr * ld + n) = *reinterpret_cast<const uint2*>(o);
                     }
                 };
                 if (p.epi == FMMT_EPI_GELU) {
-                    if (ypre) store_chunk(ypre, p.ldy, v);
+                    if (ypre) store_chunk(ypre, p.ldy, v, m);
                     gelu_inplace<T>(v, VEC);
                 } else if (p.epi == FMMT_EPI_GELU_DG) {
                     float d[VEC];
                     gelu_both_inplace<T>(v, d, VEC);
-                    if (ypre) store_chunk(ypre, p.ldy, d);
+                    if (ypre) store_chunk(ypre, p.ldy, d, m);
                 } else if (!NOOPS && p.epi == FMMT_EPI_GELU_BWD) {
                     float ax[VEC];
                     load_chunk(auxg, p.ldaux, ax);
@@ -162,7 +172,7 @@
 #pragma unroll
                     for (int e = 0; e < VEC; ++e) v[e] += (e < w) ? rx[e] : 0.f;
                 }
-                store_chunk(yg, p.ldy, v);
+                store_chunk(yg, p.ldy, v, my);
             }
         }
 }
diff --git a/facialmmt_amd/csrc/gemm_ph3.h b/facialmmt_amd/csrc/gemm_ph3.h
--- a/facialmmt_amd/csrc/gemm_ph3.h
+++ b/facialmmt_amd/csrc/gemm_ph3.h
@@ -19,8 +19,9 @@
 
 template <int EPI = 2, bool STAGGER = true, int WT = 2>
 __global__ __launch_bounds__(512) void linear_nt_ph3_kernel(LinArgs p) {
-    const int p_M = p.M, p_K = p.K, p_ldx = p.ldx, p_ldw = p.ldw, p_ldy = p.ldy, p_ldaux = p.ldaux, p_ldres = p.ldres, p_tiles_m = p.tiles_m, p_tiles_n = p.tiles_n,
-              p_rows_per_scale = p.rows_per_scale;
+    const int p_M = p.m_rows ? min(max(*p.m_rows, 0), p.M) : p.M;
+    const int p_K = p.K, p_ldx = p.ldx, p_ldw = p.ldw, p_ldy = p.ldy, p_ldaux = p.ldaux, p_ldres = p.ldres, p_tiles_n = p.tiles_n, p_rows_per_scale = p.rows_per_scale;
+    const int p_tiles_m = p.m_rows ? (p_M + (WT * 96) - 1) / (WT * 96) : p.tiles_m;
     const void* const p_x = p.x; const void* const p_w = p.w; const void* const p_aux = p.aux; const void* const p_res = p.res;
     void* const p_y = p.y; void* const p_y_pre = p.y_pre;
     const float* const p_bias = p.bias; const float* const p_rowscale = p.rowscale;
diff --git a/facialmmt_amd/csrc/layernorm.hip b/facialmmt_amd/csrc/layernorm.hip
--- a/facialmmt_amd/csrc/layernorm.hip
+++ b/facialmmt_amd/csrc/layernorm.hip
@@ -19,6 +19,10 @@
     const void* add;
     void* dx;
     float* part;
+    const int* m_rows;
+    const int* row_delta;
+    int rows_per_img;
+    void* copy_dst;
 };
 
 template <bool MERGE>
@@ -49,14 +53,23 @@
     const T* __restrict__ xg = reinterpret_cast<const T*>(p.x);
     T* __restrict__ yg = reinterpret_cast<T*>(p.y);
     const float invC = 1.0f / (float)p.C;
+    const int m_rows = p.m_rows ? min(max(*p.m_rows, 0), p.M) : p.M;
     for (int row = blockIdx.x * ROWS + rib; row < p.M; row += gridDim.x * ROWS) {
+        const int xrow = p.row_delta ? row + p.row_delta[row / p.rows_per_img] : row;
+        if (row >= m_rows) {
+            if (p.copy_dst) {
+                T* __restrict__ cg = reinterpret_cast<T*>(p.copy_dst);
+                for (int c = sub; c < chunks; c += G) stvec<T>(cg + (size_t)xrow * p.C + c * VEC, ldvec<T>(xg + (size_t)xrow * p.C + c * VEC));
+            }
+            continue;
+        }
         Vec<T> v[NCH];
         float s = 0.f;
 #pragma unroll
         for (int i = 0; i < NCH; ++i) {
             const int c = sub + i * G;
             if (c < chunks) {
-                v[i] = ldvec<T>(xg + src_offset<MERGE>(row, c * VEC, p.C, p.merge_hw));
+                v[i] = ldvec<T>(xg + src_offset<MERGE>(xrow, c * VEC, p.C, p.merge_hw));
 #pragma unroll
                 for (int e = 0; e < VEC; ++e) s += v[i].get(e);
             }
@@ -114,7 +127,21 @@
 #pragma unroll
         for (int e = 0; e < VEC; ++e) dg[i][e] = db[i][e] = 0.f;
 
+    const int m_rows = p.m_rows ? min(max(*p.m_rows, 0), p.M) : p.M;
     for (int row = blockIdx.x * ROWS + rib; row < p.M; row += gridDim.x * ROWS) {
+        const int xrow = p.row_delta ? row + p.row_delta[row / p.rows_per_img] : row;
+        if (row >= m_rows) {
+            for (int c = sub; c < chunks; c += G) {
+                Vec<T> o;
+                if (addg) o = ldvec<T>(addg + (size_t)xrow * p.C + c * VEC);
+                else {
+#pragma unroll
+                    for (int e = 0; e < VEC; ++e) o.set(e, 0.f);
+                }
+                stvec<T>(dxg + (size_t)xrow * p.C + c * VEC, o);
+            }
+            continue;
+        }
         const float mean = p.mean[row], rstd = p.rstd[row];
         constexpr bool EARLY_ADD = MERGE || NCH >= 3;
         Vec<T> xv[NCH], gv[NCH], avp[EARLY_ADD ? NCH : 1];
@@ -124,7 +151,7 @@
             for (int i = 0; i < NCH; ++i) {
                 const int c = sub + i * G;
                 if (c < chunks) {
-                    const size_t off = src_offset<MERGE>(row, c * VEC, p.C, p.merge_hw);
+                    const size_t off = src_offset<MERGE>(xrow, c * VEC, p.C, p.merge_hw);
                     xv[i] = ldvec<T>(xg + off);
                     gv[i] = ldvec<T>(dyg + (size_t)row * p.C + c * VEC);
                     if (addg) avp[i] = ldvec<T>(addg + off);
@@ -136,7 +163,7 @@
             const int c = sub + i * G;
             if (c < chunks) {
                 if constexpr (!EARLY_ADD) {
-                    xv[i] = ldvec<T>(xg + src_offset<MERGE>(row, c * VEC, p.C, p.merge_hw));
+                    xv[i] = ldvec<T>(xg + src_offset<MERGE>(xrow, c * VEC, p.C, p.merge_hw));
                     gv[i] = ldvec<T>(dyg + (size_t)row * p.C + c * VEC);
                 }
 #pragma unroll
@@ -157,7 +184,7 @@
         for (int i = 0; i < NCH; ++i) {
             const int c = sub + i * G;
             if (c < chunks) {
-                const size_t off = src_offset<MERGE>(row, c * VEC, p.C, p.merge_hw);
+                const size_t off = src_offset<MERGE>(xrow, c * VEC, p.C, p.merge_hw);
                 Vec<T> o, av;
                 if constexpr (EARLY_ADD) {
                     if (addg) av = avp[i];
@@ -269,12 +296,14 @@
 
 }
 
-extern "C" int fmmt_layernorm_fwd(int dtype, int M, int C, const void* x, const float* gamma, const float* beta,
-                                  float eps, void* y, float* mean, float* rstd, int merge_hw, void* stream) {
+namespace {
+int ln_fwd_launch(int dtype, int M, int C, const void* x, const float* gamma, const float* beta, float eps, void* y, float* mean, float* rstd, int merge_hw,
+                  const int* m_rows, const int* row_delta, int rows_per_img, void* copy_dst, void* stream) {
     if (int e = check_ln(dtype, M, C, merge_hw)) return e;
     LnArgs a{};
     a.M = M; a.C = C; a.x = x; a.gamma = gamma; a.beta = beta; a.eps = eps; a.y = y; a.mean = mean; a.rstd = rstd;
     a.merge_hw = merge_hw;
+    a.m_rows = m_rows; a.row_delta = row_delta; a.rows_per_img = rows_per_img; a.copy_dst = copy_dst;
     hipStream_t st = reinterpret_cast<hipStream_t>(stream);
     const int vec = dtype == FMMT_BF16 ? 8 : 4;
     int g, nch;
@@ -285,18 +314,31 @@
     if (dtype == FMMT_BF16) return merge_hw ? launch_ln<bf16, true, false>(a, g, nch, grid, st) : launch_ln<bf16, false, false>(a, g, nch, grid, st);
     return merge_hw ? launch_ln<float, true, false>(a, g, nch, grid, st) : launch_ln<float, false, false>(a, g, nch, grid, st);
 }
+}
+
+extern "C" int fmmt_layernorm_fwd(int dtype, int M, int C, const void* x, const float* gamma, const float* beta,
+                                  float eps, void* y, float* mean, float* rstd, int merge_hw, void* stream) {
+    return ln_fwd_launch(dtype, M, C, x, gamma, beta, eps, y, mean, rstd, merge_hw, nullptr, nullptr, 1, nullptr, stream);
+}
+
+extern "C" int fmmt_layernorm_fwd_rows(int dtype, int M, int C, const void* x, const float* gamma, const float* beta, float eps, void* y, float* mean,
+                                       float* rstd, const int* m_rows, const int* row_delta, int rows_per_img, void* copy_dst, void* stream) {
+    if (!m_rows || (row_delta && (rows_per_img <= 0 || M % rows_per_img))) return FMMT_EINVAL;
+    return ln_fwd_launch(dtype, M, C, x, gamma, beta, eps, y, mean, rstd, 0, m_rows, row_delta, rows_per_img, copy_dst, stream);
+}
 
 extern "C" size_t fmmt_layernorm_bwd_workspace(int C) { return (size_t)LN_BWD_MAX_BLOCKS * 2 * (size_t)C * sizeof(float); }
 
-extern "C" int fmmt_layernorm_bwd(int dtype, int M, int C, const void* dy, const void* x, const float* mean,
-                                  const float* rstd, const float* gamma, const void* add, void* dx,
-                                  float* dgamma, float* dbeta, int merge_hw,
-                                  void* workspace, size_t workspace_bytes, void* stream) {
+namespace {
+int ln_bwd_launch(int dtype, int M, int C, const void* dy, const void* x, const float* mean, const float* rstd, const float* gamma, const void* add, void* dx,
+                  float* dgamma, float* dbeta, int merge_hw, void* workspace, size_t workspace_bytes,
+                  const int* m_rows, const int* row_delta, int rows_per_img, void* stream) {
     if (int e = check_ln(dtype, M, C, merge_hw)) return e;
     if (workspace_bytes < fmmt_layernorm_bwd_workspace(C)) return FMMT_EWORKSPACE;
     LnArgs a{};
     a.M = M; a.C = C; a.x = x; a.gamma = gamma; a.mean = const_cast<float*>(mean); a.rstd = const_cast<float*>(rstd);
     a.merge_hw = merge_hw; a.dy = dy; a.add = add; a.dx = dx; a.part = reinterpret_cast<float*>(workspace);
+    a.m_rows = m_rows; a.row_delta = row_delta; a.rows_per_img = rows_per_img;
     hipStream_t st = reinterpret_cast<hipStream_t>(stream);
     const int vec = dtype == FMMT_BF16 ? 8 : 4;
     int g, nch;
@@ -312,3 +354,18 @@
     FMMT_CHECK_LAUNCH();
     return 0;
 }
+}
+
+extern "C" int fmmt_layernorm_bwd(int dtype, int M, int C, const void* dy, const void* x, const float* mean,
+                                  const float* rstd, const float* gamma, const void* add, void* dx,
+                                  float* dgamma, float* dbeta, int merge_hw,
+                                  void* workspace, size_t workspace_bytes, void* stream) {
+    return ln_bwd_launch(dtype, M, C, dy, x, mean, rstd, gamma, add, dx, dgamma, dbeta, merge_hw, workspace, workspace_bytes, nullptr, nullptr, 1, stream);
+}
+
+extern "C" int fmmt_layernorm_bwd_rows(int dtype, int M, int C, const void* dy, const void* x, const float* mean, const float* rstd, const float* gamma,
+                                       const void* add, void* dx, float* dgamma, float* dbeta, void* workspace, size_t workspace_bytes,
+                                       const int* m_rows, const int* row_delta, int rows_per_img, void* stream) {
+    if (!m_rows || (row_delta && (rows_per_img <= 0 || M % rows_per_img))) return FMMT_EINVAL;
+    return ln_bwd_launch(dtype, M, C, dy, x, mean, rstd, gamma, add, dx, dgamma, dbeta, 0, workspace, workspace_bytes, m_rows, row_delta, rows_per_img, stream);
+}
diff --git a/facialmmt_amd/csrc/rows.hip b/facialmmt_amd/csrc/rows.hip
--- /dev/null
+++ b/facialmmt_amd/csrc/rows.hip
@@ -0,0 +1,78 @@
+#include "fmmt_common.h"
+#include "../../include/fmmt.h"
+
+namespace {
+
+constexpr int PLAN_THREADS = 256;
+
+__global__ __launch_bounds__(PLAN_THREADS) void droppath_plan_kernel(const float* __restrict__ scale, int n_img, int granule, int tokens,
+                                                                     int* __restrict__ perm, float* __restrict__ scale_c, int* __restrict__ delta,
+                                                                     int* __restrict__ words) {
+    __shared__ int cnt[PLAN_THREADS + 1];
+    const int d = blockIdx.x, t = threadIdx.x;
+    const float* s = scale + (size_t)d * n_img;
+    const int per = (n_img + PLAN_THREADS - 1) / PLAN_THREADS;
+    const int i0 = min(t * per, n_img), i1 = min(i0 + per, n_img);
+    int k = 0;
+    for (int i = i0; i < i1; ++i) k += s[i] != 0.f ? 1 : 0;
+    cnt[t + 1] = k;
+    if (t == 0) cnt[0] = 0;
+    __syncthreads();
+    if (t == 0)
+        for (int i = 1; i <= PLAN_THREADS; ++i) cnt[i] += cnt[i - 1];
+    __syncthreads();
+    const int n_keep = cnt[PLAN_THREADS];
+    int kept_before = cnt[t];
+    for (int i = i0; i < i1; ++i) {
+        const bool kept = s[i] != 0.f;
+        const int c = kept ? kept_before : n_keep + (i - kept_before);
+        perm[(size_t)d * n_img + c] = i;
+        scale_c[(size_t)d * n_img + c] = s[i];
+        delta[(size_t)d * n_img + c] = (i - c) * tokens;
+        kept_before += kept ? 1 : 0;
+    }
+    if (t == 0) {
+        const int up = (n_keep + granule - 1) / granule * granule;
+        const int n_proc = min(n_img, max(granule, up));
+        words[2 * d] = n_proc;
+        words[2 * d + 1] = n_proc * tokens;
+    }
+}
+
+__global__ __launch_bounds__(256) void gather_rows_kernel(const uint4* __restrict__ src, uint4* __restrict__ dst, int M, int chunks, int tokens,
+                                                          const int* __restrict__ m_rows, const int* __restrict__ delta) {
+    const int rows = min(max(*m_rows, 0), M);
+    const long long total = (long long)rows * chunks;
+    for (long long q = (long long)blockIdx.x * 256 + threadIdx.x; q < total; q += (long long)gridDim.x * 256) {
+        const int r = (int)(q / chunks), c = (int)(q - (long long)r * chunks);
+        const int sr = r + delta[r / tokens];
+        dst[(size_t)r * chunks + c] = src[(size_t)sr * chunks + c];
+    }
+}
+
+bool aligned16r(const void* p) { return (reinterpret_cast<uintptr_t>(p) & 15) == 0; }
+
+}
+
+extern "C" int fmmt_droppath_plan(int n_draws, int n_img, int granule, int tokens, const float* scale, int* perm, float* scale_c, int* row_delta,
+                                  int* words, void* stream) {
+    if (n_draws <= 0 || n_img <= 0 || granule <= 0 || tokens <= 0 || n_img % granule || n_img > 65536) return FMMT_EINVAL;
+    if ((long long)n_img * tokens >= (1ll << 31)) return FMMT_EINVAL;
+    if (!scale || !perm || !scale_c || !row_delta || !words) return FMMT_EINVAL;
+    hipLaunchKernelGGL(droppath_plan_kernel, dim3(n_draws), dim3(PLAN_THREADS), 0, reinterpret_cast<hipStream_t>(stream), scale, n_img, granule, tokens,
+                       perm, scale_c, row_delta, words);
+    FMMT_CHECK_LAUNCH();
+    return 0;
+}
+
+extern "C" int fmmt_gather_rows(int M, size_t row_bytes, int tokens, const void* src, void* dst, const int* m_rows, const int* row_delta, void* stream) {
+    if (M <= 0 || row_bytes == 0 || tokens <= 0 || M % tokens || !src || !dst || !m_rows || !row_delta) return FMMT_EINVAL;
+    if (row_bytes % 16 || !aligned16r(src) || !aligned16r(dst)) return FMMT_EALIGN;
+    const int chunks = (int)(row_bytes / 16);
+    long long blocks = ((long long)M * chunks + 255) / 256;
+    if (blocks > 4096) blocks = 4096;
+    hipLaunchKernelGGL(gather_rows_kernel, dim3((unsigned)blocks), dim3(256), 0, reinterpret_cast<hipStream_t>(stream),
+                       reinterpret_cast<const uint4*>(src), reinterpret_cast<uint4*>(dst), M, chunks, tokens, m_rows, row_delta);
+    FMMT_CHECK_LAUNCH();
+    return 0;
+}
diff --git a/facialmmt_amd/modules/SwinTransformer/Swin_Transformer.py b/facialmmt_amd/modules/SwinTransformer/Swin_Transformer.py
--- a/facialmmt_amd/modules/SwinTransformer/Swin_Transformer.py
+++ b/facialmmt_amd/modules/SwinTransformer/Swin_Transformer.py
@@ -15,6 +15,7 @@
         raise NotImplementedError("facialmmt_amd HIP path: " + msg)
 
 
+DROP_PATH_ROWS = True
 DROP_PATH_ONE_DRAW = True
 
 
@@ -24,13 +25,18 @@
         super().__init__()
         self.drop_prob = float(drop_prob)
         self._rows = None
+        self._plans = None
+        self.last_plan = None
 
     def sample_scale(self, n: int, device):
+        self.last_plan = None
         if self.drop_prob == 0.0 or not self.training:
             return None
         if self._rows:
             row = self._rows.pop(0)
+            plan = self._plans.pop(0) if self._plans else None
             if row.shape[0] == n and row.device == torch.device(device):
+                self.last_plan = plan
                 return row
         keep = 1.0 - self.drop_prob
         return torch.empty(n, dtype=torch.float32, device=device).bernoulli_(keep).div_(keep)
@@ -192,8 +198,12 @@
         if ops.mlp_ln_fusable(x, mlp.fc1.weight, mlp.fc2.weight, mlp.fc1.bias, mlp.fc2.bias) and (mlp.drop.p == 0.0 or not self.training):
             return ops.mlp_ln(x, self.norm2.weight, self.norm2.bias, self.norm2.eps, mlp.fc1.weight, mlp.fc1.bias, mlp.fc2.weight, mlp.fc2.bias,
                               self._scale(B, x.device), L)
+        scale = self._scale(B, x.device)
+        plan = self.drop_path.last_plan if scale is not None else None
+        if plan is not None and DROP_PATH_ROWS and (mlp.drop.p == 0.0 or not self.training) and ops.mlp_rows_ok(x, mlp.fc1.weight, mlp.fc2.weight, mlp.fc1.bias, mlp.fc2.bias, L):
+            return ops.mlp_rows(x, self.norm2.weight, self.norm2.bias, self.norm2.eps, mlp.fc1.weight, mlp.fc1.bias, mlp.fc2.weight, mlp.fc2.bias, plan, L)
         x, xn = ops.residual_layer_norm(x, self.norm2.weight, self.norm2.bias, self.norm2.eps)
-        return mlp(xn, res=x, rowscale=self._scale(B, x.device), rows_per_scale=L)
+        return mlp(xn, res=x, rowscale=scale, rows_per_scale=L)
 
     def extra_repr(self) -> str:
         return (f"dim={self.dim}, input_resolution={self.input_resolution}, num_heads={self.num_heads}, "
@@ -356,13 +366,24 @@
     def _draw_drop_paths(self, n, device):
         dps = [blk.drop_path for layer in self.layers for blk in layer.blocks if isinstance(blk.drop_path, DropPath) and blk.drop_path.drop_prob > 0.0]
         for dp in dps:
-            dp._rows = None
+            dp._rows = dp._plans = None
         if not DROP_PATH_ONE_DRAW or not self.training or not dps or self._dp_keep.numel() != 2 * len(dps) or self._dp_keep.device != torch.device(device):
             return
         keep = self._dp_keep
         pool = torch.where(torch.rand(keep.shape[0], n, dtype=torch.float32, device=device) < keep, self._dp_inv, 0.0)
         for i, dp in enumerate(dps):
             dp._rows = [pool[2 * i], pool[2 * i + 1]]
+        if DROP_PATH_ROWS and self.patch_embed.proj.weight.is_cuda:
+            i = 0
+            for layer in self.layers:
+                mine = [blk.drop_path for blk in layer.blocks if isinstance(blk.drop_path, DropPath) and blk.drop_path.drop_prob > 0.0]
+                g = ops.DROP_ROWS_GRANULE.get(layer.dim)
+                if mine and g and n % g == 0:
+                    H, W = layer.input_resolution
+                    plans = ops.droppath_plan(pool[2 * i:2 * (i + len(mine))], g, H * W)
+                    for j, dp in enumerate(mine):
+                        dp._plans = [None, plans[2 * j + 1]]
+                i += len(mine)
 
     def _init_weights(self, m):
         if isinstance(m, nn.Linear):
diff --git a/facialmmt_amd/ops.py b/facialmmt_amd/ops.py
--- a/facialmmt_amd/ops.py
+++ b/facialmmt_amd/ops.py
@@ -33,11 +33,16 @@
     return torch.empty(max(int(nbytes), 16), dtype=torch.uint8, device=device)
 
 
-def linear_raw(x2, w, bias, *, epi=EPI_NONE, y_pre=None, aux=None, res=None, rowscale=None, rows_per_scale=1):
+def linear_raw(x2, w, bias, *, epi=EPI_NONE, y_pre=None, aux=None, res=None, rowscale=None, rows_per_scale=1, m_rows=None, row_delta=None, out=None):
     M, K = x2.shape
     N = w.shape[0]
-    y = torch.empty((M, N), dtype=x2.dtype, device=x2.device)
+    y = out if out is not None else torch.empty((M, N), dtype=x2.dtype, device=x2.device)
     lib = _lib.load()
+    if m_rows is not None:
+        rc = lib.fmmt_linear_fwd_rows(dtype_code(x2.dtype), M, N, K, _p(x2), K, _p(w), K, _p(bias), _p(y), N, _p(y_pre),
+                                      epi, _p(aux), N, _p(res), N, _p(rowscale), rows_per_scale, _p(m_rows), _p(row_delta), _st())
+        check(rc, f"fmmt_linear_fwd_rows(M={M},N={N},K={K})")
+        return y
     if epi == EPI_NONE and res is None and rowscale is None and K >= 4096:
         nbytes = lib.fmmt_linear_splitk_workspace(M, N, K)
         if nbytes:
@@ -52,15 +57,25 @@
     return y
 
 
-def wgrad_partials_raw(dy2, x2, want_bias, ws, nbytes, rowscale=None, rows_per_scale=1, x_gelu=False):
+_WGRAD_ROWS = [None]
+
+
+def wgrad_partials_raw(dy2, x2, want_bias, ws, nbytes, rowscale=None, rows_per_scale=1, x_gelu=False, m_rows=None):
     M, N = dy2.shape
     K = x2.shape[1]
+    if m_rows is None:
+        m_rows = _WGRAD_ROWS[0]
+    if m_rows is not None:
+        rc = _lib.load().fmmt_linear_wgrad_partials_rows(dtype_code(dy2.dtype), M, N, K, _p(dy2), N, _p(x2), K, 1 if want_bias else 0, _p(rowscale), rows_per_scale,
+                                                         EPI_GELU if x_gelu else EPI_NONE, _p(ws), nbytes, _p(m_rows), _st())
+        check(rc, f"fmmt_linear_wgrad_partials_rows(M={M},N={N},K={K})")
+        return
     rc = _lib.load().fmmt_linear_wgrad_partials(dtype_code(dy2.dtype), M, N, K, _p(dy2), N, _p(x2), K, 1 if want_bias else 0,
                                                 _p(rowscale), rows_per_scale, EPI_GELU if x_gelu else EPI_NONE, _p(ws), nbytes, _st())
     check(rc, f"fmmt_linear_wgrad_partials(M={M},N={N},K={K})")
 
 
-def wgrad_raw(dy2, x2, want_bias, rowscale=None, rows_per_scale=1, x_gelu=False, out=None):
+def wgrad_raw(dy2, x2, want_bias, rowscale=None, rows_per_scale=1, x_gelu=False, out=None, m_rows=None):
     M, N = dy2.shape
     K = x2.shape[1]
     lib = _lib.load()
@@ -72,12 +87,16 @@
         db = torch.empty((N,), dtype=torch.float32, device=dy2.device) if want_bias else None
     nbytes = lib.fmmt_linear_wgrad_workspace(dtype_code(dy2.dtype), M, N, K)
     ws = _ws(nbytes, dy2.device)
-    if M <= 2048:
+    if M <= 2048 and m_rows is None:
         rc = lib.fmmt_linear_wgrad(dtype_code(dy2.dtype), M, N, K, _p(dy2), N, _p(x2), K, _p(dw), _p(db), _p(rowscale), rows_per_scale,
                                    EPI_GELU if x_gelu else EPI_NONE, _p(ws), nbytes, _st())
         check(rc, f"fmmt_linear_wgrad(M={M},N={N},K={K})")
         return dw, db
-    wgrad_partials_raw(dy2, x2, want_bias, ws, nbytes, rowscale, rows_per_scale, x_gelu)
+    _WGRAD_ROWS[0] = m_rows
+    try:
+        wgrad_partials_raw(dy2, x2, want_bias, ws, nbytes, rowscale, rows_per_scale, x_gelu)
+    finally:
+        _WGRAD_ROWS[0] = None
     rc = lib.fmmt_linear_wgrad_finish(dtype_code(dy2.dtype), M, N, K, _p(dw), _p(db), _p(ws), nbytes, _st())
     check(rc, f"fmmt_linear_wgrad_finish(M={M},N={N},K={K})")
     return dw, db
@@ -709,6 +728,130 @@
 
 def mlp(x, w1, b1, w2, b2, res=None, rowscale=None, rows_per_scale=1):
     return MlpFn.apply(x, w1, b1, w2, b2, res, rowscale, rows_per_scale, torch.is_grad_enabled())
+
+
+DROP_ROWS_GRANULE = {384: 16}
+
+
+class DropPlan:
+    __slots__ = ("perm", "scale_c", "row_delta", "n_proc", "m_rows")
+
+    def __init__(self, perm, scale_c, row_delta, words):
+        self.perm, self.scale_c, self.row_delta, self.n_proc, self.m_rows = perm, scale_c, row_delta, words[0:1], words[1:2]
+
+
+def droppath_plan(scale, granule, tokens):
+    _need_cuda(scale, "droppath_plan")
+    scale = scale.contiguous()
+    d, n = scale.shape
+    perm = torch.empty((d, n), dtype=torch.int32, device=scale.device)
+    delta = torch.empty_like(perm)
+    scale_c = torch.empty_like(scale)
+    words = torch.empty((d, 2), dtype=torch.int32, device=scale.device)
+    check(_lib.load().fmmt_droppath_plan(d, n, granule, tokens, _p(scale), _p(perm), _p(scale_c), _p(delta), _p(words), _st()), f"fmmt_droppath_plan(n={n},G={granule})")
+    return [DropPlan(perm[i], scale_c[i], delta[i], words[i]) for i in range(d)]
+
+
+def droppath_plan_reference(scale, granule, tokens):
+    d, n = scale.shape
+    if n % granule:
+        raise ValueError(f"n_img={n} is no multiple of the granule {granule}: no plan, the block takes the plain path")
+    kept = scale != 0
+    perm = torch.argsort((~kept).to(torch.int8), dim=1, stable=True).to(torch.int32)
+    scale_c = torch.gather(scale, 1, perm.long())
+    delta = (perm - torch.arange(n, dtype=torch.int32, device=scale.device)) * tokens
+    n_keep = kept.sum(1)
+    n_proc = torch.clamp((n_keep + granule - 1) // granule * granule, min=granule, max=n).to(torch.int32)
+    return perm, scale_c, delta.to(torch.int32), torch.stack((n_proc, n_proc * tokens), dim=1).to(torch.int32)
+
+
+def gather_rows(src2, tokens, m_rows, row_delta):
+    dst = torch.empty_like(src2)
+    M = src2.shape[0]
+    check(_lib.load().fmmt_gather_rows(M, src2.shape[1] * src2.element_size(), tokens, _p(src2), _p(dst), _p(m_rows), _p(row_delta), _st()), f"fmmt_gather_rows(M={M})")
+    return dst
+
+
+_ROWS_OK: dict = {}
+MLP_ROWS_FAMILIES = (256, 192, 36, 192, 192, 192)
+
+
+def mlp_rows_kernels(M, C, tokens):
+    lib = _lib.load()
+    return (lib.fmmt_linear_fwd_rows_kernel(M, 4 * C, C, 1, 1, EPI_GELU_DG, 0, 0, 0, 1, 0),
+            lib.fmmt_linear_fwd_rows_kernel(M, C, 4 * C, 1, 0, EPI_NONE, 0, 1, 1, tokens, 1),
+            lib.fmmt_linear_fwd_rows_kernel(M, 4 * C, C, 0, 0, EPI_MUL_AUX, 1, 0, 1, tokens, 0),
+            lib.fmmt_linear_fwd_rows_kernel(M, C, 4 * C, 0, 0, EPI_NONE, 0, 0, 0, 1, 0),
+            lib.fmmt_linear_wgrad_rows_kernel(M, C, 4 * C, 1, tokens),
+            lib.fmmt_linear_wgrad_rows_kernel(M, 4 * C, C, 0, 1))
+
+
+def mlp_rows_shape_ok(M, C, tokens, dtype) -> bool:
+    g = DROP_ROWS_GRANULE.get(C)
+    if not g or dtype != torch.bfloat16 or M <= 0 or M % (g * tokens):
+        return False
+    key = (M, C, tokens)
+    if key not in _ROWS_OK:
+        _ROWS_OK[key] = mlp_rows_kernels(M, C, tokens) == MLP_ROWS_FAMILIES
+    return _ROWS_OK[key]
+
+
+def mlp_rows_ok(x, w1, w2, b1, b2, tokens) -> bool:
+    C = x.shape[-1]
+    return bool(x.is_cuda and torch.is_grad_enabled() and w1.shape == (4 * C, C) and w2.shape == (C, 4 * C) and b1 is not None and b2 is not None
+                and _MLP_SAVE_DG and _MLP_SAVE_H and mlp_rows_shape_ok(x.numel() // C, C, tokens, x.dtype))
+
+
+class MlpRowsFn(Function):
+
+    @staticmethod
+    def forward(ctx, x, ln_w, ln_b, eps, w1, b1, w2, b2, scale_c, row_delta, m_rows, tokens):
+        _need_cuda(x, "mlp_rows")
+        lib = _lib.load()
+        C = x.shape[-1]
+        x2 = x.reshape(-1, C).contiguous()
+        M, dev, dt = x2.shape[0], x.device, x.dtype
+        g, b = ln_w.detach().float().contiguous(), ln_b.detach().float().contiguous()
+        xn = torch.empty_like(x2)
+        y = torch.empty_like(x2)
+        mean = torch.empty(M, dtype=torch.float32, device=dev)
+        rstd = torch.empty(M, dtype=torch.float32, device=dev)
+        check(lib.fmmt_layernorm_fwd_rows(dtype_code(dt), M, C, _p(x2), _p(g), _p(b), float(eps), _p(xn), _p(mean), _p(rstd), _p(m_rows), _p(row_delta), tokens,
+                                          _p(y), _st()), f"fmmt_layernorm_fwd_rows(M={M},C={C})")
+        w1l, w2l = _lp(w1, dt), _lp(w2, dt)
+        dg = torch.empty((M, w1.shape[0]), dtype=dt, device=dev)
+        h = linear_raw(xn, w1l, b1.detach(), epi=EPI_GELU_DG, y_pre=dg, m_rows=m_rows)
+        linear_raw(h, w2l, b2.detach(), res=x2, rowscale=scale_c, rows_per_scale=tokens, m_rows=m_rows, row_delta=row_delta, out=y)
+        ctx.save_for_backward(x2, xn, mean, rstd, g, w1, w2, dg, h, scale_c, row_delta, m_rows)
+        ctx.tokens = tokens
+        ctx.xshape = x.shape
+        return y.reshape(x.shape)
+
+    @staticmethod
+    def backward(ctx, dy):
+        x2, xn, mean, rstd, g, w1, w2, dg, h, scale_c, row_delta, m_rows = ctx.saved_tensors
+        lib = _lib.load()
+        C, T = x2.shape[1], ctx.tokens
+        M, dt = x2.shape[0], x2.dtype
+        dy2 = dy.reshape(-1, C).contiguous()
+        dyc = gather_rows(dy2, T, m_rows, row_delta)
+        dh = linear_raw(dyc, _lp(w2, dt, transpose=True), None, epi=EPI_MUL_AUX, aux=dg, rowscale=scale_c, rows_per_scale=T, m_rows=m_rows)
+        dw2, db2 = wgrad_raw(dyc, h, True, scale_c, T, m_rows=m_rows)
+        dxn = linear_raw(dh, _lp(w1, dt, transpose=True), None, m_rows=m_rows)
+        dw1, db1 = wgrad_raw(dh, xn, True, m_rows=m_rows)
+        del dh
+        dx = torch.empty_like(x2)
+        dgam = torch.empty(C, dtype=torch.float32, device=x2.device)
+        dbet = torch.empty(C, dtype=torch.float32, device=x2.device)
+        nbytes = lib.fmmt_layernorm_bwd_workspace(C)
+        ws = _ws(nbytes, x2.device)
+        check(lib.fmmt_layernorm_bwd_rows(dtype_code(dt), M, C, _p(dxn), _p(x2), _p(mean), _p(rstd), _p(g), _p(dy2), _p(dx), _p(dgam), _p(dbet), _p(ws), nbytes,
+                                          _p(m_rows), _p(row_delta), T, _st()), f"fmmt_layernorm_bwd_rows(M={M},C={C})")
+        return dx.reshape(ctx.xshape), dgam, dbet, None, dw1, db1, dw2, db2, None, None, None, None
+
+
+def mlp_rows(x, ln_w, ln_b, eps, w1, b1, w2, b2, plan, tokens):
+    return MlpRowsFn.apply(x, ln_w, ln_b, eps, w1, b1, w2, b2, plan.scale_c, plan.row_delta, plan.m_rows, tokens)
 
 
 class LayerNormFn(Function):
diff --git a/include/fmmt.h b/include/fmmt.h
--- a/include/fmmt.h
+++ b/include/fmmt.h
@@ -204,6 +204,7 @@
 #include "fmmt_eval_collect.h"
 #include "fmmt_pool_head_rows.h"
 #include "fmmt_guard.h"
+#include "fmmt_rows.h"
 
 #ifdef __cplusplus
 }
diff --git a/include/fmmt_rows.h b/include/fmmt_rows.h
--- /dev/null
+++ b/include/fmmt_rows.h
@@ -0,0 +1,31 @@
+#ifndef FMMT_ROWS_H
+#define FMMT_ROWS_H
+#include <stddef.h>
+#include <stdint.h>
+
+#ifdef __cplusplus
+extern "C" {
+#endif
+
+int fmmt_droppath_plan(int n_draws, int n_img, int granule, int tokens, const float* scale, int32_t* perm, float* scale_c, int32_t* row_delta,
+                       int32_t* words, void* stream);
+int fmmt_gather_rows(int M, size_t row_bytes, int tokens, const void* src, void* dst, const int32_t* m_rows, const int32_t* row_delta, void* stream);
+int fmmt_linear_fwd_rows(int dtype, int M, int N, int K, const void* x, int ldx, const void* w, int ldw, const float* bias, void* y, int ldy,
+                         void* y_pre, int epi, const void* aux, int ldaux, const void* res, int ldres, const float* rowscale, int rows_per_scale,
+                         const int32_t* m_rows, const int32_t* row_delta, void* stream);
+int fmmt_linear_fwd_rows_kernel(int M, int N, int K, int has_bias, int has_y_pre, int epi, int has_aux, int has_res, int has_rowscale, int rows_per_scale,
+                                int has_row_delta);
+int fmmt_linear_wgrad_rows_kernel(int M, int N, int K, int has_rowscale, int rows_per_scale);
+int fmmt_linear_wgrad_partials_rows(int dtype, int M, int N, int K, const void* dy, int lddy, const void* x, int ldx, int want_bias,
+                                    const float* rowscale, int rows_per_scale, int x_epi, void* workspace, size_t workspace_bytes,
+                                    const int32_t* m_rows, void* stream);
+int fmmt_layernorm_fwd_rows(int dtype, int M, int C, const void* x, const float* gamma, const float* beta, float eps, void* y, float* mean,
+                            float* rstd, const int32_t* m_rows, const int32_t* row_delta, int rows_per_img, void* copy_dst, void* stream);
+int fmmt_layernorm_bwd_rows(int dtype, int M, int C, const void* dy, const void* x, const float* mean, const float* rstd, const float* gamma,
+                            const void* add, void* dx, float* dgamma, float* dbeta, void* workspace, size_t workspace_bytes,
+                            const int32_t* m_rows, const int32_t* row_delta, int rows_per_img, void* stream);
+
+#ifdef __cplusplus
+}
+#endif
+#endif
```

Result: faster. 74.96 utterances/s (median of 6 runs) (+1.3%).
